# suryatmodulus/livekit-server

Hardware: AMD Instinct MI355X
Metric: forwarded RTP pkts/sec per GPU & node (bit-exact) + % HBM roofline (higher is better)
Workload: dtype u8; 1 GPU; configs[1]: 100 rooms x 10 participants per GPU, VP8 3-layer simulcast + Opus, 18000 DownTracks, 2% loss, 1% reorder, layer switching; batch=1 s of media per step, step=raw datagrams -> Buffer.calc -> forward (lkf_ingest_device + lkf_run), parallelism=room-sharded x1

## Files before the change

### livekit-server_amd/csrc/forward_kernels.hip

```cpp
#include <hip/hip_runtime.h>

#include "../../include/lkfwd.h"
#ifndef LKF_SVC_STATS
#define LKF_SVC_STATS 0
#endif
#if LKF_SVC_STATS
__device__ unsigned long long g_svc[64 * 48];
#define SVC_ADD(k, v) atomicAdd(&g_svc[(blockIdx.x & 63) * 48 + (k)], (unsigned long long)(v))
#endif
#include "dd_device.h"
#include "fwd_state.h"
#include "kernels.h"
#include "sender_device.h"

namespace lkf {

using u8 = uint8_t;
using u16 = uint16_t;
using u32 = uint32_t;
using u64 = uint64_t;
using i32 = int32_t;
using i64 = int64_t;

constexpr u64 HALF64 = 1ull << 63;
constexpr i32 INVALID = -1;


#ifndef LKF_CHECKED
#define LKF_CHECKED 0
#endif
#if LKF_CHECKED
__device__ unsigned long long g_chk[4];
__device__ __noinline__ void chk_fail(u32 site, u64 idx, u64 cap) {
  if (atomicAdd(&g_chk[0], 1ull) == 0) {
    g_chk[1] = site;
    g_chk[2] = idx;
    g_chk[3] = cap;
  }
}
#define CHK(cond, site, idx, cap)                   \
  do {                                              \
    if (!(cond)) chk_fail(site, u64(idx), u64(cap)); \
  } while (0)
#else
#define CHK(cond, site, idx, cap) \
  do {                            \
  } while (0)
#endif
enum ChkSite : u32 {
  CK_DEC_DT = 1,
  CK_DEC_TRACK,
  CK_DEC_PKT,
  CK_DEC_TUPLE,
  CK_DEC_SEQ,
  CK_DEC_LAYER,
  CK_DEC_EVENT,
  CK_EMIT_POS,
  CK_EMIT_DT,
  CK_EMIT_TUPLE,
  CK_EMIT_PKT,
  CK_EMIT_ARENA,
  CK_EMIT_OUT,
  CK_EMIT_BYTES,
  CK_EMIT_DD,
  CK_EMIT_GROUP,
  CK_PAD_DT,
  CK_PAD_SEQ,
  CK_EV_ORDER,
};

struct PktV {
  u64 esn, ets;
  i64 arr;
  u32 arenaOff, ssrc;
  u16 poff, plen;
  u8 hdr0, hdr1, flags, vfirst, vbits, vhs, tl0, tid, keyidx, vp9;
  int8_t spatial, temporal, layer;
  u16 pid;
};

__device__ __forceinline__ PktV decode_pkt(uint4 a, uint4 b, uint4 c, uint4 d) {
  PktV v;
  v.esn = (u64(a.y) << 32) | a.x;
  v.ets = (u64(a.w) << 32) | a.z;
  v.arr = i64((u64(b.y) << 32) | b.x);
  v.arenaOff = b.z;
  v.ssrc = c.x;
  v.poff = u16(c.y & 0xffff);
  v.plen = u16(c.y >> 16);
  v.hdr0 = u8(c.z);
  v.hdr1 = u8(c.z >> 8);
  v.spatial = int8_t(c.z >> 16);
  v.temporal = int8_t(c.z >> 24);
  v.flags = u8(c.w);
  v.vfirst = u8(c.w >> 8);
  v.vbits = u8(c.w >> 16);
  v.vhs = u8(c.w >> 24);
  v.pid = u16(d.x & 0xffff);
  v.tl0 = u8(d.x >> 16);
  v.tid = u8(d.x >> 24);
  v.keyidx = u8(d.y);
  v.layer = int8_t(d.y >> 8);
  v.vp9 = u8(d.y >> 24);
  return v;
}

__device__ __forceinline__ PktV load_pkt(const lkf_pkt *p) {
  const uint4 *q = reinterpret_cast<const uint4 *>(p);
  return decode_pkt(q[0], q[1], q[2], q[3]);
}

__device__ __forceinline__ uint4 rfl(uint4 v) {
  v.x = __builtin_amdgcn_readfirstlane(v.x);
  v.y = __builtin_amdgcn_readfirstlane(v.y);
  v.z = __builtin_amdgcn_readfirstlane(v.z);
  v.w = __builtin_amdgcn_readfirstlane(v.w);
  return v;
}

__device__ __forceinline__ u32 lane_id() { return threadIdx.x & 63u; }
__device__ __forceinline__ u32 rl32(u32 v, u32 l) { return __builtin_amdgcn_readlane(v, l); }
__device__ __forceinline__ u64 rl64(u64 v, u32 l) {
  return (u64(rl32(u32(v >> 32), l)) << 32) | u64(rl32(u32(v), l));
}
__device__ __forceinline__ u32 sh32(u32 v, int src) { return u32(__shfl(int(v), src, 64)); }
__device__ __forceinline__ u64 sh64(u64 v, int src) {
  return (u64(sh32(u32(v >> 32), src)) << 32) | u64(sh32(u32(v), src));
}
__device__ __forceinline__ int prev_in(u64 m, u64 lt) {
  const u64 pm = m & lt;
  return pm ? 63 - __clzll(pm) : -1;
}
__device__ __forceinline__ u32 excl_scan_u32(u32 v, u32 lane) {
  u32 x = v;
#pragma unroll
  for (int o = 1; o < 64; o <<= 1) {
    u32 y = u32(__shfl_up(int(x), o, 64));
    if (lane >= u32(o)) x += y;
  }
  return x - v;
}
__device__ __forceinline__ u32 wave_sum_u32(u32 v) {
#pragma unroll
  for (int o = 32; o > 0; o >>= 1) v += u32(__shfl_xor(int(v), o, 64));
  return v;
}
__device__ __forceinline__ u64 wave_max_u64(u64 v) {
#pragma unroll
  for (int o = 32; o > 0; o >>= 1) {
    u64 y = sh64(v, int(threadIdx.x) ^ o);
    v = y > v ? y : v;
  }
  return v;
}

__device__ __forceinline__ u64 wave_or_u64(u64 v) {
#pragma unroll
  for (int o = 32; o > 0; o >>= 1) v |= sh64(v, int(threadIdx.x) ^ o);
  return rl64(v, 0);
}
__device__ __forceinline__ void wave_lds_sync() { __syncthreads(); }

struct Lane {
  DTHot &h;
  RangeEntry *rm;
  RangeEntry *rmG;
  u32 rmNew;
  bool rmLoaded;
  bool vcDirty;
  VP8Cold *vc;
  i32 *dropKey;
  i32 *exKey;
  i32 *missKey;
  i32 *missVal;
  SeqMeta *seq;
  u32 seqSize;
  SeqRM *srm;
  u32 srmCap;
  u32 kind, codec, hasRefTS, clockRate;
  u32 *offs;
  u8 extPlayout, extAbs, extDD, extTcc;
  DDState *dd;
  const DDStruct *ddRing;
  DDStruct *ddS;
  u32 ddSSlot;
  const DDPkt *ddPkts;
  const u16 *ddSpill;
  u8 *ddBuf;
  DDPkt *ddPktL;
  u32 *err;
};

__device__ __forceinline__ bool hasf(const Lane &L, u32 f) { return (L.h.flags & f) != 0; }
__device__ __forceinline__ void setf(Lane &L, u32 f, bool v) {
  if (v)
    L.h.flags |= f;
  else
    L.h.flags &= ~f;
}

__device__ __forceinline__ RangeEntry rm_at(const Lane &L, int i) {
  int idx = (int(L.h.rmHead) + i) % kRangeCap;
  return L.rm[idx];
}
__device__ __forceinline__ void rm_load(Lane &L) {
  if (L.rmLoaded) return;
  L.rmLoaded = true;
  const u32 nc = L.h.rmCount, old = nc - min(L.rmNew, nc);
  if (!old) return;
  wave_lds_sync();
  for (u32 i = lane_id(); i < old; i += 64) {
    const u32 idx = (u32(L.h.rmHead) + i) % kRangeCap;
    L.rm[idx] = L.rmG[idx];
  }
  wave_lds_sync();
}
__device__ __forceinline__ void rm_reset(Lane &L, u64 start, u64 val) {
  L.h.rmHead = 0;
  L.h.rmCount = 0;
  L.rmNew = 0;
  L.h.rmOpenStart = start;
  L.h.rmOpenValue = val;
}
__device__ __forceinline__ bool rm_exclude(Lane &L, u64 s, u64 e) {
  if (e == s || (e - s) > HALF64) return false;
  if (L.h.rmOpenStart > s) return false;
  u64 nv = L.h.rmOpenValue + (e - s);
  if (L.h.rmOpenStart == s) {
    L.h.rmOpenStart = e;
    L.h.rmOpenValue = nv;
    return true;
  }
  RangeEntry c;
  c.start = L.h.rmOpenStart;
  c.end = s - 1;
  c.value = L.h.rmOpenValue;
  if (L.h.rmCount < kRangeCap) {
    int idx = (int(L.h.rmHead) + int(L.h.rmCount)) % kRangeCap;
    L.rm[idx] = c;
    L.h.rmCount++;
  } else {
    L.rm[L.h.rmHead] = c;
    L.h.rmHead = u16((L.h.rmHead + 1) % kRangeCap);
  }
  L.rmNew++;
  L.h.rmOpenStart = e;
  L.h.rmOpenValue = nv;
  return true;
}
__device__ __forceinline__ bool rm_get(Lane &L, u64 key, u64 &out) {
  out = 0;
  if (key >= L.h.rmOpenStart) {
    out = L.h.rmOpenValue;
    return true;
  }
  const int nc = L.h.rmCount;
  if (nc == 0) return false;
  rm_load(L);
  if (key < rm_at(L, 0).start) return false;
  const u32 l = lane_id();
  int best = -1;
  bool bestIn = false;
  u64 bestVal = 0;
  for (int base = 0; base <= nc; base += 64) {
    const int i = base + int(l);
    bool in = false, between = false;
    u64 val = 0;
    if (i <= nc) {
      u64 nextStart = L.h.rmOpenStart;
      if (i < nc) {
        const RangeEntry rv = rm_at(L, i);
        in = (key - rv.start) < HALF64 && (rv.end - key) < HALF64;
        val = rv.value;
        nextStart = rv.start;
      }
      if (i > 0) {
        const u64 before = key - rm_at(L, i - 1).end;
        const u64 after = nextStart - key;
        between = before > 0 && before < HALF64 && after > 0 && after < HALF64;
      }
    }
    const u64 m = __ballot(in || between);
    if (m) {
      const u32 j = 63 - __clzll(m);
      best = base + int(j);
      bestIn = rl32(u32(in), j) != 0;
      bestVal = rl64(val, j);
    }
  }
  if (best < 0 || !bestIn) return false;
  out = bestVal;
  return true;
}

__device__ __forceinline__ void mg_updateSnOffset(Lane &L) {
  u64 v = 0;
  rm_get(L, L.h.extHighestIncomingSN + 1, v);
  L.h.snOffset = v;
}
__device__ __forceinline__ void mg_setLastSnTs(Lane &L, u64 esn, u64 ets) {
  L.h.extHighestIncomingSN = esn - 1;
  L.h.extLastSN = esn;
  L.h.extSecondLastSN = esn - 1;
  rm_reset(L, esn, 0);
  mg_updateSnOffset(L);
  L.h.extLastTS = ets;
  L.h.extSecondLastTS = ets;
}
__device__ __forceinline__ void mg_updateSnTsOffsets(Lane &L, u64 esn, u64 ets, u64 snAdj, u64 tsAdj) {
  L.h.extHighestIncomingSN = esn - 1;
  rm_reset(L, esn, esn - L.h.extLastSN - snAdj);
  mg_updateSnOffset(L);
  L.h.tsOffset = ets - L.h.extLastTS - tsAdj;
}
__device__ __forceinline__ void mg_packetDropped(Lane &L, u64 esn) {
  if (L.h.extHighestIncomingSN != esn) return;
  rm_exclude(L, L.h.extHighestIncomingSN, L.h.extHighestIncomingSN + 1);
  L.h.extLastSN = L.h.extSecondLastSN;
  mg_updateSnOffset(L);
  L.h.extLastTS = L.h.extSecondLastTS;
  setf(L, F_LAST_MARKER, hasf(L, F_SECOND_LAST_MARKER));
}
enum { ORD_CONTIG = 0, ORD_OOO = 1, ORD_GAP = 2, ORD_DUP = 3 };
enum { MG_OK = 0, MG_PADDING, MG_DUP, MG_OOO_MISS };
__device__ __forceinline__ void mg_inorder(Lane &L, const PktV &p, bool marker, u64 &osn, u64 &ots) {
  L.h.extHighestIncomingSN = p.esn;
  u64 msn = p.esn - L.h.snOffset;
  u64 mts = p.ets - L.h.tsOffset;
  L.h.extSecondLastSN = L.h.extLastSN;
  L.h.extLastSN = msn;
  L.h.extSecondLastTS = L.h.extLastTS;
  L.h.extLastTS = mts;
  setf(L, F_SECOND_LAST_MARKER, hasf(L, F_LAST_MARKER));
  setf(L, F_LAST_MARKER, marker);
  if (p.flags & LKF_PKT_KEYFRAME) {
    L.h.extRtxGateSn = msn;
    setf(L, F_RTX_GATE, true);
  }
  if (hasf(L, F_RTX_GATE) && (msn - L.h.extRtxGateSn) > 2000) setf(L, F_RTX_GATE, false);
  osn = msn;
  ots = mts;
}

__device__ int mg_update(Lane &L, const PktV &p, bool marker, int &ord, u64 &osn, u64 &ots) {
  i64 diff = i64(p.esn - L.h.extHighestIncomingSN);
  if ((diff == 1 && p.plen != 0) || diff > 1) {
    L.h.extHighestIncomingSN = p.esn;
    ord = diff > 1 ? ORD_GAP : ORD_CONTIG;
    u64 msn = p.esn - L.h.snOffset;
    u64 mts = p.ets - L.h.tsOffset;
    L.h.extSecondLastSN = L.h.extLastSN;
    L.h.extLastSN = msn;
    L.h.extSecondLastTS = L.h.extLastTS;
    L.h.extLastTS = mts;
    setf(L, F_SECOND_LAST_MARKER, hasf(L, F_LAST_MARKER));
    setf(L, F_LAST_MARKER, marker);
    if (p.flags & LKF_PKT_KEYFRAME) {
      L.h.extRtxGateSn = msn;
      setf(L, F_RTX_GATE, true);
    }
    if (hasf(L, F_RTX_GATE) && (msn - L.h.extRtxGateSn) > 2000) setf(L, F_RTX_GATE, false);
    osn = msn;
    ots = mts;
    return MG_OK;
  }
  if (diff < 0) {
    ord = ORD_OOO;
    u64 off = 0;
    if (!rm_get(L, p.esn, off)) return MG_OOO_MISS;
    u64 esn = p.esn - off;
    if (esn >= L.h.extLastSN) return MG_OOO_MISS;
    osn = esn;
    ots = p.ets - L.h.tsOffset;
    return MG_OK;
  }
  if (diff == 1) {
    L.h.extHighestIncomingSN = p.esn;
    rm_exclude(L, L.h.extHighestIncomingSN, L.h.extHighestIncomingSN + 1);
    mg_updateSnOffset(L);
    ord = ORD_CONTIG;
    return MG_PADDING;
  }
  ord = ORD_DUP;
  return MG_DUP;
}

__device__ __forceinline__ int miss_find(const Lane &L, i32 key) {
  const u32 l = lane_id();
  for (int base = 0; base < int(L.h.missCount); base += 64) {
    const int i = base + int(l);
    const int idx = (L.h.missHead + i) % kMissCap;
    const u64 m = __ballot(i < int(L.h.missCount) && L.missKey[idx] == key);
    if (m) return (L.h.missHead + base + __ffsll((long long)m) - 1) % kMissCap;
  }
  return -1;
}
__device__ __forceinline__ bool set_has(const i32 *keys, u8 head, u8 count, i32 key) {
  for (int i = 0; i < count; i++)
    if (keys[(head + i) % kSetCap] == key) return true;
  return false;
}
__device__ __forceinline__ bool set_has_u(const i32 *keys, u8 head, u8 count, i32 key) {
  const u32 l = lane_id();
  return __ballot(l < count && keys[(head + l) % kSetCap] == key) != 0;
}
__device__ __forceinline__ void set_add(i32 *keys, u8 &head, u8 &count, i32 key, int keep) {
  if (set_has_u(keys, head, count, key)) return;
  wave_lds_sync();
  keys[(head + count) % kSetCap] = key;
  count++;
  if (count > keep) {
    head = u8((head + count - keep) % kSetCap);
    count = u8(keep);
  }
  wave_lds_sync();
}

__device__ void vp8_record_missing_wide(Lane &L, i32 prevMax, i32 ext, i32 off) {
  const int e0 = L.h.missCount;
  int inE = 0;
  for (int i = 0; i < e0; i++) {
    int idx = (L.h.missHead + i) % kMissCap;
    i32 k = L.missKey[idx];
// ... 316 lines not shown
      break;
  }
}

__device__ bool fw_sourceSwitch(Lane &L, const PktV &p, i32 layer) {
  if (!hasf(L, F_STARTED)) {
    setf(L, F_STARTED, true);
    L.h.referenceLayerSpatial = layer;
    mg_setLastSnTs(L, p.esn, p.ets);
    if (hasf(L, F_VP8)) vp8_setLast(L, p);
    return true;
  } else if (L.h.referenceLayerSpatial == INVALID) {
    L.h.referenceLayerSpatial = layer;
  }
  const u64 extLastTS = L.h.extLastTS;
  u64 extExpectedTS = extLastTS;
  u64 extRefTS = extExpectedTS;
  if (L.hasRefTS) {
    i32 ref = L.h.referenceLayerSpatial;
    if (layer < 0 || layer >= 3 || ref < 0 || ref >= 3) return false;
    const bool svc = L.codec == LKF_CODEC_VP9 || L.codec == LKF_CODEC_AV1;
    const u32 off = svc ? 0u : L.offs[ref * 3 + layer];
    if (!svc && layer != ref && off == 0) return false;
    u32 ts = u32(p.ets) + off;
    extRefTS = (extRefTS & 0xFFFFFFFF00000000ull) + u64(ts);
    u32 e32 = u32(extExpectedTS);
    if (u32(ts - e32) < (1u << 31) && ts < e32) extRefTS += (1ull << 32);
    if (u32(e32 - ts) < (1u << 31) && e32 < ts && extRefTS >= (1ull << 32)) extRefTS -= (1ull << 32);
  }
  if (hasf(L, F_HAS_EXPECTED)) {
    if (hasf(L, F_STATS_INIT)) {
      i64 diff = (p.arr - L.h.statsFirstTime) * i64(L.clockRate) / 1000000000LL;
      extExpectedTS = L.h.statsExtStartTS + u64(diff);
    } else if (L.h.preStartTime != 0) {
      i64 since = p.arr - L.h.preStartTime;
      u64 rtpDiff = u64(since * i64(L.clockRate) / 1000000000LL);
      extExpectedTS = L.h.extFirstTS + rtpDiff;
      if (L.h.refTSOffset == 0) L.h.refTSOffset = extExpectedTS - extRefTS;
    }
  }
  extRefTS += L.h.refTSOffset;
  u64 extNextTS;
  const double cr = double(L.clockRate);
  if (L.h.lastSSRC == 0) {
    double diffSeconds = double(i64(extExpectedTS - extRefTS)) / cr;
    if (diffSeconds >= 0.0) {
      if (hasf(L, F_RESUME_BEHIND) && diffSeconds > 0.2)
        extNextTS = extExpectedTS;
      else if (diffSeconds > 2.0)
        extNextTS = extExpectedTS;
      else
        extNextTS = extRefTS;
    } else {
      extNextTS = extRefTS;
    }
    setf(L, F_RESUME_BEHIND, false);
  } else {
    double diffSeconds = double(i64(extRefTS - extLastTS)) / cr;
    if (diffSeconds < 0.0) {
      if (fabs(diffSeconds) > 0.05) return false;
      extNextTS = extLastTS + 1;
    } else {
      extNextTS = extRefTS;
    }
  }
  if (i64(extNextTS - extLastTS) <= 0) extNextTS = extLastTS + 1;
  mg_updateSnTsOffsets(L, p.esn, p.ets, 1, extNextTS - extLastTS);
  if (hasf(L, F_VP8)) vp8_updateOffsets(L, p);
  return true;
}

__device__ __forceinline__ int fw_common(Lane &L, const PktV &p, i32 layer, bool marker, int &ord, u64 &osn,
                                         u64 &ots) {
  if (L.h.lastSSRC != p.ssrc) {
    if (!fw_sourceSwitch(L, p, layer)) return LKF_DROP_SWITCH;
    L.h.lastSSRC = p.ssrc;
  }
  int r = mg_update(L, p, marker, ord, osn, ots);
  if (r == MG_PADDING) return LKF_DROP_PADDING;
  if (r == MG_DUP) return LKF_DROP_DUPLICATE;
  if (r == MG_OOO_MISS) return LKF_DROP_OOO_MISS;
  return -1;
}

template <bool DDK = false>
__device__ __forceinline__ void vls_rollback(Lane &L) {
  if (DDK && hasf(L, F_DD)) {
    L.dd->mask = L.dd->prevMask;
    if (L.dd->flags & DS_HAS_PREV_MASK)
      L.dd->flags |= DS_HAS_MASK;
    else
      L.dd->flags &= ~u32(DS_HAS_MASK);
  }
  L.h.curS = L.h.prevS;
  L.h.curT = L.h.prevT;
  L.h.tgtS = L.h.ptgtS;
  L.h.tgtT = L.h.ptgtT;
}

struct Fwd {
  int ord;
  u64 osn, ots;
  bool switching, resuming, marker;
  int cbLen;
  u64 cb;
  int ddLen;
};

template <bool DDK>
__device__ int fw_translate(Lane &L, const PktV &p, u32 k, Fwd &o) {
  o.switching = o.resuming = o.marker = false;
  o.cbLen = 0;
  o.cb = 0;
  o.ddLen = 0;
  const i32 layer = p.layer;
  if (hasf(L, F_MUTED) || hasf(L, F_PUBMUTED)) return LKF_DROP_MUTED;
  if (!hasf(L, F_VIDEO)) return fw_common(L, p, layer, false, o.ord, o.osn, o.ots);
  if (L.h.tgtS == INVALID || L.h.tgtT == INVALID) return LKF_DROP_PAUSED;
  bool isSelected = false, isSwitching = false, isResuming = false;
  const bool kf = p.flags & LKF_PKT_KEYFRAME;
  const bool pktMarker = p.hdr1 & 0x80;
  if (hasf(L, F_SIMULCAST)) {
    if (L.h.curS != L.h.tgtS) {
      bool isActive = L.h.curS != INVALID && L.h.curT != INVALID;
      bool found = false;
      if (kf) {
        if (layer > L.h.curS && layer <= L.h.tgtS) found = true;
        if (layer < L.h.curS && layer >= L.h.tgtS) found = true;
      }
      if (found) {
        L.h.prevS = L.h.curS;
        L.h.prevT = L.h.curT;
        L.h.curS = layer;
        L.h.curT = p.temporal;
        L.h.ptgtS = L.h.tgtS;
        L.h.ptgtT = L.h.tgtT;
        if (L.h.curS >= L.h.maxS || L.h.curS == L.h.seenS) L.h.tgtS = L.h.curS;
        isSwitching = true;
        if (!isActive) isResuming = true;
      }
    }
    if (L.h.curS > L.h.maxS && layer <= L.h.maxS && kf) {
      L.h.prevS = L.h.curS;
      L.h.prevT = L.h.curT;
      L.h.curS = layer;
      L.h.ptgtS = L.h.tgtS;
      L.h.ptgtT = L.h.tgtT;
      if (L.h.curS >= L.h.maxS || L.h.curS == L.h.seenS) L.h.tgtS = layer;
      isSwitching = true;
    }
    isSelected = layer == L.h.curS;
  }
  bool marker = pktMarker;
  if (hasf(L, F_VP9)) {
    bool relevant = false;
    if (p.flags & LKF_PKT_VP9) {
      const bool U = p.vp9 & LKF_VP9_U, B = p.vp9 & LKF_VP9_B, E = p.vp9 & LKF_VP9_E, P = p.vp9 & LKF_VP9_P;
      const i32 pS = p.spatial, pT = p.temporal;
      i32 cS = L.h.curS, cT = L.h.curT;
      bool zero = false;
      if (L.h.curS != L.h.tgtS || L.h.curT != L.h.tgtT) {
        i32 uS = L.h.curS, uT = L.h.curT;
        const bool curValid = L.h.curS != INVALID && L.h.curT != INVALID;
        if (!curValid) {
          if (!kf)
            zero = true;
          else {
            uS = pS;
            uT = pT;
          }
        } else {
          if (L.h.curT != L.h.tgtT) {
            if (L.h.curT < L.h.tgtT) {
              if (pT > L.h.curT && pT <= L.h.tgtT && U && B) cT = uT = pT;
            } else if (E) {
              uT = L.h.tgtT;
            }
          }
          if (L.h.curS != L.h.tgtS) {
            if (L.h.curS < L.h.tgtS) {
              if (pS > L.h.curS && pS <= L.h.tgtS && !P && B) cS = uS = pS;
            } else if (E) {
              uS = L.h.tgtS;
            }
          }
        }
        if (!zero && (uS != L.h.curS || uT != L.h.curT)) {
          isSwitching = true;
          if (!curValid && uS != INVALID && uT != INVALID) isResuming = true;
          L.h.prevS = L.h.curS;
          L.h.prevT = L.h.curT;
          L.h.curS = uS;
          L.h.curT = uT;
        }
      }
      if (!zero) {
        if (E && pS == cS && (P || L.h.tgtS <= L.h.curS)) marker = true;
        isSelected = !(pS > cS || (pS == cS && pT > cT));
        relevant = true;
      }
    }
    if (!isSelected) {
      if (relevant && hasf(L, F_STARTED)) {
        int ord;
        u64 a, b;
        if (mg_update(L, p, marker, ord, a, b) == MG_OK && ord == ORD_CONTIG) mg_packetDropped(L, p.esn);
      }
      return LKF_DROP_NOT_SELECTED;
    }
  }
  if (DDK && hasf(L, F_DD)) {
    const bool inDD = (p.flags & LKF_PKT_DD) && L.ddPkts;
    if (inDD) {
      const u32 ln = lane_id();
      if (ln < sizeof(DDPkt) / 16)
        reinterpret_cast<uint4 *>(L.ddPktL)[ln] = reinterpret_cast<const uint4 *>(L.ddPkts + k)[ln];
      wave_lds_sync();
    }
    const bool hasDD = inDD && (L.ddPktL->flags & DP_VALID);
#if LKF_SVC_STATS
    const u64 tS0 = __builtin_amdgcn_s_memtime();
#endif
    const dd::SelResult r = dd::dd_select(*L.dd, L.ddRing, hasDD ? L.ddPktL : nullptr, pktMarker, L.h.curS, L.h.curT, L.h.prevS,
                                          L.h.prevT, L.h.tgtS, L.h.tgtT, L.ddBuf, L.ddS, L.ddSSlot, L.ddSpill);
#if LKF_SVC_STATS
    if (lane_id() == 0) {
      SVC_ADD(13, __builtin_amdgcn_s_memtime() - tS0);
      SVC_ADD(14, 1ull);
    }
#endif
    if (r.limit && lane_id() == 0) atomicOr(L.err, 16u);
    L.ddSSlot = r.stagedSlot;
    if (!r.selected) {
      if (r.relevant && hasf(L, F_STARTED)) {
        int ord;
        u64 a, b;
        if (mg_update(L, p, false, ord, a, b) == MG_OK && ord == ORD_CONTIG) mg_packetDropped(L, p.esn);
      }
      return LKF_DROP_NOT_SELECTED;
    }
    isSelected = true;
    isSwitching = r.switching;
    isResuming = r.resuming;
    marker = r.marker;
    o.ddLen = r.ddLen;
  }
  if (!isSelected) return LKF_DROP_NOT_SELECTED;
  o.resuming = isResuming;
  o.switching = isSwitching;
  o.marker = marker;
  if (hasf(L, F_DEFICIENT) && L.h.tgtS < L.h.curS) {
    if (isSwitching) vls_rollback<DDK>(L);
    return LKF_DROP_DOWNGRADE;
  }
  int dr = fw_common(L, p, layer, marker, o.ord, o.osn, o.ots);
  if (dr >= 0 || p.plen == 0) {
    if (isSwitching) vls_rollback<DDK>(L);
    return dr;
  }
  i32 tl = L.h.curT;
  bool tSwitch = false;
  if (hasf(L, F_TLS_VP8)) {
    i32 cur = L.h.curT, tgt = L.h.tgtT, nxt = cur;
    if (cur != tgt && (p.flags & LKF_PKT_VP8) && (p.vbits & LKF_VP8_T)) {
      i32 tid = i32(p.tid);
      if (cur < tgt) {
        if (tid > cur && tid <= tgt && (p.vbits & LKF_VP8_S) && (p.vbits & LKF_VP8_Y)) {
          tl = tid;
          nxt = tid;
        }
      } else if (pktMarker) {
        nxt = tgt;
      }
    }
    if (nxt != L.h.curT) {
      tSwitch = true;
      L.h.prevS = L.h.curS;
      L.h.prevT = L.h.curT;
      L.h.curT = nxt;
    }
  }
  if (hasf(L, F_VP8)) {
    int cr;
    if (!(p.flags & LKF_PKT_VP8))
      cr = CM_ERR;
    else
      cr = vp8_update(L, p, o.ord == ORD_OOO, o.ord == ORD_GAP, tl, o.cb, o.cbLen);
    if (cr != CM_OK) {
      if (cr == CM_FILTERED) mg_packetDropped(L, p.esn);
      if (isSwitching || tSwitch) vls_rollback<DDK>(L);
      return cr == CM_FILTERED ? LKF_DROP_TEMPORAL : cr == CM_PICID_MISS ? LKF_DROP_PICID_MISS : LKF_DROP_OTHER;
    }
  }
  return -1;
}


__device__ __forceinline__ u32 pack4(u8 a, u8 b, u8 c, u8 d) {
  return u32(a) | (u32(b) << 8) | (u32(c) << 16) | (u32(d) << 24);
}
struct __attribute__((aligned(8))) U4x8 {
  u32 x, y, z, w;
};
__device__ __forceinline__ void store_fwd(FwdRec *dst, FwdBase *wdst, u64 bSN, u64 bTS, u64 sn, u64 ts, u32 pkt,
                                          u32 relOff, u32 outLen, u32 flags, u32 ddLen, u32 aux) {
  if ((((sn - bSN) + 0x80000000ull) >> 32) != 0 || (((ts - bTS) + 0x80000000ull) >> 32) != 0) {
    flags |= T_WIDE;
    *wdst = FwdBase{sn, ts};
  }
  *reinterpret_cast<U4x8 *>(dst) = U4x8{u32(sn), u32(ts), pkt, relOff >> 4};
  reinterpret_cast<uint2 *>(dst)[2] = make_uint2(outLen | (flags << 16) | (ddLen << 24), aux);
}
__device__ __forceinline__ u32 vp8_aux(u32 mpid, u32 mtl0, u32 mkey) {
  return (mpid & 0xffffu) | ((mtl0 & 0xffu) << 16) | ((mkey & 0x1fu) << 24);
}
__device__ __forceinline__ u32 vp8_aux_of(u64 cb) {
  if (!(cb & 0x80)) return 0;
  const u32 x = u32(cb >> 8) & 0xff;
  int idx = 2;
  u32 pid = 0, tl0 = 0, key = 0;
  if (x & 0x80) {
    const u32 b = u32(cb >> (8 * idx)) & 0xff;
    if (b & 0x80) {
      pid = ((b & 0x7f) << 8) | (u32(cb >> (8 * (idx + 1))) & 0xff);
      idx += 2;
    } else {
      pid = b;
      idx++;
    }
  }
  if (x & 0x40) tl0 = u32(cb >> (8 * idx++)) & 0xff;
  if (x & 0x30) key = u32(cb >> (8 * idx)) & 0x1f;
  return vp8_aux(pid, tl0, key);
}
__device__ __forceinline__ void store_rec(SeqMeta *dst, const SeqMeta &m) {
  uint4 *d = reinterpret_cast<uint4 *>(dst);
  d[0] = make_uint4(u32(m.sourceSeqNo) | (u32(m.targetSeqNo) << 16), m.timestamp, m.lastNack,
                    pack4(m.marker, m.nacked, u8(m.layer), m.codecLen));
  d[1] = make_uint4(pack4(m.codec[0], m.codec[1], m.codec[2], m.codec[3]),
                    pack4(m.codec[4], m.codec[5], m.codec[6], m.codec[7]), 0u, 0u);
}

__device__ __forceinline__ void seq_invalidate(Lane &L, u32 n) {
  const SeqMeta z = {};
  for (u32 i = lane_id(); i < n; i += 64) {
    u32 x = u32(L.h.seqHighSlot) + 1 + i;
    while (x >= L.seqSize) x -= L.seqSize;
    store_rec(L.seq + x, z);
  }
}
__device__ __forceinline__ RangeEntry *srm_ring(SeqRM *h) { return reinterpret_cast<RangeEntry *>(h + 1); }
__device__ bool srm_get(SeqRM *h, u32 cap, u64 key, u64 &out) {
  out = 0;
  if (key >= h->openStart) {
    out = h->openValue;
    return true;
  }
  const u32 nc = h->count;
  const RangeEntry *ring = srm_ring(h);
  if (nc == 0 || key < ring[h->head].start) return false;
  for (i32 idx = i32(nc); idx >= 0; idx--) {
    u64 start = h->openStart;
    if (idx != i32(nc)) {
      const RangeEntry rv = ring[(h->head + u32(idx)) % cap];
      if ((key - rv.start) < HALF64 && (rv.end - key) < HALF64) {
        out = rv.value;
        return true;
      }
      start = rv.start;
    }
    if (idx > 0) {
      const RangeEntry pv = ring[(h->head + u32(idx) - 1) % cap];
      const u64 before = key - pv.end, after = start - key;
      if (before > 0 && before < HALF64 && after > 0 && after < HALF64) return false;
    }
  }
  return false;
}
__device__ bool srm_exclude(SeqRM *h, u32 cap, u64 s, u64 e, bool store) {
  if (e == s || (e - s) > HALF64) return false;
  if (h->openStart > s) return false;
  const u64 nv = h->openValue + (e - s);
  if (h->openStart == s) {
    if (store) {
      h->openStart = e;
      h->openValue = nv;
    }
    return true;
  }
  if (store) {
    RangeEntry c;
    c.start = h->openStart;
    c.end = s - 1;
    c.value = h->openValue;
    RangeEntry *ring = srm_ring(h);
    if (h->count < cap) {
      ring[(h->head + h->count) % cap] = c;
      h->count++;
    } else {
      ring[h->head] = c;
      h->head = (h->head + 1) % cap;
    }
    h->openStart = e;
    h->openValue = nv;
  }
  return true;
}
__device__ __noinline__ void seq_push_rm(DTHot *h, SeqMeta *seq, u32 size, SeqRM *srm, u32 cap, u64 esn,
                                         const SeqMeta *rec, u64 ets) {
  const bool init = !(h->flags & F_SEQ_INIT);
  u64 snOff = srm->snOffset;
  if (init) {
    h->flags |= F_SEQ_INIT;
    h->seqExtStartSN = esn;
    h->seqExtHighestSN = esn;
    h->seqExtHighestTS = ets;
    u64 off = 0;
    if (srm_get(srm, cap, esn + 1, off)) snOff = off;
    if (lane_id() == 0) srm->snOffset = snOff;
    h->seqHighSlot = u16((esn - snOff) % size);
  }
  if (esn < h->seqExtStartSN) return;
  const u64 adjH = h->seqExtHighestSN - snOff;
  u64 adjM = esn - snOff;
  if (esn < h->seqExtHighestSN) {
    u64 off = 0;
    if (!srm_get(srm, cap, esn, off)) return;
    adjM = esn - off;
  }
  const i64 delta = i64(adjM - adjH);
  if (delta <= -i64(size)) return;
  u32 slot;
  if (delta >= 0) {
    slot = u32((u64(h->seqHighSlot) + u64(delta) % size) % size);
  } else {
    const i32 sl = i32(h->seqHighSlot) + i32(delta);
    slot = u32(sl < 0 ? sl + i32(size) : sl);
  }
  if (adjM > adjH + 1) {
    const u64 nInv = (adjM - adjH - 1) < u64(size) ? (adjM - adjH - 1) : u64(size);
    for (u32 i = lane_id(); i < u32(nInv); i += 64) seq[(u32(h->seqHighSlot) + 1 + i) % size] = SeqMeta{};
  }
  if (lane_id() == 0) seq[slot] = *rec;
  if (esn > h->seqExtHighestSN) {
    h->seqExtHighestSN = esn;
    h->seqHighSlot = u16(slot);
  }
  if (ets > h->seqExtHighestTS) h->seqExtHighestTS = ets;
}

template <bool RM>
__device__ void seq_push(Lane &L, i64 arrMs, u64 inSN, u64 esn, u64 ets, bool marker, int8_t layer, u64 cb,
                         int cbLen) {
  const u32 size = L.seqSize;
  if (hasf(L, F_SEQ_INIT) && esn == L.h.seqExtHighestSN + 1) {
    u32 slot = u32(L.h.seqHighSlot) + 1;
    if (slot == size) slot = 0;
    SeqMeta m = {};
    m.sourceSeqNo = u16(inSN);
    m.targetSeqNo = u16(esn);
    m.timestamp = u32(ets);
    m.lastNack = u32(arrMs - L.h.seqStartMs);
    m.marker = marker;
    m.layer = layer;
    m.codecLen = u8(cbLen);
#pragma unroll
    for (int i = 0; i < 8; i++) m.codec[i] = u8(cb >> (8 * i));
    CHK(slot < size, CK_DEC_SEQ, slot, size);
    if (lane_id() == 0) store_rec(L.seq + slot, m);
    L.h.seqExtHighestSN = esn;
    L.h.seqHighSlot = u16(slot);
    if (ets > L.h.seqExtHighestTS) L.h.seqExtHighestTS = ets;
    return;
  }

  if (hasf(L, F_SEQ_RM) && (!hasf(L, F_SEQ_INIT) || esn < L.h.seqExtHighestSN)) {
    if (!RM) {
      if (lane_id() == 0) atomicOr(L.err, 32u);
      return;
    }
    SeqMeta m = {};
    m.sourceSeqNo = u16(inSN);
    m.targetSeqNo = u16(esn);
    m.timestamp = u32(ets);
    m.lastNack = u32(arrMs - L.h.seqStartMs);
    m.marker = marker;
    m.layer = layer;
    m.codecLen = u8(cbLen);
#pragma unroll
    for (int i = 0; i < 8; i++) m.codec[i] = u8(cb >> (8 * i));
    __shared__ SeqMeta sRec;
    if (lane_id() == 0) sRec = m;
    __syncthreads();
    seq_push_rm(&L.h, L.seq, size, L.srm, L.srmCap, esn, &sRec, ets);
    __syncthreads();
    return;
  }
  if (!hasf(L, F_SEQ_INIT)) {
    setf(L, F_SEQ_INIT, true);
    L.h.seqExtStartSN = esn;
    L.h.seqExtHighestSN = esn;
    L.h.seqExtHighestTS = ets;
    L.h.seqHighSlot = u16(esn % size);
  }
  if (esn < L.h.seqExtStartSN) return;
  const u64 adjH = L.h.seqExtHighestSN;
  const u64 adjM = esn;
  const i64 delta = i64(adjM - adjH);
  if (delta <= -i64(size)) return;
  u32 slot;
  if (delta >= 0) {
    u32 dm = delta < i64(size) ? u32(delta) : u32(u64(delta) % size);
    slot = L.h.seqHighSlot + dm;
    if (slot >= size) slot -= size;
  } else {
    i32 sl = i32(L.h.seqHighSlot) + i32(delta);
    slot = u32(sl < 0 ? sl + i32(size) : sl);
  }
  if (adjM > adjH + 1) {
    const u64 nInv = (adjM - adjH - 1) < u64(size) ? (adjM - adjH - 1) : u64(size);
    seq_invalidate(L, u32(nInv));
  }
  SeqMeta m = {};
  m.sourceSeqNo = u16(inSN);
  m.targetSeqNo = u16(esn);
  m.timestamp = u32(ets);
  m.lastNack = u32(arrMs - L.h.seqStartMs);
  m.marker = marker;
  m.nacked = 0;
  m.layer = layer;
  m.codecLen = u8(cbLen);
#pragma unroll
  for (int i = 0; i < 8; i++) m.codec[i] = u8(cb >> (8 * i));
  CHK(slot < size, CK_DEC_SEQ, slot, size);
  L.seq[slot] = m;
  if (esn > L.h.seqExtHighestSN) {
    L.h.seqExtHighestSN = esn;
    L.h.seqHighSlot = u16(slot);
  }
  if (ets > L.h.seqExtHighestTS) L.h.seqExtHighestTS = ets;
}

__device__ __forceinline__ u64 wave_sum(u64 v) {
  for (int o = 32; o > 0; o >>= 1) v += __shfl_xor(v, o, 64);
  return v;
}

__global__ void k_batch_init(u32 ntracks, u32 ndts, u32 nstats, u32 *__restrict__ tBegin, u32 *__restrict__ tEnd,
                             u32 *__restrict__ tRuns, u32 *__restrict__ err, u64 *__restrict__ stats,
                             u32 *__restrict__ fwdCnt, u64 *__restrict__ fwdBytes) {
  const u32 stride = gridDim.x * blockDim.x;
  for (u32 i = blockIdx.x * blockDim.x + threadIdx.x; i < ntracks || i < ndts || i < nstats || i < 4; i += stride) {
    if (i < ntracks) {
      tBegin[i] = 0;
      tEnd[i] = 0;
      tRuns[i] = 0;
    }
    if (i < ndts) {
      fwdCnt[i] = 0;
      fwdBytes[i] = 0;
    }
    if (i < nstats) stats[i] = 0;
    if (i < 4) err[i] = 0;
  }
}

__global__ void k_track_ranges(const RunDesc *__restrict__ desc, u32 ntracks, u32 *__restrict__ tBegin,
                               u32 *__restrict__ tEnd, u32 *__restrict__ tRuns, u32 *__restrict__ err) {
  const lkf_pkt *__restrict__ pkts = reinterpret_cast<const lkf_pkt *>(desc->pkts);
  u32 n = desc->n;
  const u64 *nDev = reinterpret_cast<const u64 *>(desc->nDev);
  u32 i = blockIdx.x * blockDim.x + threadIdx.x;
  if (nDev && *nDev < n) n = u32(*nDev);
  if (i >= n) return;
  u32 t = pkts[i].track;
  if (t >= ntracks) {
    atomicOr(err, 1u);
    return;
  }
  u32 tp = i > 0 ? pkts[i - 1].track : 0xffffffffu;
  u32 tn = i + 1 < n ? pkts[i + 1].track : 0xffffffffu;
  if (tp != t) {
    tBegin[t] = i;
    if (atomicAdd(&tRuns[t], 1u) != 0) atomicOr(err, 2u);
  }
  if (tn != t) tEnd[t] = i + 1;
}

constexpr int SCAN_T = 256;
#ifndef LKF_SCAN_ITEMS
#define LKF_SCAN_ITEMS 4
#endif
constexpr int SCAN_ITEMS = LKF_SCAN_ITEMS;
constexpr int SCAN_TILE = SCAN_T * SCAN_ITEMS;

struct ScanIn {
  int mode;
  const u32 *perm;
  const DevDT *dts;
  const u32 *tBegin, *tEnd;
  const u32 *cnt;
  const u64 *bytes;
  u32 *gFirst;
  u64 gCap;
};

__device__ __forceinline__ void scan_load(const ScanIn &in, u32 i, u64 &a, u64 &b) {
  const u32 d = in.perm ? in.perm[i] : i;
  if (in.mode == 3) {
    a = in.cnt[i] != 0 ? 1 : 0;
    b = in.cnt[i] & 0xffffu;
    return;
  }
  if (in.mode == 2) {
    a = in.cnt[i];
    b = 0;
    return;
  }
  if (in.mode == 0) {
    DevDT dt = in.dts[d];
    a = dt.active ? u64(in.tEnd[dt.track] - in.tBegin[dt.track]) : 0;
    b = 0;
  } else {
    a = in.cnt[d];
    b = in.bytes[d];
  }
}

__device__ __forceinline__ void block_scan_excl(u64 &a, u64 &b, u64 &ta, u64 &tb) {
  const int lane = threadIdx.x & 63, wid = threadIdx.x >> 6;
  u64 ia = a, ib = b;
  for (int o = 1; o < 64; o <<= 1) {
    u64 xa = __shfl_up(ia, o, 64), xb = __shfl_up(ib, o, 64);
    if (lane >= o) {
      ia += xa;
      ib += xb;
    }
  }
  __shared__ u64 wa[SCAN_T / 64], wb[SCAN_T / 64];
  if (lane == 63) {
    wa[wid] = ia;
    wb[wid] = ib;
  }
  __syncthreads();
  u64 pa = 0, pb = 0;
  ta = tb = 0;
  for (int w = 0; w < SCAN_T / 64; w++) {
    if (w < wid) {
      pa += wa[w];
      pb += wb[w];
    }
    ta += wa[w];
    tb += wb[w];
  }
  __syncthreads();
  a = pa + ia - a;
  b = pb + ib - b;
}

constexpr u32 kScanStHead = 16;
constexpr u32 kScanSpin = 1u << 22;

__device__ __forceinline__ void gr_put(u64 *g, u32 v, u32 tag = 1) {
  __hip_atomic_store(g, (u64(tag) << 32) | u64(v), __ATOMIC_RELAXED, __HIP_MEMORY_SCOPE_AGENT);
}

__global__ void __launch_bounds__(SCAN_T) k_scan_1p(ScanIn in, u32 n, u32 nb, u64 *__restrict__ st,
                                                    u64 *__restrict__ outA, u64 *__restrict__ outB,
                                                    u64 *__restrict__ totA, u64 *__restrict__ totB) {
  __shared__ u32 sTile, sLast;
  __shared__ u64 sPre[2];
  __shared__ u32 sBad;
  u32 *const ctr = reinterpret_cast<u32 *>(st);
  u64 *const gr = st + kScanStHead;
  const u32 tid = threadIdx.x, lane = tid & 63;
  if (tid == 0) {
    sTile = atomicAdd(&ctr[0], 1u);
    sBad = 0;
  }
  __syncthreads();
  const u32 tile = sTile;
  const u32 i0 = tile * SCAN_TILE + tid * SCAN_ITEMS;
  u64 va[SCAN_ITEMS], vb[SCAN_ITEMS], ta = 0, tb = 0;
#pragma unroll
  for (int k = 0; k < SCAN_ITEMS; k++) {
    va[k] = vb[k] = 0;
    if (i0 + k < n) scan_load(in, i0 + k, va[k], vb[k]);
    ta += va[k];
    tb += vb[k];
  }
  u64 ea = ta, eb = tb, TA, TB;
  block_scan_excl(ea, eb, TA, TB);
  u64 *const g = gr + 8 * size_t(tile);
  if (tid == 0) {
    if (tile == 0) {
      gr_put(g + 4, u32(TA)), gr_put(g + 5, u32(TA >> 32)), gr_put(g + 6, u32(TB)), gr_put(g + 7, u32(TB >> 32));
      sPre[0] = sPre[1] = 0;
    } else {
      gr_put(g + 0, u32(TA)), gr_put(g + 1, u32(TA >> 32)), gr_put(g + 2, u32(TB)), gr_put(g + 3, u32(TB >> 32));
    }
  }
  if (tile > 0 && tid < 64) {
    u64 pa = 0, pb = 0;
    int j = int(tile) - 1;
    for (u32 spins = 0;;) {
      const u64 x = lane < 8 ? __hip_atomic_load(gr + 8 * size_t(j) + lane, __ATOMIC_RELAXED, __HIP_MEMORY_SCOPE_AGENT)
                             : 0ull;
      const u64 rdy = __ballot(lane < 8 && (x >> 32) != 0);
      const u64 poison = __ballot(lane < 8 && (x >> 32) == 2);
      const u32 v = u32(x);
      if ((rdy & 0xF0) == 0xF0 || (rdy & 0x0F) == 0x0F) {
        const int o = (rdy & 0xF0) == 0xF0 ? 4 : 0;
        if (poison & (0x0Full << o)) {
          if (lane == 0) sBad = 1;
          break;
        }
        const u64 a = (u64(u32(__shfl(int(v), o + 1, 64))) << 32) | u32(__shfl(int(v), o, 64));
        const u64 b = (u64(u32(__shfl(int(v), o + 3, 64))) << 32) | u32(__shfl(int(v), o + 2, 64));
        pa += a;
        pb += b;
        if (o == 4) break;
        j--;
        spins = 0;
        continue;
      }
      if (++spins > kScanSpin) {
        if (lane == 0) sBad = 1;
        break;
      }
      __builtin_amdgcn_s_sleep(1);
    }
    if (lane == 0) {
      const u64 ia = pa + TA, ib = pb + TB;
      const u32 tag = sBad ? 2u : 1u;
      gr_put(g + 4, u32(ia), tag), gr_put(g + 5, u32(ia >> 32), tag), gr_put(g + 6, u32(ib), tag),
          gr_put(g + 7, u32(ib >> 32), tag);
      sPre[0] = pa;
      sPre[1] = pb;
    }
  }
  __syncthreads();
  u64 ca = sPre[0] + ea, cb = sPre[1] + eb;
#pragma unroll
  for (int k = 0; k < SCAN_ITEMS; k++) {
    const u32 d = i0 + k;
    if (d < n) {
      outA[d] = ca;
      if (outB) outB[d] = cb;
      if (in.gFirst && va[k]) {
        const u64 r0 = ca, r1 = min(r0 + va[k], in.gCap);
        for (u64 gg = (r0 + 63) >> 6; (gg << 6) < r1; gg++) in.gFirst[gg] = d;
      }
    }
    ca += va[k];
    cb += vb[k];
  }
  if (tile == nb - 1 && tid == 0) {
    *totA = sBad ? ~0ull : sPre[0] + TA;
    if (totB) *totB = sBad ? ~0ull : sPre[1] + TB;
  }
  __syncthreads();
  if (tid == 0) sLast = atomicAdd(&ctr[2], 1u) == nb - 1 ? 1u : 0u;
  __syncthreads();
  if (sLast) {
    for (u32 k = tid; k < 8 * nb; k += SCAN_T)
      __hip_atomic_store(gr + k, 0ull, __ATOMIC_RELAXED, __HIP_MEMORY_SCOPE_AGENT);
    if (tid == 0) {
      __hip_atomic_store(&ctr[0], 0u, __ATOMIC_RELAXED, __HIP_MEMORY_SCOPE_AGENT);
      __hip_atomic_store(&ctr[2], 0u, __ATOMIC_RELAXED, __HIP_MEMORY_SCOPE_AGENT);
    }
  }
}

struct SsEnt;
struct LaneOut {
  FwdRec *outT;
  FwdBase *outW;
  u64 nFwd, nBytes, nTuples;
  u64 bSN, bTS;
  SenderStats *ss;
  u32 *ssRing, *ssGap;
  SsEnt *ssBuf;
  u32 ssN;
  i32 sentDiff;
  u32 relOff;
  u32 drops[LKF_DROP_NREASONS];
  u8 *ddArena;
  u64 *ddUsed;
  u64 ddCap;
#if LKF_CHECKED
  u64 tupBase, tupCap;
#endif
};

__device__ __forceinline__ double rl_f64(double v, u32 k) {
  return __builtin_bit_cast(double, rl64(__builtin_bit_cast(u64, v), k));
}

struct SsEnt {
  u32 sn, ts;
  i64 t;
  u32 hp;
  u32 fl;
};
static_assert(sizeof(SsEnt) == 24, "SsEnt is 24 B");
__device__ __forceinline__ void ss_put(SsEnt *e, u64 sn, u64 ts, i64 t, u32 hdr, u32 pay, bool marker, bool kf) {
  *reinterpret_cast<uint2 *>(e) = make_uint2(u32(sn), u32(ts));
  reinterpret_cast<uint2 *>(e)[1] = make_uint2(u32(u64(t)), u32(u64(t) >> 32));
  reinterpret_cast<uint2 *>(e)[2] = make_uint2(hdr | (pay << 16), (marker ? 1u : 0u) | (kf ? 2u : 0u));
}

#ifndef LKF_SS_SCALAR
#define LKF_SS_SCALAR 0
#endif
__device__ __forceinline__ void ss_flush(SenderStats &S, u32 *ring, u32 *gap, const SsEnt *buf, u32 m, u64 bSN,
                                      u64 bTS) {
  if (m <= u32(LKF_SS_SCALAR)) {
    for (u32 i = 0; i < m; i++) {
      const SsEnt &e = buf[i];
      ss::ss_update(S, ring, gap, e.t, widen32(bSN, e.sn), widen32(bTS, e.ts), (e.fl & 1) != 0, e.hp & 0xffffu,
                    e.hp >> 16, 0);
      if (e.fl & 2) S.keyFrames++;
      wave_lds_sync();
    }
    return;
  }
  const u32 lane = lane_id();
  const u64 lt = (1ull << lane) - 1;
  const bool valid = lane < m;
  u64 esn = 0, ets = 0;
  i64 t = 0;
  u32 hdr = 0, pay = 0;
  bool marker = false, kf = false;
  if (valid) {
    const SsEnt &e = buf[lane];
    esn = widen32(bSN, e.sn);
    ets = widen32(bTS, e.ts);
    t = e.t;
    hdr = e.hp & 0xffffu;
    pay = e.hp >> 16;
    marker = e.fl & 1;
    kf = e.fl & 2;
  }
  const u64 pEsn = sh64(esn, lane ? int(lane) - 1 : 0), pEts = sh64(ets, lane ? int(lane) - 1 : 0);
  u32 pos = 0;
  while (pos < m) {
    const bool inSeg = valid && lane >= pos;
    const u64 prev = lane > pos ? pEsn : S.extHighestSN;
    const u64 g = esn - prev;
    const bool ok = S.initialized && pay > 0 && i64(g) > 0 && g <= 64 && ets >= S.extStartTS &&
                    (lane == pos || ets >= pEts);
    const u64 badM = __ballot(inSeg && !ok);
    const u32 end = badM ? u32(__ffsll((long long)badM) - 1) : m;
    if (end > pos) {
      const bool act = lane >= pos && lane < end;
      if (act && g >= 2) {
        atomicAdd(&gap[g - 1 > u64(kGapBins) ? kGapBins - 1 : u32(g - 2)], 1u);
        for (u64 q = prev + 1; q != esn; q++) ring[q & ss::kSnMask] = 0;
      }
      if (act)
        ring[esn & ss::kSnMask] =
            u32(u16(hdr + pay)) | (u32(u8(hdr)) << 16) | ((marker ? ss::kFlagMarker : 0u) << 24);
      const u64 before = (lane > pos && pEts > S.extHighestTS) ? pEts : S.extHighestTS;
      const u64 upM = __ballot(act && ets > before);
      const bool isNew = act && ets != (lane > pos ? pEts : S.lastJitterExtTimestamp);
      const u64 newM = __ballot(isNew);
      const i64 since = i64(u64(t) - u64(S.firstTime));
      const u64 rtp = u64(i64(u64(since) * u64(i64(S.clockRate))) / 1000000000LL);
      const u64 transit = rtp - ets;
      const int pn = prev_in(newM, lt);
      const u64 pnT = sh64(transit, pn >= 0 ? pn : int(lane));
      const u64 prevTransit = pn >= 0 ? pnT : S.lastTransit;
      i64 dj = i64(transit - prevTransit);
      if (dj < 0) dj = i64(0 - u64(dj));
      const double dd = double(dj);
      const u64 useM = __ballot(isNew && prevTransit != 0);
      const u32 sumB = wave_sum_u32(act ? hdr + pay : 0u), sumH = wave_sum_u32(act ? hdr : 0u);
      const u32 lost = wave_sum_u32((act && g >= 2) ? u32(g - 1) : 0u);
      const u32 frames = u32(__popcll(__ballot(act && marker))), kfs = u32(__popcll(__ballot(act && kf)));
      double j = S.jitter, mj = S.maxJitter;
      for (u64 w = newM; w; w &= w - 1) {
        const u32 k = u32(__ffsll((long long)w) - 1);
        if ((useM >> k) & 1) {
          j += (rl_f64(dd, k) - j) / 16;
          if (j > mj) mj = j;
        }
      }
      const u64 lastEsn = rl64(esn, end - 1);
      u64 trL = 0, etsL = 0, tU = 0, etsU = 0;
      if (newM) {
        const u32 kl = 63 - __clzll(newM);
        trL = rl64(transit, kl);
        etsL = rl64(ets, kl);
      }
      if (upM) {
        const u32 ku = 63 - __clzll(upM);
        tU = rl64(u64(t), ku);
        etsU = rl64(ets, ku);
      }
      wave_lds_sync();
      if (lane == 0) {
        S.jitter = j;
        S.maxJitter = mj;
        if (newM) {
          S.lastTransit = trL;
          S.lastJitterExtTimestamp = etsL;
        }
        if (upM) {
          S.highestTime = i64(tU);
          S.extHighestTS = etsU;
        }
        S.extHighestSN = lastEsn;
        S.packetsLost += lost;
        S.bytes += sumB;
        S.headerBytes += sumH;
        S.frames += frames;
        S.keyFrames += kfs;
      }
      wave_lds_sync();
    }
    pos = end;
    if (pos < m) {
      ss::ss_update(S, ring, gap, i64(rl64(u64(t), pos)), rl64(esn, pos), rl64(ets, pos), rl32(u32(marker), pos) != 0,
                    rl32(hdr, pos), rl32(pay, pos), 0);
      if (rl32(u32(kf), pos)) S.keyFrames++;
      wave_lds_sync();
      pos++;
    }
  }
}

__device__ __forceinline__ void fwd_base(LaneOut &o, u64 fwM, u64 osn, u64 ots) {
  if (!fwM || o.nFwd != 0) return;
  const u32 f0 = u32(__ffsll((long long)fwM) - 1);
  o.bSN = rl64(osn, f0);
  o.bTS = rl64(ots, f0);
}

template <bool DDK>
__device__ __forceinline__ void decide_step(Lane &L, const PktV &p, u32 k, LaneOut &o) {
  o.nTuples++;
  Fwd f;
  const u32 fl = L.h.flags;
  const bool contig = p.ssrc == L.h.lastSSRC && p.plen != 0 && p.esn == L.h.extHighestIncomingSN + 1;
  int dr;
  f.switching = f.resuming = false;
  f.cbLen = 0;
  f.cb = 0;
  f.ddLen = 0;
  f.ord = ORD_CONTIG;
  int cls;
  const i32 layer = p.layer;
  const bool kf = p.flags & LKF_PKT_KEYFRAME;
  if (fl & (F_MUTED | F_PUBMUTED)) {
    cls = LKF_DROP_MUTED;
  } else if (!(fl & F_VIDEO)) {
    cls = contig ? -1 : -2;
  } else if (L.h.tgtS == INVALID || L.h.tgtT == INVALID) {
    cls = LKF_DROP_PAUSED;
  } else if (!(fl & F_SIMULCAST)) {
    cls = (fl & (F_VP9 | F_DD)) ? -2 : LKF_DROP_NOT_SELECTED;
  } else {
    const bool willSwitch =
        kf && ((L.h.curS != L.h.tgtS && ((layer > L.h.curS && layer <= L.h.tgtS) ||
                                         (layer < L.h.curS && layer >= L.h.tgtS))) ||
               (L.h.curS > L.h.maxS && layer <= L.h.maxS));
    if (willSwitch)
      cls = -2;
    else if (layer != L.h.curS)
      cls = LKF_DROP_NOT_SELECTED;
    else if ((fl & F_DEFICIENT) && L.h.tgtS < L.h.curS)
      cls = LKF_DROP_DOWNGRADE;
    else if (contig && (fl & F_VP8) && (p.flags & LKF_PKT_VP8) && (fl & F_TLS_VP8))
      cls = -1;
    else
      cls = -2;
  }
  if (cls >= 0) {
    dr = cls;
  } else if (cls == -2) {
    dr = fw_translate<DDK>(L, p, k, f);
  } else if (!(fl & F_VIDEO)) {
    f.marker = false;
    mg_inorder(L, p, false, f.osn, f.ots);
    dr = -1;
  } else {
    const bool pktMarker = p.hdr1 & 0x80;
    f.marker = pktMarker;
    mg_inorder(L, p, pktMarker, f.osn, f.ots);
    i32 tl = L.h.curT;
    bool tSwitch = false;
    {
      const i32 cur = L.h.curT, tgt = L.h.tgtT;
      i32 nxt = cur;
      if (cur != tgt && (p.vbits & LKF_VP8_T)) {
        const i32 tid = i32(p.tid);
        if (cur < tgt) {
          if (tid > cur && tid <= tgt && (p.vbits & LKF_VP8_S) && (p.vbits & LKF_VP8_Y)) {
            tl = tid;
            nxt = tid;
          }
        } else if (pktMarker) {
          nxt = tgt;
        }
      }
      if (nxt != L.h.curT) {
        tSwitch = true;
        L.h.prevS = L.h.curS;
        L.h.prevT = L.h.curT;
        L.h.curT = nxt;
      }
    }
    const int cr = vp8_update(L, p, false, false, tl, f.cb, f.cbLen);
    if (cr != CM_OK) {
      if (cr == CM_FILTERED) mg_packetDropped(L, p.esn);
      if (tSwitch) vls_rollback(L);
      dr = cr == CM_FILTERED ? LKF_DROP_TEMPORAL : cr == CM_PICID_MISS ? LKF_DROP_PICID_MISS : LKF_DROP_OTHER;
    } else {
      dr = -1;
    }
  }
  if (dr >= 0) {
#pragma unroll
    for (int i = 0; i < LKF_DROP_NREASONS; i++) o.drops[i] += (dr == i) ? 1u : 0u;
    return;
  }
  const int cc = p.hdr0 & 0xf;
  const bool playout = L.extPlayout && !hasf(L, F_PLAYOUT_ACKED);
  const bool ddOn = DDK && f.ddLen > 0 && L.extDD;
  const int eh = (ddOn && f.ddLen > 16) ? 2 : 1;
  int extBytes = (ddOn ? eh + f.ddLen : 0) + (playout ? eh + 3 : 0) + (L.extAbs ? eh + 3 : 0) + (L.extTcc ? eh + 2 : 0);
  int extBlock = extBytes ? 4 + ((extBytes + 3) & ~3) : 0;
  int hdrLen = 12 + 4 * cc + extBlock;
  const bool useCodec = f.cbLen > 0 && (p.flags & LKF_PKT_VP8);
  int payLen = useCodec ? (f.cbLen + int(p.plen) - int(p.vhs)) : int(p.plen);
  const bool marker = f.marker || (p.hdr1 & 0x80);
  u32 flags = (f.switching ? LKF_OUT_SWITCHING : 0) | (f.resuming ? LKF_OUT_RESUMING : 0) |
              ((p.flags & LKF_PKT_KEYFRAME) ? LKF_OUT_KEYFRAME : 0) | (marker ? LKF_OUT_MARKER : 0) |
              (playout ? T_PLAYOUT : 0) | (useCodec ? T_CODEC : 0) | (ddOn ? T_DD : 0);
  u32 ddLen = ddOn ? u32(f.ddLen) : 0u;
  u32 aux = useCodec ? vp8_aux_of(f.cb) : 0u;
  if (DDK && ddOn) {
    u64 off = 0;
    if (lane_id() == 0) off = atomicAdd((unsigned long long *)o.ddUsed, (unsigned long long)f.ddLen);
    off = rl64(off, 0);
    if (off + u64(f.ddLen) > o.ddCap) {
      if (lane_id() == 0) atomicOr(L.err, 64u);
      flags &= ~u32(T_DD);
      ddLen = 0;
    } else {
      wave_lds_sync();
      for (int i = int(lane_id()); i < f.ddLen; i += 64) o.ddArena[off + u64(i)] = L.ddBuf[i];
      aux = u32(off);
    }
  }
#if LKF_CHECKED
  CHK(o.tupBase + o.nFwd < o.tupCap, CK_DEC_TUPLE, o.tupBase + o.nFwd, o.tupCap);
#endif
  fwd_base(o, 1ull, f.osn, f.ots);
  if (lane_id() == 0)
    store_fwd(o.outT + o.nFwd, o.outW + o.nFwd, o.bSN, o.bTS, f.osn, f.ots, k, o.relOff, u32(hdrLen + payLen), flags,
              ddLen, aux);
  seq_push<DDK>(L, p.arr / 1000000LL, p.esn, f.osn, f.ots, marker, p.layer, f.cb, f.cbLen);
  if (!hasf(L, F_STATS_INIT) && payLen > 0) {
    setf(L, F_STATS_INIT, true);
    L.h.statsFirstTime = p.arr;
    L.h.statsExtStartTS = f.ots;
  }
  if (lane_id() == 0)
    ss_put(o.ssBuf + o.ssN, f.osn, f.ots, p.arr, p.poff, u32(payLen), marker, (p.flags & LKF_PKT_KEYFRAME) != 0);
  o.ssN++;
  o.nFwd++;
  o.nBytes += u64(hdrLen + payLen);
  o.sentDiff += i32(p.poff) - hdrLen;
  o.relOff += u32((hdrLen + payLen + 15) & ~15);
}


#ifndef LKF_DECIDE_WAVES
#define LKF_DECIDE_WAVES 5
#endif
#ifndef LKF_DECIDE_DD_WAVES
#define LKF_DECIDE_DD_WAVES 3
#endif
#define DECIDE_ATTR __attribute__((amdgpu_waves_per_eu(DDK ? LKF_DECIDE_DD_WAVES : LKF_DECIDE_WAVES, 8)))

__device__ __forceinline__ void vm_drain() {
  __builtin_amdgcn_s_waitcnt(0x0F70);
}

__device__ __forceinline__ void pin_loaded(const uint4 &a, const uint4 &b, const uint4 &c, const uint4 &d) {
  asm volatile("" ::"v"(a.x), "v"(a.y), "v"(a.z), "v"(a.w), "v"(b.x), "v"(b.y), "v"(b.z), "v"(b.w), "v"(c.x),
               "v"(c.y), "v"(c.z), "v"(c.w), "v"(d.x), "v"(d.y), "v"(d.z), "v"(d.w));
}

__device__ __forceinline__ bool steady_state(const Lane &L) {
  const u32 fl = L.h.flags;
  return (fl & F_VIDEO) && (fl & F_SIMULCAST) && !(fl & (F_MUTED | F_PUBMUTED)) &&
         L.h.tgtS != INVALID && L.h.tgtT != INVALID && L.h.curS == L.h.tgtS && L.h.curS <= L.h.maxS &&
         L.h.curS >= 0 && L.h.curS < 3;
}

__global__ void __launch_bounds__(64) k_layer_index(const RunDesc *__restrict__ desc, const u32 *__restrict__ tBegin,
                                                    const u32 *__restrict__ tEnd, u32 stride, u32 *__restrict__ list,
                                                    u32 *__restrict__ before, u32 *__restrict__ cnt,
                                                    u64 *__restrict__ zero2) {
  const lkf_pkt *__restrict__ pkts = reinterpret_cast<const lkf_pkt *>(desc->pkts);
  const u32 t = blockIdx.x, lane = threadIdx.x;
  if (zero2 && t == 0 && lane < 2) zero2[lane] = 0;
  const u64 lt = (1ull << lane) - 1;
  const u32 b = tBegin[t], e = tEnd[t];
  u32 c0 = 0, c1 = 0, c2 = 0;
  for (u32 base = b; base < e; base += 64) {
    const u32 i = base + lane;
    const int l = i < e ? int(reinterpret_cast<const int8_t *>(pkts + i)[53]) : -1;
    const u64 m0 = __ballot(l == 0), m1 = __ballot(l == 1), m2 = __ballot(l == 2);
    if (i < e) {
      const u32 r0 = c0 + u32(__popcll(m0 & lt)), r1 = c1 + u32(__popcll(m1 & lt)), r2 = c2 + u32(__popcll(m2 & lt));
      before[i] = r0;
      before[stride + i] = r1;
      before[2 * size_t(stride) + i] = r2;
      if (l == 0) list[b + r0] = i;
      if (l == 1) list[stride + b + r1] = i;
      if (l == 2) list[2 * size_t(stride) + b + r2] = i;
    }
    c0 += u32(__popcll(m0));
    c1 += u32(__popcll(m1));
    c2 += u32(__popcll(m2));
  }
  if (lane == 0) {
    cnt[t * 3] = c0;
    cnt[t * 3 + 1] = c1;
    cnt[t * 3 + 2] = c2;
  }
}

#ifndef LKF_SVC_CHAINS
#define LKF_SVC_CHAINS 1
#endif
constexpr int kSvcDDBytes = 48;
constexpr int kSvcFrames = 72;
enum : u32 { SK_BAD = 0, SK_FWD = 1, SK_MDROP = 2, SK_NDROP = 3 };

#if LKF_SVC_STATS
#define SVC_WHY(c) \
  if (why == 0 && inWin && !good) why = (c)
#else
#define SVC_WHY(c)
#endif

template <bool DDK>
__device__ __forceinline__ u32 svc_run(Lane &L, LaneOut &o, const PktV &p, u32 pi, u32 n, u32 pos, u32 nextAt,
                                       bool valid, i32 &sentAcc, u8 *sScr, u8 *sFD) {
  const u32 lane = lane_id();
  const u64 lt = (1ull << lane) - 1;
  const u32 fl = L.h.flags;
  const bool inWin = valid && lane >= pos && pi < nextAt;
  const u64 winM = __ballot(inWin);
  const bool dd = DDK && (fl & F_DD);
  {
    const int ns = (fl & (F_MUTED | F_PUBMUTED)) ? LKF_DROP_MUTED
                   : (L.h.tgtS == INVALID || L.h.tgtT == INVALID) ? LKF_DROP_PAUSED
                                                                  : -1;
    if (ns >= 0) {
      const u32 k = u32(__popcll(winM));
      o.nTuples += k;
      if (ns == LKF_DROP_MUTED)
        o.drops[LKF_DROP_MUTED] += k;
      else
        o.drops[LKF_DROP_PAUSED] += k;
      return pos + k;
    }
  }
  const bool curValid = L.h.curS != INVALID && L.h.curT != INVALID;
  const bool started = fl & F_STARTED;
  const bool relevantDrop = curValid && started;
  bool uni = true;
  const DDStruct *s = nullptr;
  int hiPos = -1, maxTgt = -1;
  u32 hiTarget = 0;
  bool swAll = false;
  u32 aboveM = 0, hiChain = 0xffffffffu;
  if (DDK && dd) {
    const DDState &d = *L.dd;
    uni = (d.flags & DS_KF_VALID) && (d.flags & DS_CACHE_INIT);
    uni = uni && u32(d.slot) == L.ddSSlot;
    s = L.ddS;
    for (int i = 0; uni && i < int(d.numTargets); i++) {
      if (!((d.dtActive >> i) & 1) || i32(s->dtS[i]) > L.h.tgtS || i32(s->dtT[i]) > L.h.tgtT) continue;
      const int target = s->dtTarget[i];
      maxTgt = max(maxTgt, target);
      if (d.numChains == 0 || !((d.chBroken >> s->protectedBy[target]) & 1)) {
        hiPos = i;
        hiTarget = u32(target);
        if (d.numChains) hiChain = s->protectedBy[target];
        break;
      }
      aboveM |= 1u << s->protectedBy[target];
    }
    swAll = hiPos >= 0 && (i32(s->dtS[hiPos]) != L.h.curS || i32(s->dtT[hiPos]) != L.h.curT);
  }
#if LKF_SVC_STATS
  if (!uni && lane == 0) SVC_ADD(3, 1ull);
  u32 why = 0;
#endif
  if (!uni) return pos;
#if LKF_SVC_STATS
  const u64 tA = __builtin_amdgcn_s_memtime();
  u64 tB = tA, tC = tA;
#endif
  bool good = inWin;
  u32 kind = SK_BAD;
  int nsr = LKF_DROP_NOT_SELECTED;
  bool mk = false;
  int ddLen = 0;
  u64 ddEfn = 0;
  bool ddPut = false, ddFwdSel = false;
  u32 chBrk = 0, chRst = 0;
  if (!dd) {
    const bool isV = p.flags & LKF_PKT_VP9;
    const bool U = p.vp9 & LKF_VP9_U, B = p.vp9 & LKF_VP9_B, E = p.vp9 & LKF_VP9_E, P = p.vp9 & LKF_VP9_P;
    const i32 pS = p.spatial, pT = p.temporal;
    const bool kf = p.flags & LKF_PKT_KEYFRAME;
    bool zero = !isV, sw = false;
    if (isV && (L.h.curS != L.h.tgtS || L.h.curT != L.h.tgtT)) {
      if (!curValid) {
        if (kf)
          sw = true;
        else
          zero = true;
      } else {
        i32 uS = L.h.curS, uT = L.h.curT;
        if (L.h.curT != L.h.tgtT) {
          if (L.h.curT < L.h.tgtT) {
            if (pT > L.h.curT && pT <= L.h.tgtT && U && B) uT = pT;
          } else if (E) {
            uT = L.h.tgtT;
          }
        }
        if (L.h.curS != L.h.tgtS) {
          if (L.h.curS < L.h.tgtS) {
            if (pS > L.h.curS && pS <= L.h.tgtS && !P && B) uS = pS;
          } else if (E) {
            uS = L.h.tgtS;
          }
        }
        sw = uS != L.h.curS || uT != L.h.curT;
      }
    }
    good = good && !sw;
    SVC_WHY(2);
    const bool sel = !zero && !(pS > L.h.curS || (pS == L.h.curS && pT > L.h.curT));
    mk = (p.hdr1 & 0x80) || (!zero && E && pS == L.h.curS && (P || L.h.tgtS <= L.h.curS));
    if (!sel) {
      kind = (!zero && started) ? SK_MDROP : SK_NDROP;
    } else if ((fl & F_DEFICIENT) && L.h.tgtS < L.h.curS) {
      kind = SK_NDROP;
      nsr = LKF_DROP_DOWNGRADE;
    } else {
      kind = SK_FWD;
    }
  } else if (DDK) {
    DDState &d = *L.dd;
    DDPkt dp;
    const bool hasDD = inWin && (p.flags & LKF_PKT_DD) && L.ddPkts;
    const DDPkt *const dpg = L.ddPkts + (hasDD ? pi : 0u);
    {
      const uint4 *src = reinterpret_cast<const uint4 *>(dpg);
      uint4 *dst = reinterpret_cast<uint4 *>(&dp);
#pragma unroll
      for (int k = 0; k < int(kDDPktScalar / 16); k++) dst[k] = hasDD ? src[k] : make_uint4(0, 0, 0, 0);
    }
    const bool ddLane = hasDD && (dp.flags & DP_VALID);
    const bool tmplSrc = LKF_DD_FASTBEST && u32(dp.slot) == u32(d.slot) && dp.custom == 0 &&
                         !(dp.flags & DP_ATTACHED) && dp.tmplIdx < s->numTmpl;
    const DDTmpl &tq = s->t[tmplSrc ? dp.tmplIdx : 0];
    auto chainDiff = [&](int c) -> u32 { return tmplSrc ? dd_tmpl_chain(tq, c) : dd_chain_diff(*dpg, c); };
    const u64 cl0 = d.cLast;
    const u64 efn = dp.extFN;
    const u64 ddM = __ballot(ddLane);
    const int pdl = prev_in(ddM, lt);
    const u64 pEfnL = sh64(efn, pdl >= 0 ? pdl : int(lane));
    const u64 pEfn = pdl >= 0 && u32(pdl) >= pos ? pEfnL : cl0;
    const u64 fi = efn - cl0;
    if (ddLane) good = good && efn >= pEfn && fi < u64(kSvcFrames) - 8;
    SVC_WHY(3);
    const bool newF = ddLane && efn != pEfn;
    const u32 dti = hiPos >= 0 ? dd::dti_at(dp.dtis, int(hiTarget)) : 0u;
    const bool t0 = hiPos >= 0 && dti != 0;
    if (ddLane) good = good && (maxTgt < 0 || int(dp.ndti) > maxTgt);
    SVC_WHY(4);
    const u64 newM = __ballot(inWin && newF);
    const u64 upto = newM & (lt | (1ull << lane));
    const u32 head = (fi == 0 || !upto) ? pos : u32(63 - __clzll(upto));
    const u64 after = newM & ~((2ull << lane) - 1);
    const u32 nextHead = after ? u32(__ffsll((long long)after) - 1) : 64u;
    const u64 frameM = (nextHead >= 64 ? ~0ull : ((1ull << nextHead) - 1)) & ~((1ull << head) - 1) & ddM;
    const int headL = frameM ? __ffsll((long long)frameM) - 1 : int(lane);
    const bool t0Head = sh32(u32(t0), headL) != 0;
    const u32 cache0 = dd::c_get(d, cl0);
    const bool drop0 = fi == 0 && cache0 == dd::SD_DROPPED;
    const bool early = ddLane && (drop0 || (!t0Head && int(lane) != headL));
    const bool eval = ddLane && !early;
    if (eval) good = good && t0 == t0Head;
    SVC_WHY(5);
    if (eval)
      good = good && !(dp.flags & DP_ATTACHED) && !(dp.extFlags & (LKF_DD_STRUCTURE_UPDATED | LKF_DD_ACTIVE_UPDATED)) &&
             dp.extKFN == d.extKeyFrameNum && int(dp.nchain) == int(d.numChains);
    SVC_WHY(6);
    ddFwdSel = eval && t0;
    if (ddFwdSel) good = good && !swAll && (d.flags & DS_FN_INIT);
    SVC_WHY(7);
    const u64 ordBadM = __ballot(ddLane && inWin && !(efn >= pEfn && fi < u64(kSvcFrames) - 8));
    const u32 ordEnd = ordBadM ? u32(__ffsll((long long)ordBadM) - 1) : 64u;
    const bool adds = inWin && lane < ordEnd && eval && (!t0 || (dp.extFlags & LKF_DD_INTEGRITY));
    for (int c = 0; c < int(d.numChains); c++) {
      if (((d.chBroken >> c) & 1) || !adds) continue;
      bool hit = dd::x_has(d, c, efn);
      if (efn > cl0) {
        const u64 k0 = cl0 >= dd::kNack ? cl0 - dd::kNack : 0, k1 = efn >= dd::kNack ? efn - dd::kNack : 0;
        const u64 a0 = cl0 >= dd::kEntries ? cl0 - dd::kEntries : 0, a1 = efn >= dd::kEntries ? efn - dd::kEntries : 0;
        hit = hit || dd::x_any_frames(d, c, k0, k1) || dd::x_any_frames(d, c, a0, a1);
      }
      if (hit) good = false;
    }
    SVC_WHY(14);
    const u64 addM = __ballot(adds);
    const bool firstAdd = adds && !(addM & frameM & lt);
    if (lane < u32(kSvcFrames)) sFD[lane] = u8(lane == 0 ? cache0 : dd::SD_UNKNOWN);
    if (lane + 64 < u32(kSvcFrames)) sFD[lane + 64] = u8(dd::SD_UNKNOWN);
    wave_lds_sync();
    if (firstAdd && fi < u64(kSvcFrames)) sFD[fi] = u8(t0 ? dd::SD_FORWARDED : dd::SD_DROPPED);
    wave_lds_sync();
    auto dec = [&](u64 e) -> u32 {
      if (e >= cl0 && e < efn) return sFD[e - cl0];
      bool old;
      return dd::c_decision(d, e, old);
    };
    if (eval && good)
      for (int c = 0; c < int(d.numChains); c++) {
        if (!((d.chActive >> c) & 1) || int(dp.nchain) <= c || chainDiff(c) != 0) continue;
        if (((aboveM >> c) & 1) || dd::x_any(d, c) || (!LKF_SVC_CHAINS && ((d.chBroken >> c) & 1)))
          good = false;
        else if (LKF_SVC_CHAINS)
          chRst |= 1u << c;
      }
    u32 rstSeen = 0;
    for (int c = 0; c < int(d.numChains); c++)
      if (__ballot(inWin && ((chRst >> c) & 1)) & lt) rstSeen |= 1u << c;
    if (eval && good)
      for (int c = 0; c < int(d.numChains); c++) {
        if (!((d.chActive >> c) & 1) || int(dp.nchain) <= c) continue;
        const u32 diff = chainDiff(c);
        if (diff == 0 || (((d.chBroken & ~rstSeen) >> c) & 1)) continue;
        const u32 sd = dec(efn - diff);
        if (sd == dd::SD_FORWARDED) continue;
        if (sd == dd::SD_UNKNOWN || u32(c) == hiChain || !LKF_SVC_CHAINS)
          good = false;
        else
          chBrk |= 1u << c;
      }
    SVC_WHY(8);
    if (ddFwdSel) good = good && (tmplSrc || dp.fdKind == FD_INLINE);
    if (ddFwdSel && good)
      for (int j = 0; j < int(dp.nfd) && (tmplSrc || j < kDDFdInline); j++) {
        const u32 f = tmplSrc ? u32(s->fdPool[tq.fdOff + j]) : u32(dpg->fd[j]);
        if (f != 0 && dec(efn - f) == dd::SD_DROPPED) good = false;
      }
    SVC_WHY(9);
#if LKF_SVC_STATS
    tB = __builtin_amdgcn_s_memtime();
#endif
    if (ddFwdSel && good) {
      const bool hasMask = d.flags & DS_HAS_MASK;
      const bool hasActive = (dp.flags & DP_ACTIVE) || hasMask;
      const u32 active = hasMask ? d.mask : dp.activeMask;
      ddLen = tmplSrc ? dd::dd_marshal_tmpl(*s, dp.tmplIdx, dp.flags, u16(efn + d.fnOffset), hasActive, active,
                                            sScr + lane * kSvcDDBytes, kSvcDDBytes)
                      : dd::dd_marshal_inl(*s, *dpg, u16(efn + d.fnOffset), hasActive, active,
                                           sScr + lane * kSvcDDBytes, kSvcDDBytes, nullptr, nullptr, false);
      if (ddLen < 0) good = false;
      mk = (p.hdr1 & 0x80) || ((dp.flags & DP_LAST) && L.h.curS == i32(dp.sid));
    }
    SVC_WHY(10);
#if LKF_SVC_STATS
    tC = __builtin_amdgcn_s_memtime();
#endif
    kind = ddFwdSel ? SK_FWD : (relevantDrop ? SK_MDROP : SK_NDROP);
    ddEfn = efn;
    ddPut = firstAdd;
  }
  const bool adv = kind == SK_FWD || kind == SK_MDROP;
  if (kind == SK_FWD) good = good && started && (fl & F_SEQ_INIT) && (fl & F_STATS_INIT);
  SVC_WHY(1);
  const u64 advM = __ballot(inWin && adv);
  const int pa = prev_in(advM, lt);
  const u64 paEsn = sh64(p.esn, pa >= 0 ? pa : int(lane));
  const u64 prevEsn = pa >= 0 && u32(pa) >= pos ? paEsn : L.h.extHighestIncomingSN;
  const u64 dEsn = p.esn - prevEsn;
  const bool contig = dEsn == 1;
  const bool gap = dEsn > 1 && dEsn < u64(L.seqSize) - 64;
  if (adv) good = good && p.ssrc == L.h.lastSSRC && p.plen != 0 && (contig || gap);
  SVC_WHY(11);
  const bool excl = kind == SK_MDROP && contig;
  if (excl) good = good && L.h.snOffset == L.h.rmOpenValue && L.h.rmOpenStart <= p.esn;
  SVC_WHY(12);
  const u64 exM = __ballot(inWin && excl);
  const u64 fwdM = __ballot(inWin && kind == SK_FWD);
  const u64 snOff = L.h.snOffset + u64(__popcll(exM & lt));
  const u64 osn = p.esn - snOff;
  const u64 ots = p.ets - L.h.tsOffset;
  const int pf = prev_in(fwdM, lt);
  const int pfs = pf >= 0 ? pf : int(lane);
  const u64 pfOsn = sh64(osn, pfs), pfOts = sh64(ots, pfs);
  const u64 prevOsn = pf >= 0 && u32(pf) >= pos ? pfOsn : L.h.seqExtHighestSN;
  const u64 hiTS = pf >= 0 && u32(pf) >= pos ? pfOts : L.h.seqExtHighestTS;
  if (kind == SK_FWD)
    good = good && ots >= hiTS && osn - prevOsn >= 1 && osn - prevOsn < u64(L.seqSize) - 64 &&
           osn - L.h.seqExtHighestSN < u64(L.seqSize) - 64;
  SVC_WHY(13);
  const u64 stopM = __ballot(inWin ? !good : (valid && lane >= pos));
  const u32 x = stopM ? u32(__ffsll((long long)stopM) - 1) : n;
#if LKF_SVC_STATS
  {
    const u32 wx = x < 64 ? rl32(why, x) : 0u;
    if (lane == 0) {
      SVC_ADD(0, 1ull);
      SVC_ADD(1, (unsigned long long)(x > pos ? x - pos : 0));
      if (x < n) SVC_ADD(16 + (wx ? wx : 15), 1ull);
    }
  }
#endif
#if LKF_SVC_STATS
  const u64 tD = __builtin_amdgcn_s_memtime();
  if (lane == 0 && dd) {
    SVC_ADD(10, (unsigned long long)(tB - tA));
    SVC_ADD(11, (unsigned long long)(tC - tB));
    SVC_ADD(12, (unsigned long long)(tD - tC));
  }
#endif
  if (x <= pos) return pos;
  const u64 runM = (x >= 64 ? ~0ull : ((1ull << x) - 1)) & ~((1ull << pos) - 1);
  const bool inRun = (runM >> lane) & 1;
  if (DDK && dd) {
    {
      DDState &d = *L.dd;
      for (int c = 0; c < int(d.numChains); c++) {
        const u64 bm = __ballot(inRun && ((chBrk >> c) & 1)), rm = __ballot(inRun && ((chRst >> c) & 1));
        if (!(bm | rm)) continue;
        const int lb = bm ? 63 - __clzll(bm) : -1, lr = rm ? 63 - __clzll(rm) : -1;
        if (lane == 0) d.chBroken = lb > lr ? (d.chBroken | (1u << c)) : (d.chBroken & ~(1u << c));
      }
      wave_lds_sync();
    }
    DDState &d = *L.dd;
    const u64 pM = __ballot(inRun && ddPut);
    const int pp = prev_in(pM, lt);
    const u64 ppE = sh64(ddEfn, pp >= 0 ? pp : int(lane));
    const u64 cur = pp >= 0 ? ppE : d.cLast;
    const bool put = inRun && ddPut && ddEfn > d.cBase;
    const bool grow = put && ddEfn > cur;
    const u64 g1M = __ballot(grow && ddEfn == cur + 1);
    const u64 gNM = __ballot(grow && ddEfn > cur + 1);
    u64 missE = 0;
    bool miss = false;
    if ((g1M >> lane) & 1) {
      const u64 ms = cur > dd::kNack + d.cBase ? cur - dd::kNack : d.cBase;
      const u64 me = ddEfn > dd::kNack + d.cBase ? ddEfn - dd::kNack : d.cBase;
      if (me > ms && dd::c_get(d, ms) == dd::SD_UNKNOWN) {
        miss = true;
        missE = ms;
      }
    }
    for (u64 m = gNM; m; m &= m - 1) {
      const u32 b = u32(__ffsll((long long)m) - 1);
      const u64 e = rl64(ddEfn, b), c0 = rl64(cur, b);
      const u64 ms = c0 > dd::kNack + d.cBase ? c0 - dd::kNack : d.cBase;
      const u64 me = e > dd::kNack + d.cBase ? e - dd::kNack : d.cBase;
      u32 st = dd::SD_UNKNOWN + 1;
      u64 ent = 0;
      if (lane < u32(e - c0 - 1)) {
        ent = c0 + 1 + lane;
        st = dd::SD_UNKNOWN;
      }
      const u64 mk2 = (me > ms && lane < u32(me - ms)) ? ms + lane : 0;
      const bool mMiss = me > ms && lane < u32(me - ms) && dd::c_get(d, mk2) == dd::SD_UNKNOWN;
      wave_lds_sync();
      if (st == dd::SD_UNKNOWN) {
        const u64 off = (ent - d.cBase) % dd::kEntries;
        const u32 bp = u32(off & 31) * 2;
        atomicOr(reinterpret_cast<unsigned long long *>(&d.masks[off >> 5]), 3ull << bp);
      }
      if (mMiss) {
        const u64 off = (mk2 - d.cBase) % dd::kEntries;
        const u32 bp = u32(off & 31) * 2;
        unsigned long long *w = reinterpret_cast<unsigned long long *>(&d.masks[off >> 5]);
        atomicAnd(w, ~(3ull << bp));
        atomicOr(w, u64(dd::SD_MISSING) << bp);
      }
      wave_lds_sync();
    }
    wave_lds_sync();
    if (miss) {
      const u64 off = (missE - d.cBase) % dd::kEntries;
      const u32 bp = u32(off & 31) * 2;
      unsigned long long *w = reinterpret_cast<unsigned long long *>(&d.masks[off >> 5]);
      atomicAnd(w, ~(3ull << bp));
      atomicOr(w, u64(dd::SD_MISSING) << bp);
    }
    if (put) {
      const u64 off = (ddEfn - d.cBase) % dd::kEntries;
      const u32 bp = u32(off & 31) * 2;
      unsigned long long *w = reinterpret_cast<unsigned long long *>(&d.masks[off >> 5]);
      atomicAnd(w, ~(3ull << bp));
      atomicOr(w, u64(kind == SK_FWD ? dd::SD_FORWARDED : dd::SD_DROPPED) << bp);
    }
    wave_lds_sync();
    const u64 aM = __ballot(put);
    const u64 eLast = aM ? rl64(ddEfn, 63 - __clzll(aM)) : 0;
    const u64 fM = __ballot(inRun && ddFwdSel);
    const u64 eF = fM ? rl64(ddEfn, 63 - __clzll(fM)) : 0;
    wave_lds_sync();
    if (aM && eLast > d.cLast) d.cLast = eLast;
    if (fM && eF > d.fnLast) d.fnLast = eF;
    wave_lds_sync();
  }
  const u64 fwR = fwdM & runM, exR = exM & runM;
  const u64 advR = advM & runM;
  const u64 setR = advR & ~exR;
  const bool f = inRun && kind == SK_FWD;
  o.nTuples += x - pos;
  {
    const bool nd = inRun && kind == SK_NDROP;
    o.drops[LKF_DROP_NOT_SELECTED] += u32(__popcll(__ballot(inRun && kind == SK_MDROP))) +
                                      u32(__popcll(__ballot(nd && nsr == LKF_DROP_NOT_SELECTED)));
    o.drops[LKF_DROP_DOWNGRADE] += u32(__popcll(__ballot(nd && nsr == LKF_DROP_DOWNGRADE)));
  }
  const int cc = p.hdr0 & 0xf;
  const bool playout = L.extPlayout && !(fl & F_PLAYOUT_ACKED);
  const bool ddOn = DDK && f && ddLen > 0 && L.extDD;
  const int eh = (ddOn && ddLen > 16) ? 2 : 1;
  const int extBytes =
      (ddOn ? eh + ddLen : 0) + (playout ? eh + 3 : 0) + (L.extAbs ? eh + 3 : 0) + (L.extTcc ? eh + 2 : 0);
  const int extBlock = extBytes ? 4 + ((extBytes + 3) & ~3) : 0;
  const int hdrLen = 12 + 4 * cc + extBlock;
  const u32 outLen = f ? u32(hdrLen + int(p.plen)) : 0u;
  const u32 aligned = (outLen + 15) & ~15u;
  const u32 relEx = excl_scan_u32(aligned, lane);
  bool ddKeep = ddOn;
  u32 ddOff = 0;
  if (DDK && dd) {
    const u32 dl = ddOn ? u32(ddLen) : 0u;
    const u32 dEx = excl_scan_u32(dl, lane);
    const u32 dTot = rl32(dEx + dl, 63);
    if (dTot) {
      u64 base = 0;
      if (lane == 0) base = atomicAdd(reinterpret_cast<unsigned long long *>(o.ddUsed), (unsigned long long)dTot);
      base = rl64(base, 0);
      if (base + dTot > o.ddCap) {
        if (lane == 0) atomicOr(L.err, 64u);
        ddKeep = false;
      } else if (ddOn) {
        u8 *dst = o.ddArena + base + dEx;
        const u32 *srcw = reinterpret_cast<const u32 *>(sScr + lane * kSvcDDBytes);
#pragma unroll
        for (int w = 0; w < kSvcDDBytes / 4; w++) {
          const u32 v = srcw[w];
#pragma unroll
          for (int b = 0; b < 4; b++)
            if (4 * w + b < ddLen) dst[4 * w + b] = u8(v >> (8 * b));
        }
        ddOff = u32(base + dEx);
      }
    }
  }
  const bool kf = p.flags & LKF_PKT_KEYFRAME;
  const u32 j = u32(__popcll(fwR & lt));
  fwd_base(o, fwR, osn, ots);
  if (f) {
#if LKF_CHECKED
    CHK(o.tupBase + o.nFwd + j < o.tupCap, CK_DEC_TUPLE, o.tupBase + o.nFwd + j, o.tupCap);
#endif
    store_fwd(o.outT + o.nFwd + j, o.outW + o.nFwd + j, o.bSN, o.bTS, osn, ots, pi, o.relOff + relEx, outLen,
              (kf ? LKF_OUT_KEYFRAME : 0) | (mk ? LKF_OUT_MARKER : 0) | (playout ? T_PLAYOUT : 0) | (ddKeep ? T_DD : 0),
              ddKeep ? u32(ddLen) : 0u, ddKeep ? ddOff : 0u);
    u32 slot = u32(L.h.seqHighSlot) + u32(osn - L.h.seqExtHighestSN);
    while (slot >= L.seqSize) slot -= L.seqSize;
    SeqMeta m = {};
    m.sourceSeqNo = u16(p.esn);
    m.targetSeqNo = u16(osn);
    m.timestamp = u32(ots);
    m.lastNack = u32(p.arr / 1000000LL - L.h.seqStartMs);
    m.marker = mk;
    m.layer = p.layer;
    m.codecLen = 0;
    CHK(slot < L.seqSize, CK_DEC_SEQ, slot, L.seqSize);
    store_rec(L.seq + slot, m);
  }
  for (u64 gm = __ballot(f && osn - prevOsn > 1); gm; gm &= gm - 1) {
    const u32 b = u32(__ffsll((long long)gm) - 1);
    const u64 from = rl64(prevOsn, b), to = rl64(osn, b);
    const u32 nsk = u32(to - from - 1);
    const u32 base = u32(L.h.seqHighSlot) + u32(from - L.h.seqExtHighestSN) + 1;
    for (u32 i = lane; i < nsk; i += 64) {
      u32 x2 = base + i;
      while (x2 >= L.seqSize) x2 -= L.seqSize;
      store_rec(L.seq + x2, SeqMeta{});
    }
  }
  if (f) ss_put(o.ssBuf + o.ssN + j, osn, ots, p.arr, p.poff, p.plen, mk, kf);
  o.ssN += u32(__popcll(fwR));
  const u32 sumLen = wave_sum_u32(outLen);
  sentAcc += f ? i32(p.poff) - hdrLen : 0;
  if (fwR) {
    o.nBytes += sumLen;
    o.nFwd += u32(__popcll(fwR));
    const u32 lastF = 63 - __clzll(fwR);
    u32 slot = u32(L.h.seqHighSlot) + u32(rl64(osn, lastF) - L.h.seqExtHighestSN);
    while (slot >= L.seqSize) slot -= L.seqSize;
    L.h.seqHighSlot = u16(slot);
    L.h.seqExtHighestSN = rl64(osn, lastF);
    L.h.seqExtHighestTS = rl64(ots, lastF);
    o.relOff += rl32(relEx + aligned, lastF);
  }
  if (advR) {
    const u64 mkM = __ballot(mk);
    const u32 lastA = 63 - __clzll(advR);
    L.h.extHighestIncomingSN = rl64(p.esn, lastA);
    const bool lastSets = (setR >> lastA) & 1;
    const u64 psM = setR & ((1ull << lastA) - 1);
    u64 sSN = L.h.extLastSN, sTS = L.h.extLastTS;
    bool sMk = fl & F_LAST_MARKER;
    if (psM) {
      const u32 b = 63 - __clzll(psM);
      sSN = rl64(osn, b);
      sTS = rl64(ots, b);
      sMk = (mkM >> b) & 1;
    }
    if (lastSets) {
      L.h.extSecondLastSN = sSN;
      L.h.extSecondLastTS = sTS;
      L.h.extLastSN = rl64(osn, lastA);
      L.h.extLastTS = rl64(ots, lastA);
      setf(L, F_SECOND_LAST_MARKER, sMk);
      setf(L, F_LAST_MARKER, (mkM >> lastA) & 1);
    } else {
      L.h.extSecondLastSN = L.h.extLastSN = sSN;
      L.h.extSecondLastTS = L.h.extLastTS = sTS;
      setf(L, F_SECOND_LAST_MARKER, sMk);
      setf(L, F_LAST_MARKER, sMk);
    }
    const u64 kfM = __ballot(((advR >> lane) & 1) && kf);
    if (kfM) {
      L.h.extRtxGateSn = rl64(osn, 63 - __clzll(kfM));
      setf(L, F_RTX_GATE, true);
    }
    if (hasf(L, F_RTX_GATE) && (rl64(osn, lastA) - L.h.extRtxGateSn) > 2000) setf(L, F_RTX_GATE, false);
    u64 m = exR;
    while (m) {
      const u32 b = u32(__ffsll((long long)m) - 1);
      const u64 s0 = rl64(p.esn, b);
      u64 e0 = s0 + 1;
      m &= m - 1;
      while (m) {
        const u32 b2 = u32(__ffsll((long long)m) - 1);
        if (rl64(p.esn, b2) != e0) break;
        e0++;
        m &= m - 1;
      }
      rm_exclude(L, s0, e0);
    }
    if (exR) L.h.snOffset = L.h.rmOpenValue;
  }
  return x;
}
#undef SVC_WHY

#ifndef LKF_DD_RESTAGE
#define LKF_DD_RESTAGE 1
#endif
__device__ __forceinline__ void dd_stage_struct(Lane &L, const DDState *sDD, u8 *sDDSRaw, u32 lane) {
  const u32 slot = __builtin_amdgcn_readfirstlane(u32(sDD->slot));
  const uint4 *gs = reinterpret_cast<const uint4 *>(L.ddRing + slot);
  uint4 *ls = reinterpret_cast<uint4 *>(sDDSRaw);
  const u32 nT = __builtin_amdgcn_readfirstlane(u32(L.ddRing[slot].numTmpl));
  const u32 nP = __builtin_amdgcn_readfirstlane(u32(L.ddRing[slot].nfdPool));
  constexpr u32 kTOff = __builtin_offsetof(DDStruct, t) / 16, kPOff = __builtin_offsetof(DDStruct, fdPool) / 16;
  const u32 nHead = kTOff + nT * (sizeof(DDTmpl) / 16), nPool = (nP + 15) / 16;
  for (u32 i = lane; i < nHead + nPool; i += 64) {
    const u32 k = i < nHead ? i : kPOff + (i - nHead);
    ls[k] = gs[k];
  }
  L.ddSSlot = slot;
  __syncthreads();
}
__device__ __forceinline__ void dd_restage(Lane &L, const DDState *sDD, u8 *sDDSRaw, u32 lane) {
  wave_lds_sync();
  const bool moved = __builtin_amdgcn_readfirstlane(int((sDD->flags & DS_KF_VALID) && u32(sDD->slot) != L.ddSSlot));
  if (LKF_DD_RESTAGE && moved) dd_stage_struct(L, sDD, sDDSRaw, lane);
}

constexpr u32 kDecideMaxK = 8;
#ifndef LKF_DEC_PREFETCH
#define LKF_DEC_PREFETCH 0
#endif
template <bool DDK>
__global__ void __launch_bounds__(64) DECIDE_ATTR k_decide_dt(DecideArgs A, const lkf_pkt *__restrict__ pkts) {
  __shared__ i32 sDrop[kSetCap];
  __shared__ i32 sEx[kSetCap];
  __shared__ i32 sMissKey[kMissCap];
  __shared__ i32 sMissVal[kMissCap];
  __shared__ RangeEntry sRm[kRangeCap];
  __shared__ __attribute__((aligned(16))) u8 sDDRaw[DDK ? sizeof(DDState) + kDDMaxBytes + 1 : 16];
  __shared__ __attribute__((aligned(16))) u8 sSvcScr[DDK ? 64 * kSvcDDBytes : 16];
  __shared__ __attribute__((aligned(16))) u8 sDDSRaw[DDK ? __builtin_offsetof(DDStruct, serBits) : 16];
  __shared__ u8 sSvcFD[kSvcFrames];
  DDState *const sDD = reinterpret_cast<DDState *>(sDDRaw);
  u8 *const sDDBuf = sDDRaw + (DDK ? sizeof(DDState) : 0);
  __shared__ uint4 sSlot[2 * kDecideMaxK];
  u64 todo;
  {
    const u32 K = A.perWave, lane = threadIdx.x;
    const u32 wj = A.waveBase + ((blockIdx.x >> 3) * K + lane) * 8 + (blockIdx.x & 7);
    u32 dj = 0xffffffffu, tj = 0, ej = 0, eej = 0, pbj = 0, pej = 0, cj = 0;
    if (lane < K && wj < A.waveEnd) {
      dj = A.sched[wj];
      tj = A.waveTrack[wj];
      ej = A.evOff[wj];
      eej = A.evOff[wj + 1];
    }
    if (dj != 0xffffffffu) {
      pbj = A.tBegin[tj];
      pej = A.tEnd[tj];
      cj = A.tracks[tj].codec;
    }
    todo = __ballot(dj != 0xffffffffu && (pbj < pej || ej < eej));
    if (lane < K) {
      sSlot[2 * lane] = make_uint4(wj, dj, tj, ej);
      sSlot[2 * lane + 1] = make_uint4(eej, pbj, pej, cj);
    }
    wave_lds_sync();
  }
  while (todo) {
  const u32 jw = u32(__ffsll(static_cast<long long>(todo))) - 1;
  todo &= todo - 1;
#if LKF_SVC_STATS
  const u64 tP0 = __builtin_amdgcn_s_memtime();
  u64 tRun = 0, tStep = 0, tLoad = 0, tSs = 0;
#endif
  u32 laneR;
  asm volatile("v_mov_b32 %0, %1" : "=v"(laneR) : "v"(threadIdx.x));
  const u32 lane = laneR;
  const u64 lt = (1ull << lane) - 1;
  const uint4 sa = sSlot[2 * jw], sb = sSlot[2 * jw + 1];
  const u32 w = __builtin_amdgcn_readfirstlane(sa.x);
  const u32 d = __builtin_amdgcn_readfirstlane(sa.y);
  const u32 track = __builtin_amdgcn_readfirstlane(sa.z);
  u32 ev = __builtin_amdgcn_readfirstlane(sa.w);
  const u32 evEnd = __builtin_amdgcn_readfirstlane(sb.x);
  CHK(d < A.maxDts, CK_DEC_DT, d, A.maxDts);
  CHK(track < A.maxTracks, CK_DEC_TRACK, track, A.maxTracks);
  CHK(evEnd <= A.nev, CK_DEC_EVENT, evEnd, A.nev);
  const DevDT dt = A.dts[d];
  const u32 pb = __builtin_amdgcn_readfirstlane(sb.y);
  u32 pe = __builtin_amdgcn_readfirstlane(sb.z);
  const u64 slot0 = A.slotBase[d];
  bool pre = LKF_DEC_PREFETCH && pe - pb <= 64u;
  uint4 r0 = make_uint4(0, 0, 0, 0), r1 = r0, r2 = r0, r3 = r0;
  if (pre && lane < pe - pb) {
    CHK(pb + lane < A.npkts, CK_DEC_PKT, pb + lane, A.npkts);
    const uint4 *ps = reinterpret_cast<const uint4 *>(pkts) + u64(pb + lane) * 4;
    r0 = ps[0];
    r1 = ps[1];
    r2 = ps[2];
    r3 = ps[3];
  }
  LaneOut o;
  o.nFwd = o.nBytes = o.nTuples = 0;
  o.sentDiff = 0;
  i32 sentAcc = 0;
  o.relOff = 0;
  o.bSN = o.bTS = 0;
  for (int i = 0; i < LKF_DROP_NREASONS; i++) o.drops[i] = 0;
  __shared__ __attribute__((aligned(16))) DTHot sHot;
  __shared__ __attribute__((aligned(16))) SenderStats sSS;
  __shared__ u32 sHot0[64];
  Lane L{sHot};
  {
    const u32 h0 = reinterpret_cast<const u32 *>(A.hot + d)[lane];
    reinterpret_cast<u32 *>(&sHot)[lane] = h0;
    sHot0[lane] = h0;
  }
  if (lane < sizeof(SenderStats) / 16)
    reinterpret_cast<uint4 *>(&sSS)[lane] = reinterpret_cast<const uint4 *>(A.ss + d)[lane];
  const bool vp8Track = __builtin_amdgcn_readfirstlane(sb.w) == LKF_CODEC_VP8;
  if (vp8Track && lane < u32(kSetCap)) {
    sDrop[lane] = A.vc[d].dropKey[lane];
    sEx[lane] = A.vc[d].exKey[lane];
  }
  __shared__ __attribute__((aligned(16))) SsEnt sSsBuf[64];
  o.ss = &sSS;
  o.ssBuf = sSsBuf;
  o.ssN = 0;
  o.ssRing = A.ssRing + size_t(d) * kSnInfoSize;
  o.ssGap = A.ssGap + size_t(d) * kGapWords;
  __syncthreads();
#if LKF_SVC_STATS
  const u64 tPa = __builtin_amdgcn_s_memtime();
#endif
  RangeEntry *const rmG = A.rm + size_t(d) * kRangeCap;
  L.rm = sRm;
  L.rmG = rmG;
  L.rmNew = 0;
  L.rmLoaded = false;
  L.vcDirty = false;
  L.vc = A.vc + d;
  L.dropKey = sDrop;
  L.exKey = sEx;
  L.missKey = sMissKey;
  L.missVal = sMissVal;
  if (vp8Track) {
    for (u32 i = lane; i < L.h.missCount; i += 64) {
      const u32 idx = (L.h.missHead + i) % kMissCap;
      sMissKey[idx] = L.vc->missKey[idx];
      sMissVal[idx] = L.vc->missVal[idx];
    }
  }
  if (slot0 + (pe - pb) > A.tupleCap) {
    if (lane == 0) atomicOr(A.err, 8u);
    pe = pb;
  }
  __syncthreads();
  L.seq = A.seq + size_t(d) * A.seqSize;
  L.seqSize = A.seqSize;
  L.srm = DDK ? reinterpret_cast<SeqRM *>(A.srm + size_t(d) * A.srmStride) : nullptr;
  L.srmCap = A.srmCap;
  const DevTrack &tk = A.tracks[track];
  L.kind = tk.kind;
  L.codec = tk.codec;
  L.hasRefTS = tk.hasRefTS;
  L.clockRate = tk.clockRate;
  L.offs = A.dtOffs + size_t(d) * kDTOffsWords;
  L.extPlayout = dt.extPlayout;
  L.extAbs = dt.extAbs;
  L.extDD = dt.extDD;
  L.extTcc = dt.extTcc;
  L.err = A.err;
  L.ddPkts = A.ddPkts;
  __shared__ __attribute__((aligned(16))) DDPkt sDDPkt;
  L.ddPktL = &sDDPkt;
  L.ddSpill = A.ddSpill;
  L.ddRing = nullptr;
  L.ddS = reinterpret_cast<DDStruct *>(sDDSRaw);
  L.ddSSlot = 0xffffffffu;
  L.dd = sDD;
  L.ddBuf = sDDBuf;
  o.ddArena = A.ddArena;
  o.ddUsed = A.ddUsed;
  o.ddCap = A.ddCap;
#if LKF_CHECKED
  o.tupBase = slot0;
  o.tupCap = A.tupleCap;
  CHK(pe <= A.npkts, CK_DEC_PKT, pe, A.npkts);
#endif
  const bool ddDT = DDK && (L.h.flags & F_DD) && A.ddState;
  if (ddDT) {
    L.ddRing = A.ddStructs + size_t(tk.ddIdx) * kDDSlots;
    const uint4 *g = reinterpret_cast<const uint4 *>(A.ddState + d);
    uint4 *l = reinterpret_cast<uint4 *>(sDD);
    const u32 nc0 = __builtin_amdgcn_readfirstlane(u32(A.ddState[d].numChains));
    const u32 nDD = (kDDStateHead + nc0 * kDDExpRow * 8) / 16;
    for (u32 i = lane; i < nDD; i += 64) l[i] = g[i];
    __syncthreads();
    if (sDD->flags & DS_KF_VALID) dd_stage_struct(L, sDD, sDDSRaw, lane);
  }
  o.outT = A.recs + slot0;
  o.outW = A.wide + slot0;
  const bool svcDT = DDK && (L.h.flags & F_VIDEO) && !(L.h.flags & F_SIMULCAST) &&
                     ((L.h.flags & F_VP9) || ((L.h.flags & F_DD) && ddDT));
  u32 nextAt = ev < evEnd ? A.events[ev].at : 0xffffffffu;
  const uint4 *src = reinterpret_cast<const uint4 *>(pkts);

  u32 kpos = pb;
#if LKF_SVC_STATS
  const u64 tP1 = __builtin_amdgcn_s_memtime();
#endif
  while (kpos < pe) {
#if LKF_SVC_STATS
    const u64 tc0 = __builtin_amdgcn_s_memtime();
#endif
    if (nextAt <= kpos) {
      while (nextAt <= kpos) {
        apply_ctl(L, A.events[ev++]);
        nextAt = ev < evEnd ? A.events[ev].at : 0xffffffffu;
      }
      vm_drain();
    }
    const bool steady = pe - pb > 64 && steady_state(L);
    u32 pi, n, lim;
    if (steady) {
      const u32 ls = u32(L.h.curS);
      CHK(size_t(ls) * A.pktStride + kpos < 3 * size_t(A.pktStride), CK_DEC_LAYER, size_t(ls) * A.pktStride + kpos,
          3 * size_t(A.pktStride));
      const u32 j = A.layerBefore[size_t(ls) * A.pktStride + kpos] + lane;
      pi = j < A.layerCnt[track * 3 + ls] ? A.layerList[size_t(ls) * A.pktStride + pb + j] : 0xffffffffu;
      const u32 stopAt = min(nextAt, pe);
      n = u32(__popcll(__ballot(pi < stopAt)));
      lim = n == 64 ? rl32(pi, 63) + 1 : stopAt;
    } else {
      n = min(64u, pe - kpos);
      pi = kpos + lane;
      lim = kpos + n;
    }
    const bool valid = lane < n;
    if (!pre) {
      r0 = r1 = r2 = r3 = make_uint4(0, 0, 0, 0);
      if (valid) {
        CHK(pi < A.npkts, CK_DEC_PKT, pi, A.npkts);
        const u64 q = u64(pi) * 4;
        r0 = src[q];
        r1 = src[q + 1];
        r2 = src[q + 2];
        r3 = src[q + 3];
      }
    }
    pre = false;
    pin_loaded(r0, r1, r2, r3);
#if LKF_SVC_STATS
    {
      u64 tl0;
      const u32 dep = __builtin_amdgcn_readfirstlane(r0.x ^ r3.w);
      asm volatile("s_memtime %0\n s_waitcnt lgkmcnt(0)" : "=s"(tl0) : "s"(dep));
      tLoad += tl0 - tc0;
    }
#endif
    const PktV p = decode_pkt(r0, r1, r2, r3);
    u32 pos = 0;
    u32 own = n;
    while (pos < n) {
      if (nextAt <= rl32(pi, pos)) {
        while (nextAt <= rl32(pi, pos)) {
          apply_ctl(L, A.events[ev++]);
          nextAt = ev < evEnd ? A.events[ev].at : 0xffffffffu;
        }
        vm_drain();
      }
      u32 x;
      bool gapStop = false;
      if (DDK && svcDT) {
#if LKF_SVC_STATS
        const u64 tr0 = __builtin_amdgcn_s_memtime();
#endif
        x = svc_run<DDK>(L, o, p, pi, n, pos, nextAt, valid, sentAcc, sSvcScr, sSvcFD);
        pos = x;
#if LKF_SVC_STATS
        const u64 tr1 = __builtin_amdgcn_s_memtime();
        tRun += tr1 - tr0;
#endif
        if (x < n && rl32(pi, x) < nextAt) {
          const u32 px = rl32(pi, x);
          decide_step<DDK>(L, load_pkt(pkts + px), px, o);
          vm_drain();
          if (ddDT) dd_restage(L, sDD, sDDSRaw, lane);
#if LKF_SVC_STATS
          tStep += __builtin_amdgcn_s_memtime() - tr1;
#endif
#if LKF_SVC_STATS
          if (lane == 0) SVC_ADD(2, 1ull);
#endif
          pos = x + 1;
        }
        continue;
      } else {
      const bool inWin = valid && lane >= pos && pi < nextAt;
      const u32 fl = L.h.flags;
      const bool video = fl & F_VIDEO;
      const i32 layer = p.layer;
      const bool kf = p.flags & LKF_PKT_KEYFRAME;
      const bool pktMarker = p.hdr1 & 0x80;
      int cls;
      if (fl & (F_MUTED | F_PUBMUTED)) {
        cls = LKF_DROP_MUTED;
      } else if (!video) {
        cls = -1;
      } else if (L.h.tgtS == INVALID || L.h.tgtT == INVALID) {
        cls = LKF_DROP_PAUSED;
      } else if (!(fl & F_SIMULCAST)) {
        cls = (fl & (F_VP9 | F_DD)) ? -2 : LKF_DROP_NOT_SELECTED;
      } else {
        const bool willSwitch =
            kf && ((L.h.curS != L.h.tgtS && ((layer > L.h.curS && layer <= L.h.tgtS) ||
                                             (layer < L.h.curS && layer >= L.h.tgtS))) ||
                   (L.h.curS > L.h.maxS && layer <= L.h.maxS));
        if (willSwitch)
          cls = -2;
        else if (layer != L.h.curS)
          cls = LKF_DROP_NOT_SELECTED;
        else if ((fl & F_DEFICIENT) && L.h.tgtS < L.h.curS)
          cls = LKF_DROP_DOWNGRADE;
        else if ((fl & F_VP8) && (fl & F_TLS_VP8) && (p.flags & LKF_PKT_VP8))
          cls = -1;
        else
          cls = -2;
      }
      const bool cand = inWin && cls == -1;
      const bool candIn = cand;
      const u64 candM = __ballot(candIn);
      const int pc = prev_in(candM, lt);
      const int pcs = pc >= 0 ? pc : int(lane);
      const u64 pcEsn = sh64(p.esn, pcs);
      const u64 prevEsn = pc >= 0 ? pcEsn : L.h.extHighestIncomingSN;
      const u64 dEsn = p.esn - prevEsn;
      const bool gapLane = candIn && dEsn > 1 && dEsn < u64(L.seqSize) - 64 &&
                           p.plen != 0 && p.ssrc == L.h.lastSSRC;
      bool ok = candIn && (dEsn == 1 || gapLane) && p.plen != 0 && p.ssrc == L.h.lastSSRC;
      const bool gapLater = candIn && pc >= 0 && dEsn > 1 && dEsn < u64(L.seqSize) - 64 && p.plen != 0 &&
                            p.ssrc == L.h.lastSSRC;
      const bool M = p.vbits & LKF_VP8_M, I = p.vbits & LKF_VP8_I, T = p.vbits & LKF_VP8_T;
      const i32 np = M ? i32(p.pid & 0x7fff) : i32(p.pid & 0x7f);
      const i32 ext = np + L.h.wrTotalWrap;
      const i32 pcExt = i32(sh32(u32(ext), pcs));
      const bool pcM = sh32(u32(M), pcs) != 0;
      const i32 prevExt = pc >= 0 ? pcExt : L.h.wrMaxPictureId;
      const bool prevM = pc >= 0 ? pcM : ((fl & F_WR_MAX_MBIT) != 0);
      bool dropT = false;
      u64 tswM = 0;
      bool overT = false;
      if (video) {
        i32 mp = prevExt;
        if (mp > 0) mp = prevM ? (prevExt & 0x7fff) : (prevExt & 0x7f);
        const bool wrapBack = L.h.wrTotalWrap > 0 && (prevExt + (L.h.wrLastWrap >> 1)) < (np + L.h.wrTotalWrap);
        const bool wraps = np < mp && (mp - np) > (prevM ? (1 << 14) : (1 << 6));
        const i32 cT = L.h.curT, gT = L.h.tgtT;
        const bool tsw = cT != gT && T &&
                         (cT < gT ? (i32(p.tid) > cT && i32(p.tid) <= gT && (p.vbits & LKF_VP8_S) &&
                                     (p.vbits & LKF_VP8_Y))
                                  : pktMarker);
        overT = candIn && T && p.tid > u8(cT);
        bool exIn = false;
        for (u64 ge = __ballot(gapLane && overT); ge; ge &= ge - 1) {
          const u32 k = u32(__ffsll((long long)ge) - 1);
          exIn = exIn || (lane > k && ext == i32(rl32(u32(ext), k)));
        }
        dropT = overT && !gapLane && !exIn;
        if (__ballot(dropT) && L.h.exCount)
          dropT = dropT && !set_has(L.exKey, L.h.exHead, L.h.exCount, ext);
        if (tsw && cT < gT) dropT = false;
        const bool tswOk = tsw && !gapLane && !dropT;
        ok = ok && !wrapBack && !wraps && (!tsw || tswOk) && (!dropT || L.h.snOffset == L.h.rmOpenValue);
        tswM = __ballot(inWin && ok && tsw);
      }
      const u64 tdM = __ballot(ok && dropT);
      const u64 snOff = L.h.snOffset + u64(__popcll(tdM & lt));
      u64 osn = p.esn - snOff;
      const u64 ots = p.ets - L.h.tsOffset;
      const bool picDrop = ok && dropT && I && ext != prevExt;
      const i32 picOff = L.h.pictureIdOffset + i32(__popcll(__ballot(picDrop) & lt));
      const bool fwdIn = ok && !dropT;
      const i32 mext = ext - picOff;
      const u16 mpid = u16(mext & 0x7fff);
      const u8 mtl0 = u8(p.tl0 - L.h.tl0Off);
      const u8 mkey = u8((p.keyidx - L.h.keyIdxOff) & 0x1f);
      u64 cb = 0;
      int cbLen = 0;
      if (video) {
        const bool mM = mpid > 127;
        const int hs = int(p.vhs) + (mM == M ? 0 : (mM ? 1 : -1));
        cbLen = vp8_marshal(p.vfirst, I, mM, mpid, p.vbits & LKF_VP8_L, mtl0, T, p.tid, p.vbits & LKF_VP8_Y,
                            p.vbits & LKF_VP8_K, mkey, hs, cb);
      }
      const u64 fwC = __ballot(fwdIn);
      const int pf = prev_in(fwC, lt);
      const int pfs = pf >= 0 ? pf : int(lane);
      const u64 pfOsn = sh64(osn, pfs);
      const u64 prevOsn = pf >= 0 ? pfOsn : L.h.seqExtHighestSN;
      const u64 pfOts = sh64(ots, pfs);
      const u64 hiTS = pf >= 0 ? pfOts : L.h.seqExtHighestTS;
      bool fwd = fwdIn;
      const bool tsMono = ots >= hiTS;
      const bool seqOk = (fl & F_SEQ_INIT) && (fl & F_STATS_INIT) && cbLen >= 0 && tsMono &&
                         (osn == prevOsn + 1 || (gapLane && osn - prevOsn > 1 &&
                                                 osn - prevOsn < u64(L.seqSize) - 64)) &&
                         osn - L.h.seqExtHighestSN < u64(L.seqSize) - 64;
      const bool bad =
          inWin && ((cls == -2) || (cls == -1 && !ok) || (fwdIn && !seqOk));
      const u64 stopM = __ballot(bad || (valid && lane >= pos && !inWin));
      x = stopM ? u32(__ffsll((long long)stopM) - 1) : n;
      if (tswM & ~((1ull << pos) - 1)) x = min(x, u32(__ffsll((long long)(tswM & ~((1ull << pos) - 1))) - 1) + 1u);
      if (x > pos) {
        const u64 runM = (x >= 64 ? ~0ull : ((1ull << x) - 1)) & ~((1ull << pos) - 1);
        const bool inRun = (runM >> lane) & 1;
        const u64 tdR = tdM & runM;
        fwd = fwd && inRun;
        const u64 fwR = __ballot(fwd);
        const u64 fwInR = fwR;
        const u64 selR = tdR | fwInR;
        o.nTuples += x - pos;
        o.drops[LKF_DROP_MUTED] += u32(__popcll(__ballot(inRun && cls == LKF_DROP_MUTED)));
        o.drops[LKF_DROP_PAUSED] += u32(__popcll(__ballot(inRun && cls == LKF_DROP_PAUSED)));
        o.drops[LKF_DROP_NOT_SELECTED] += u32(__popcll(__ballot(inRun && cls == LKF_DROP_NOT_SELECTED)));
        o.drops[LKF_DROP_DOWNGRADE] += u32(__popcll(__ballot(inRun && cls == LKF_DROP_DOWNGRADE)));
        o.drops[LKF_DROP_TEMPORAL] += u32(__popcll(tdR));
        const u64 pdR = video ? __ballot(picDrop && inRun) : 0ull;
        const u64 gR = __ballot(gapLane && inRun);
        if (gR) {
          for (u64 m = gR | pdR; m; m &= m - 1) {
            const u32 b = u32(__ffsll((long long)m) - 1);
            const i32 eb = i32(rl32(u32(ext), b));
            if ((pdR >> b) & 1) {
              L.vcDirty = true;
              set_add(L.dropKey, L.h.dropHead, L.h.dropCount, eb, kDropKeep);
              continue;
            }
            if (video) {
              vp8_record_missing(L, i32(rl32(u32(prevExt), b)), eb, i32(rl32(u32(picOff), b)));
              if (rl32(u32(overT), b)) {
                L.vcDirty = true;
                set_add(L.exKey, L.h.exHead, L.h.exCount, eb, kExemptKeep);
              }
            }
            const u64 from = rl64(prevOsn, b), to = rl64(osn, b);
            const u32 n = u32(to - from - 1);
            u32 base = u32(L.h.seqHighSlot) + u32(from - L.h.seqExtHighestSN) + 1;
            for (u32 i = lane; i < n; i += 64) {
              u32 x2 = base + i;
              while (x2 >= L.seqSize) x2 -= L.seqSize;
              store_rec(L.seq + x2, SeqMeta{});
            }
          }
        }
        const int cc = p.hdr0 & 0xf;
        const bool playout = L.extPlayout && !(fl & F_PLAYOUT_ACKED);
        const int extBytes = (playout ? 4 : 0) + (L.extAbs ? 4 : 0) + (L.extTcc ? 3 : 0);
        const int extBlock = extBytes ? 4 + ((extBytes + 3) & ~3) : 0;
        const int hdrLen = 12 + 4 * cc + extBlock;
        const bool useCodec = video && cbLen > 0 && (p.flags & LKF_PKT_VP8);
        const int payLen = useCodec ? (cbLen + int(p.plen) - int(p.vhs)) : int(p.plen);
        const u32 outLen = fwd ? u32(hdrLen + payLen) : 0u;
        const u32 aligned = (outLen + 15) & ~15u;
        const u32 relEx = excl_scan_u32(aligned, lane);
        const bool marker = pktMarker;
        const u32 j = u32(__popcll(fwR & lt));
        fwd_base(o, fwR, osn, ots);
        if (fwd) {
#if LKF_CHECKED
          CHK(slot0 + o.nFwd + j < A.tupleCap, CK_DEC_TUPLE, slot0 + o.nFwd + j, A.tupleCap);
#endif
          store_fwd(o.outT + o.nFwd + j, o.outW + o.nFwd + j, o.bSN, o.bTS, osn, ots, pi, o.relOff + relEx, outLen,
                    ((p.flags & LKF_PKT_KEYFRAME) ? LKF_OUT_KEYFRAME : 0) | (marker ? LKF_OUT_MARKER : 0) |
                        (playout ? T_PLAYOUT : 0) | (useCodec ? T_CODEC : 0),
                    0u, useCodec ? vp8_aux(mpid, mtl0, mkey) : 0u);
          u32 slot = u32(L.h.seqHighSlot) + u32(osn - L.h.seqExtHighestSN);
          while (slot >= L.seqSize) slot -= L.seqSize;
          SeqMeta m = {};
          m.sourceSeqNo = u16(p.esn);
          m.targetSeqNo = u16(osn);
          m.timestamp = u32(ots);
          m.lastNack = u32(p.arr / 1000000LL - L.h.seqStartMs);
          m.marker = marker;
          m.layer = p.layer;
          m.codecLen = u8(video ? cbLen : 0);
#pragma unroll
          for (int i = 0; i < 8; i++) m.codec[i] = u8(cb >> (8 * i));
          CHK(slot < L.seqSize, CK_DEC_SEQ, slot, L.seqSize);
          store_rec(L.seq + slot, m);
        }
        if (fwd) ss_put(o.ssBuf + o.ssN + j, osn, ots, p.arr, p.poff, u32(payLen), marker, kf);
        o.ssN += u32(__popcll(fwR));
        const u32 sumLen = wave_sum_u32(outLen);
        sentAcc += fwd ? i32(p.poff) - hdrLen : 0;
        if (fwR) {
          o.nBytes += sumLen;
          o.nFwd += u32(__popcll(fwR));
        }
        if (fwInR) {
          const u32 lastF = 63 - __clzll(fwInR);
          u32 slot = u32(L.h.seqHighSlot) + u32(rl64(osn, lastF) - L.h.seqExtHighestSN);
          while (slot >= L.seqSize) slot -= L.seqSize;
          L.h.seqHighSlot = u16(slot);
          L.h.seqExtHighestSN = rl64(osn, lastF);
          L.h.seqExtHighestTS = rl64(ots, lastF);
          if (video) {
            L.h.extLastPictureId = i32(rl32(u32(mext), lastF));
            L.h.lastTl0 = u8(rl32(mtl0, lastF));
            L.h.lastKeyIdx = u8(rl32(mkey, lastF));
          }
        }
        if (selR) {
          const u32 lastSel = 63 - __clzll(selR);
          const u64 mk = __ballot(video && pktMarker);
          L.h.extHighestIncomingSN = rl64(p.esn, lastSel);
          const bool lastIsF = (fwInR >> lastSel) & 1;
          const u64 pfM = fwInR & ((1ull << lastSel) - 1);
          u64 sSN = L.h.extLastSN, sTS = L.h.extLastTS;
          bool sMk = fl & F_LAST_MARKER;
          if (pfM) {
            const u32 b = 63 - __clzll(pfM);
            sSN = rl64(osn, b);
            sTS = rl64(ots, b);
            sMk = (mk >> b) & 1;
          }
          if (lastIsF) {
            L.h.extSecondLastSN = sSN;
            L.h.extSecondLastTS = sTS;
            L.h.extLastSN = rl64(osn, lastSel);
            L.h.extLastTS = rl64(ots, lastSel);
            setf(L, F_SECOND_LAST_MARKER, sMk);
            setf(L, F_LAST_MARKER, (mk >> lastSel) & 1);
          } else {
            L.h.extSecondLastSN = L.h.extLastSN = sSN;
            L.h.extSecondLastTS = L.h.extLastTS = sTS;
            setf(L, F_SECOND_LAST_MARKER, sMk);
            setf(L, F_LAST_MARKER, sMk);
          }
          if (hasf(L, F_RTX_GATE) && (rl64(osn, lastSel) - L.h.extRtxGateSn) > 2000) setf(L, F_RTX_GATE, false);
          const u64 kfM = __ballot(((selR >> lane) & 1) && kf);
          if (kfM) {
            L.h.extRtxGateSn = rl64(osn, 63 - __clzll(kfM));
            setf(L, F_RTX_GATE, true);
          }
          if (video) {
            L.h.wrMaxPictureId = i32(rl32(u32(ext), lastSel));
            setf(L, F_WR_MAX_MBIT, rl32(u32(M), lastSel) != 0);
            u64 m = tdR;
            while (m) {
              const u32 b = u32(__ffsll((long long)m) - 1);
              const u64 after = fwInR & ~((2ull << b) - 1);
              const u32 nf = after ? u32(__ffsll((long long)after) - 1) : 64u;
              const u64 runD = tdR & (nf >= 64 ? ~0ull : ((1ull << nf) - 1)) & ~((1ull << b) - 1);
              const u64 s0 = rl64(p.esn, b);
              rm_exclude(L, s0, s0 + u64(__popcll(runD)));
              m &= ~runD;
            }
            if (tdR) L.h.snOffset = L.h.rmOpenValue;
            const u64 tswR = tswM & runM;
            if (tswR) {
              const u32 b = 63 - __clzll(tswR);
              const i32 nxt = L.h.curT < L.h.tgtT ? i32(rl32(u32(p.tid), b)) : L.h.tgtT;
              L.h.prevS = L.h.curS;
              L.h.prevT = L.h.curT;
              L.h.curT = nxt;
            }
            u64 pd = pdR;
            L.h.pictureIdOffset += i32(__popcll(pd));
            while (pd && !gR) {
              const u32 b = u32(__ffsll((long long)pd) - 1);
              L.vcDirty = true;
              set_add(L.dropKey, L.h.dropHead, L.h.dropCount, i32(rl32(u32(ext), b)), kDropKeep);
              pd &= pd - 1;
            }
          }
        }
        if (fwR) o.relOff += rl32(relEx + aligned, 63 - __clzll(fwR));
      }
      gapStop = x < n && rl32(u32(gapLater), x) != 0;
      }
      pos = x;
      if (x < n && rl32(pi, x) < nextAt && !gapStop) {
        const uint4 a0 = make_uint4(rl32(r0.x, x), rl32(r0.y, x), rl32(r0.z, x), rl32(r0.w, x));
        const uint4 a1 = make_uint4(rl32(r1.x, x), rl32(r1.y, x), rl32(r1.z, x), rl32(r1.w, x));
        const uint4 a2 = make_uint4(rl32(r2.x, x), rl32(r2.y, x), rl32(r2.z, x), rl32(r2.w, x));
        const uint4 a3 = make_uint4(rl32(r3.x, x), rl32(r3.y, x), rl32(r3.z, x), rl32(r3.w, x));
        const u32 px = rl32(pi, x);
        decide_step<DDK>(L, decode_pkt(a0, a1, a2, a3), px, o);
        vm_drain();
        if (DDK && ddDT) dd_restage(L, sDD, sDDSRaw, lane);
        pos = x + 1;
        if (steady && !steady_state(L)) {
          own = x + 1;
          lim = px + 1;
          break;
        }
      }
    }
    if (steady) {
      const u32 skipped = (lim - kpos) - own;
      o.nTuples += skipped;
      o.drops[LKF_DROP_NOT_SELECTED] += skipped;
    }
    if (o.ssN) {
      wave_lds_sync();
#if LKF_SVC_STATS
      const u64 ts0 = __builtin_amdgcn_s_memtime();
#endif
      ss_flush(sSS, o.ssRing, o.ssGap, sSsBuf, o.ssN, o.bSN, o.bTS);
#if LKF_SVC_STATS
      tSs += __builtin_amdgcn_s_memtime() - ts0;
#endif
      o.ssN = 0;
    }
    kpos = lim;
  }
#if LKF_SVC_STATS
  const u64 tP2 = __builtin_amdgcn_s_memtime();
#endif
  while (ev < evEnd) apply_ctl(L, A.events[ev++]);
  __syncthreads();
  {
    const u32 h1 = reinterpret_cast<const u32 *>(&sHot)[lane];
    if (h1 != sHot0[lane]) reinterpret_cast<u32 *>(A.hot + d)[lane] = h1;
  }
  if (o.nFwd && lane < sizeof(SenderStats) / 16)
    reinterpret_cast<uint4 *>(A.ss + d)[lane] = reinterpret_cast<const uint4 *>(&sSS)[lane];
  if (L.rmNew) {
    wave_lds_sync();
    const u32 nc = L.h.rmCount, nn = min(L.rmNew, nc);
    for (u32 i = lane; i < nn; i += 64) {
      const u32 idx = (u32(L.h.rmHead) + nc - nn + i) % kRangeCap;
      rmG[idx] = sRm[idx];
    }
  }
  if (ddDT) {
    wave_lds_sync();
    uint4 *g = reinterpret_cast<uint4 *>(A.ddState + d);
    const uint4 *l = reinterpret_cast<const uint4 *>(sDD);
    const u32 nDD = (kDDStateHead + u32(sDD->numChains) * kDDExpRow * 8) / 16;
    for (u32 i = lane; i < nDD; i += 64) g[i] = l[i];
  }
  if ((L.h.flags & F_VP8) && L.vcDirty) {
    if (lane < u32(kSetCap)) {
      L.vc->dropKey[lane] = sDrop[lane];
      L.vc->exKey[lane] = sEx[lane];
    }
    for (u32 i = lane; i < L.h.missCount; i += 64) {
      const u32 idx = (L.h.missHead + i) % kMissCap;
      L.vc->missKey[idx] = sMissKey[idx];
      L.vc->missVal[idx] = sMissVal[idx];
    }
  }
  const i32 sentRun = i32(wave_sum_u32(u32(sentAcc)));
  if (lane == 0) {
    A.fwdCnt[d] = u32(o.nFwd);
    A.fwdBytes[d] = o.relOff;
    if (o.nFwd) A.fbase[d] = FwdBase{o.bSN, o.bTS};
    if (o.nFwd) atomicAdd((unsigned long long *)&A.dtCum[d].packets, (unsigned long long)o.nFwd);
    const u64 nSent = o.nBytes + u64(i64(sentRun) + o.sentDiff);
    if (nSent) atomicAdd((unsigned long long *)&A.dtCum[d].bytes, (unsigned long long)nSent);
    A.dtCum[d].flags = L.h.flags;
    u64 *st = A.stats + size_t(1 + (w % kStatCopies)) * kStatWords;
    if (o.nTuples) atomicAdd((unsigned long long *)&st[0], (unsigned long long)o.nTuples);
    if (o.nFwd) atomicAdd((unsigned long long *)&st[1], (unsigned long long)o.nFwd);
    if (o.nBytes) atomicAdd((unsigned long long *)&st[2], (unsigned long long)o.nBytes);
#pragma unroll
    for (int i = 0; i < LKF_DROP_NREASONS; i++)
      if (o.drops[i]) atomicAdd((unsigned long long *)&st[4 + i], (unsigned long long)o.drops[i]);
  }
#if LKF_SVC_STATS
  if (DDK && lane == 0 && (L.h.flags & (F_DD | F_VP9))) {
    const u64 tP3 = __builtin_amdgcn_s_memtime();
    SVC_ADD(4, (unsigned long long)(tP1 - tP0));
    SVC_ADD(5, (unsigned long long)tRun);
    SVC_ADD(6, (unsigned long long)tStep);
    SVC_ADD(7, (unsigned long long)(tP2 - tP1 - tRun - tStep));
    SVC_ADD(8, (unsigned long long)(tP3 - tP2));
    SVC_ADD(9, 1ull);
  }
  if (!DDK && lane == 0) {
    const u64 tP3 = __builtin_amdgcn_s_memtime();
    SVC_ADD(32, (unsigned long long)(tPa - tP0));
    SVC_ADD(33, (unsigned long long)(tP1 - tPa));
    SVC_ADD(34, (unsigned long long)(tP2 - tP1));
    SVC_ADD(35, (unsigned long long)(tP3 - tP2));
    SVC_ADD(36, 1ull);
    SVC_ADD(37, (unsigned long long)(pe - pb));
    SVC_ADD(38, tLoad);
    SVC_ADD(39, tSs);
  }
#endif
  }
}

constexpr int EMIT_T = 64;
constexpr int EMIT_G = 64;
constexpr int PRE_MAX = 96;
constexpr int PRE_MAX_DD = 352;

#ifndef LKF_EMIT_U
#define LKF_EMIT_U 6
#endif
constexpr int EMIT_U = LKF_EMIT_U;

__device__ __forceinline__ u32 align_byte(u32 hi, u32 lo, u32 sh) {
  return __builtin_amdgcn_alignbyte(hi, lo, sh);
}
__device__ __forceinline__ uint4 keep_bytes(uint4 v, int kb) {
  const u32 bits = u32(kb < 0 ? 0 : kb > 16 ? 16 : kb) * 8;
  const u64 lo = bits >= 64 ? ~0ull : ((1ull << bits) - 1);
  const u64 hi = bits <= 64 ? 0ull : bits >= 128 ? ~0ull : ((1ull << (bits - 64)) - 1);
  v.x &= u32(lo);
  v.y &= u32(lo >> 32);
  v.z &= u32(hi);
  v.w &= u32(hi >> 32);
  return v;
}
struct __attribute__((aligned(4))) U4A {
  u32 x, y, z, w;
};
__device__ __forceinline__ uint4 window_of(const U4A &a, u32 b, u32 rb) {
  uint4 v;
  v.x = align_byte(a.y, a.x, rb);
  v.y = align_byte(a.z, a.y, rb);
  v.z = align_byte(a.w, a.z, rb);
  v.w = align_byte(b, a.w, rb);
  return v;
}
__device__ __forceinline__ uint4 load_window(const u8 *arena, u64 s) {
  const u8 *q = arena + (s & ~u64(3));
  return window_of(*reinterpret_cast<const U4A *>(q), *reinterpret_cast<const u32 *>(q + 16), u32(s & 3));
}
__device__ __forceinline__ void store16(u8 *p, uint4 v) {
  __builtin_nontemporal_store(v.x, reinterpret_cast<u32 *>(p));
  __builtin_nontemporal_store(v.y, reinterpret_cast<u32 *>(p) + 1);
  __builtin_nontemporal_store(v.z, reinterpret_cast<u32 *>(p) + 2);
  __builtin_nontemporal_store(v.w, reinterpret_cast<u32 *>(p) + 3);
}

struct EmitRec {
  u64 extSN, extTS;
  u64 outOff;
  u64 src;
  u32 d, ord;
  u32 pkt, len, flags, ddLen, aux;
  PktV p;
  DevDT dt;
};

__device__ __forceinline__ EmitRec emit_locate(const EmitArgs &A, u64 r, u32 pLo, u32 pHi) {
  EmitRec q;
  u32 lo = pLo, hi = pHi;
  while (hi - lo > 1) {
    const u32 mid = (lo + hi) >> 1;
    if (A.recBase[mid] <= r)
      lo = mid;
    else
      hi = mid;
  }
  CHK(lo < A.ndts, CK_EMIT_POS, lo, A.ndts);
  const u32 d = A.perm[lo];
  CHK(d < A.maxDts, CK_EMIT_DT, d, A.maxDts);
  CHK(A.slotBase[d] + (r - A.recBase[lo]) < A.tupleCap, CK_EMIT_TUPLE, A.slotBase[d] + (r - A.recBase[lo]),
      A.tupleCap);
  const FwdRec *rp = A.recs + (A.slotBase[d] + (r - A.recBase[lo]));
  const U4x8 ra = *reinterpret_cast<const U4x8 *>(rp);
  const uint2 rb = reinterpret_cast<const uint2 *>(rp)[2];
  const u32 tPkt = ra.z, tLen = rb.x & 0xffffu, tFlags = (rb.x >> 16) & 0xffu, tDDLen = rb.x >> 24, tAux = rb.y;
  CHK(tPkt < A.npkts, CK_EMIT_PKT, tPkt, A.npkts);
  q.p = load_pkt(A.pkts + tPkt);
  q.dt = A.dts[d];
  const FwdBase fb = A.fbase[d];
  q.outOff = A.byteBase[lo] + (u64(ra.w) << 4);
  CHK(r < A.outCap, CK_EMIT_OUT, r, A.outCap);
  CHK(q.outOff + tLen <= A.outByteCap, CK_EMIT_BYTES, q.outOff + tLen, A.outByteCap);
  CHK(u64(q.p.arenaOff) + q.p.poff + q.p.plen <= A.arenaLen, CK_EMIT_ARENA, u64(q.p.arenaOff) + q.p.poff + q.p.plen,
      A.arenaLen);
  CHK(!(tFlags & T_DD) || u64(tAux) + tDDLen <= A.ddCap, CK_EMIT_DD, u64(tAux) + tDDLen, A.ddCap);
  q.extSN = widen32(fb.sn, ra.x);
  q.extTS = widen32(fb.ts, ra.y);
  if (tFlags & T_WIDE) {
    const FwdBase wv = A.wide[A.slotBase[d] + (r - A.recBase[lo])];
    q.extSN = wv.sn;
    q.extTS = wv.ts;
  }
  q.d = d;
  q.ord = u32(r - A.recBase[lo]);
  q.pkt = tPkt;
  q.len = tLen;
  q.flags = tFlags;
  q.ddLen = tDDLen;
  q.aux = tAux;
  q.src = u64(q.p.arenaOff) + q.p.poff + ((tFlags & T_CODEC) ? u32(q.p.vhs) : 0u);
  return q;
}

template <int PRE, bool WRITE>
__device__ __forceinline__ int emit_marshal(const EmitArgs &A, const EmitRec &q, u8 *w) {
  const PktV &p = q.p;
  const DevDT &dt = q.dt;
  const u32 tFlags = q.flags, tAux = q.aux;
  const int tDDLen = int(q.ddLen);
  auto put = [&](int i, u8 v) {
    if (WRITE) w[i] = v;
  };
  const int cc = p.hdr0 & 0xf;
  const bool playout = tFlags & T_PLAYOUT;
  const bool ddOn = (PRE == PRE_MAX_DD) && (tFlags & T_DD);
  const bool hasExt = playout || dt.extAbs || ddOn || dt.extTcc;
  const u16 tcc = dt.extTcc ? u16(A.twccBase[q.d] + q.ord) : u16(0);
  put(0, u8((p.hdr0 & 0xe0) | (hasExt ? 0x10 : 0) | cc));
  put(1, u8(((tFlags & LKF_OUT_MARKER) ? 0x80 : 0) | (dt.pt & 0x7f)));
  const u16 sn = u16(q.extSN);
  const u32 ts = u32(q.extTS);
  put(2, u8(sn >> 8));
  put(3, u8(sn));
  put(4, u8(ts >> 24));
  put(5, u8(ts >> 16));
  put(6, u8(ts >> 8));
  put(7, u8(ts));
  put(8, u8(dt.ssrc >> 24));
  put(9, u8(dt.ssrc >> 16));
  put(10, u8(dt.ssrc >> 8));
  put(11, u8(dt.ssrc));
  int n = 12;
  if (WRITE) {
    const u8 *raw = A.arena + p.arenaOff;
    for (int i = 0; i < 4 * cc; i++) w[n + i] = raw[12 + i];
  }
  n += 4 * cc;
  if (hasExt && !(ddOn && tDDLen > 16)) {
    const int eb = (ddOn ? 1 + tDDLen : 0) + (playout ? 4 : 0) + (dt.extAbs ? 4 : 0) + (dt.extTcc ? 3 : 0);
    const int words = (eb + 3) >> 2;
    put(n++, 0xBE);
    put(n++, 0xDE);
    put(n++, u8(words >> 8));
    put(n++, u8(words));
    if (ddOn) {
      put(n++, u8((dt.extDD << 4) | (tDDLen - 1)));
      if (WRITE)
        for (int i = 0; i < tDDLen; i++) w[n + i] = A.ddArena[tAux + i];
      n += tDDLen;
    }
    if (playout) {
      put(n++, u8((dt.extPlayout << 4) | 2));
      put(n++, dt.playout[0]);
      put(n++, dt.playout[1]);
      put(n++, dt.playout[2]);
    }
    if (dt.extAbs) {
      put(n++, u8((dt.extAbs << 4) | 2));
      put(n++, 0);
      put(n++, 0);
      put(n++, 0);
    }
    if (dt.extTcc) {
      put(n++, u8((dt.extTcc << 4) | 1));
      put(n++, u8(tcc >> 8));
      put(n++, u8(tcc));
    }
    for (int i = eb; i < 4 * words; i++) put(n++, 0);
  } else if (hasExt) {
    const int eb = 2 + tDDLen + (playout ? 5 : 0) + (dt.extAbs ? 5 : 0) + (dt.extTcc ? 4 : 0);
    const int words = (eb + 3) >> 2;
    put(n++, 0x10);
    put(n++, 0x00);
    put(n++, u8(words >> 8));
    put(n++, u8(words));
    put(n++, dt.extDD);
    put(n++, u8(tDDLen));
    if (WRITE)
      for (int i = 0; i < tDDLen; i++) w[n + i] = A.ddArena[tAux + i];
    n += tDDLen;
    if (playout) {
      put(n++, dt.extPlayout);
      put(n++, 3);
      put(n++, dt.playout[0]);
      put(n++, dt.playout[1]);
      put(n++, dt.playout[2]);
    }
    if (dt.extAbs) {
      put(n++, dt.extAbs);
      put(n++, 3);
      put(n++, 0);
      put(n++, 0);
      put(n++, 0);
    }
    if (dt.extTcc) {
      put(n++, dt.extTcc);
      put(n++, 2);
      put(n++, u8(tcc >> 8));
      put(n++, u8(tcc));
    }
    for (int i = eb; i < 4 * words; i++) put(n++, 0);
  }
  if (tFlags & T_CODEC) {
    const u16 mpid = u16(tAux & 0xffffu);
    const bool mM = mpid > 127, M = p.vbits & LKF_VP8_M;
    const int hs = int(p.vhs) + (mM == M ? 0 : (mM ? 1 : -1));
    u64 cb = 0;
    const int cl = vp8_marshal(p.vfirst, p.vbits & LKF_VP8_I, mM, mpid, p.vbits & LKF_VP8_L, u8(tAux >> 16),
                               p.vbits & LKF_VP8_T, p.tid, p.vbits & LKF_VP8_Y, p.vbits & LKF_VP8_K,
                               u8(tAux >> 24), hs, cb);
#pragma unroll
    for (int i = 0; i < 6; i++)
      if (i < cl) put(n + i, u8(cb >> (8 * i)));
    n += cl > 0 ? cl : 0;
  }
  return n;
}

#ifndef LKF_EMIT_XCD
#define LKF_EMIT_XCD 1
#endif
template <int PRE>
__global__ void __launch_bounds__(EMIT_T) k_emit(EmitArgs A) {
  __shared__ __attribute__((aligned(16))) u8 pre[EMIT_G][PRE];
  __shared__ u64 sSrc[EMIT_G];
  __shared__ u32 sCs[EMIT_G];
  __shared__ u32 sLen[EMIT_G];
  __shared__ u32 sPre[EMIT_G];
  const u32 lane = threadIdx.x;
  const u64 total = A.totals[0];
  const u64 ngroups = (total + EMIT_G - 1) / EMIT_G;
  if (total > A.outCap || A.totals[1] > A.outByteCap) {
    if (blockIdx.x == 0 && lane == 0) atomicOr(A.err, 4u);
    return;
  }
  const u32 nx = (LKF_EMIT_XCD && gridDim.x % 8 == 0) ? 8u : 1u;
  const u32 xcd = blockIdx.x % nx, slotInX = blockIdx.x / nx, perX = gridDim.x / nx;
  const u64 gpx = (ngroups + nx - 1) / nx;
  const u64 gBeg = u64(xcd) * gpx, gEnd = min(ngroups, gBeg + gpx);
  for (u64 g = gBeg + slotInX; g < gEnd; g += perX) {
    const u64 r0 = g * EMIT_G;
    const u32 nrec = u32(min(u64(EMIT_G), total - r0));
    CHK(g + 1 < A.gCap, CK_EMIT_GROUP, g + 1, A.gCap);
    const u32 pLo = A.gFirst[g];
    const u32 pHi = (g + 1 < ngroups) ? A.gFirst[g + 1] + 1 : A.ndts;
    u64 outOff = 0;
    if (lane < nrec) {
      const EmitRec q = emit_locate(A, r0 + lane, pLo, pHi);
      const u32 tLen = q.len;
      outOff = q.outOff;
      lkf_out o;
      o.ext_sn = q.extSN;
      o.ext_ts = q.extTS;
      o.out_off = outOff;
      o.dt = q.d;
      o.pkt = q.pkt;
      o.out_len = u16(tLen);
      o.flags = u8(q.flags & 0x0f);
      o.layer = q.p.layer;
      o.reserved = 0;
      A.out[r0 + lane] = o;
      u8 *w = pre[lane];
      const int n = emit_marshal<PRE, true>(A, q, w);
      const u64 src = q.src;
      const int R = (n + 15) & ~15;
      if (R > n) {
        const uint4 v = load_window(A.arena, src);
        const u32 vw[4] = {v.x, v.y, v.z, v.w};
        for (int i = n; i < R; i++) {
          const int b = i - n;
          w[i] = (i < int(tLen)) ? u8(vw[b >> 2] >> (8 * (b & 3))) : 0;
        }
      }
      sSrc[lane] = src;
      sLen[lane] = tLen;
      sPre[lane] = u32(n) | (u32(R) << 16);
    }
    const u64 gByte = rl64(outOff, 0);
// ... 1194 lines not shown
```

### livekit-server_amd/csrc/ingress_kernels.hip

```cpp
#include <cstdlib>
#include <vector>
#include <algorithm>
#include <hip/hip_runtime.h>

#include "../../include/lkfwd.h"
#include "dd_device.h"
#include "fwd_state.h"
#include "kernels.h"

namespace lkf {

using u8 = uint8_t;
using u16 = uint16_t;
using u32 = uint32_t;
using u64 = uint64_t;
using i16 = int16_t;
using i32 = int32_t;
using i64 = int64_t;

typedef const __attribute__((address_space(3))) u8 *LdsBytes;
struct StagedBytes {
  LdsBytes lds;
  const u8 *g;
  int n;
// ... 531 lines not shown
    h.rmCount++;
  } else {
    ring[h.rmHead] = c;
    h.rmHead = u16((h.rmHead + 1) % kRangeCap);
  }
  h.rmOpenStart = e;
  h.rmOpenValue = nv;
  return true;
}
__device__ __forceinline__ bool irm_get(const StreamHot &h, const RangeEntry *ring, u64 key, u64 &out) {
  out = 0;
  if (key >= h.rmOpenStart) {
    out = h.rmOpenValue;
    return true;
  }
  const int nc = h.rmCount;
  const u64 firstStart = nc > 0 ? ring[h.rmHead].start : h.rmOpenStart;
  if (key < firstStart) return false;
  RangeEntry next;
  next.start = h.rmOpenStart;
  next.end = 0;
  next.value = h.rmOpenValue;
  const u64 half = 1ull << 63;
  for (int idx = nc; idx >= 0; idx--) {
    if (idx != nc) {
      const RangeEntry rv = next;
      if ((key - rv.start) < half && (rv.end - key) < half) {
        out = rv.value;
        return true;
      }
    }
    if (idx > 0) {
      const RangeEntry prev = ring[(h.rmHead + idx - 1) % kRangeCap];
      const u64 before = key - prev.end, after = next.start - key;
      if (before > 0 && before < half && after > 0 && after < half) return false;
      next = prev;
    }
  }
  return false;
}

__device__ __noinline__ double level_smooth(double prev, u32 activeDuration, u8 loudest, u32 observeDuration,
                                            double smoothFactor) {
  const double activityWeight = 20.0 * log10(double(activeDuration) / double(observeDuration));
  const double adjusted = double(loudest) - activityWeight;
  const double linear = pow(10.0, adjusted * (-1.0 / 20));
  return prev + (linear - prev) * smoothFactor;
}
__device__ __forceinline__ void level_observe(StreamHot &h, const DevStream &s, u8 level, u32 durationMs, i64 arrivalNs) {
  h.lastObservedNs = arrivalNs;
  h.observedDuration += durationMs;
  if (level <= s.activeLevel) {
    h.activeDuration += durationMs;
    if (h.loudest > level) h.loudest = level;
  }
  if (h.observedDuration >= s.observeDuration) {
    h.smoothedLevel = h.activeDuration >= s.minActiveDuration
                          ? level_smooth(h.smoothedLevel, h.activeDuration, h.loudest, s.observeDuration, s.smoothFactor)
                          : 0.0;
    h.loudest = 127;
    h.activeDuration = 0;
    h.observedDuration = 0;
  }
}

__device__ __forceinline__ void level_step(StreamHot &h, const DevStream &s, u32 pflags, u32 ts, u8 level,
                                           i64 arrival) {
  if (!(h.flags & S_LVL_TS_INIT)) {
    h.flags |= S_LVL_TS_INIT;
    h.latestTSForAudioLevel = ts;
  }
  if (pflags & IP_LEVEL) {
    if (u32(ts - h.latestTSForAudioLevel) < (1u << 31)) {
      const i64 dur = (i64(ts) - i64(h.latestTSForAudioLevel)) * 1000 / i64(s.clockRate);
      if (dur > 0) level_observe(h, s, level, u32(dur), arrival);
      h.latestTSForAudioLevel = ts;
    }
  }
}

__global__ void __launch_bounds__(64) k_ing_lists(const lkf_raw_pkt *__restrict__ raws,
                                                  const DevStream *__restrict__ streams, u32 nstreams,
                                                  const u32 *__restrict__ tBegin, const u32 *__restrict__ tEnd,
                                                  u32 stride, u32 *__restrict__ list, u32 *__restrict__ cnt) {
  const u32 t = blockIdx.x, lane = threadIdx.x;
  const u64 lt = (1ull << lane) - 1;
  const u32 b = tBegin[t], e = tEnd[t];
  u32 c[3] = {0, 0, 0};
  for (u32 base = b; base < e; base += 64) {
    const u32 i = base + lane;
    int l = -1;
    if (i < e) {
      const u32 sid = raws[i].stream;
      if (sid < nstreams) l = int(streams[sid].layer);
      if (l > 2) l = -1;
    }
#pragma unroll
    for (int k = 0; k < 3; k++) {
      const u64 m = __ballot(l == k);
      if (l == k) list[size_t(k) * stride + b + c[k] + u32(__popcll(m & lt))] = i;
      c[k] += u32(__popcll(m));
    }
  }
  if (lane == 0)
    for (int k = 0; k < 3; k++) cnt[t * 3 + k] = c[k];
}

__device__ inline u64 wa16_ext(u64 &cycles, u64 &extHighest, u16 &start, u16 &highest, u32 &flags, u32 initBit,
                               u16 val) {
  const u64 full = 1ull << 16;
  if (!(flags & initBit)) {
    start = val;
    highest = val;
    extHighest = cycles + u64(val);
    flags |= initBit;
    return u64(val);
  }
  const u16 gap = u16(val - highest);
  if (gap > u16(full >> 1)) {
    u64 cyc = cycles;
    const u64 total = extHighest - u64(start) + 1;
    const bool wrapBack = u64(highest) < (full >> 1) && u64(val) >= (full >> 1);
    if (total > (full >> 1)) {
      if (wrapBack) cyc -= full;
      return cyc + u64(val);
    }
    if (!(u16(val - start) > u16(full >> 1)) && wrapBack) cyc -= full;
    return cyc + u64(val);
  }
  if (val < highest) cycles += full;
  highest = val;
  extHighest = cycles + u64(val);
  return extHighest;
}

__device__ inline void ph_set(DDIngState &d, u64 seq, bool r) {
  const u64 i = (seq - d.phBase) % u64(kFICPktWords * 64);
  if (r)
    d.phBits[i >> 6] |= 1ull << (i & 63);
  else
    d.phBits[i >> 6] &= ~(1ull << (i & 63));
}
__device__ inline void ph_add(DDIngState &d, u64 seq) {
  if (!(d.flags & DI_PH_INIT)) {
    d.flags |= DI_PH_INIT;
    d.phBase = seq > 100 ? seq - 100 : 0;
    d.phLast = seq;
    ph_set(d, seq, true);
    return;
  }
  if (seq <= d.phBase) return;
  if (seq <= d.phLast) {
    if (d.phLast - seq < u64(kFICPktWords * 64)) ph_set(d, seq, true);
    return;
  }
  if (seq - d.phLast - 1 >= u64(kFICPktWords * 64)) {
    for (int w = 0; w < kFICPktWords; w++) d.phBits[w] = 0;
  } else {
    for (u64 i = d.phLast + 1; i < seq; i++) ph_set(d, i, false);
  }
  ph_set(d, seq, true);
  d.phLast = seq;
}
__device__ inline bool ph_consecutive(const DDIngState &d, u64 start, u64 end) {
  const u64 pc = u64(kFICPktWords * 64);
  if (start > end || end - start >= pc) return false;
  const u64 si = (start - d.phBase) % pc, ei = (end - d.phBase) % pc;
  const int sIdx = int(si >> 6), sOff = int(si & 63), eIdx = int(ei >> 6), eOff = int(ei & 63);
  if (sIdx == eIdx && end - start <= 64) {
    const int w = eOff - sOff + 1;
    const u64 tb = (w >= 64 ? ~0ull : ((1ull << w) - 1)) << sOff;
    return (d.phBits[sIdx] & tb) == tb;
  }
  const u64 lhs = (d.phBits[sIdx] >> sOff) + 1;
  const u64 rhs = (64 - sOff) >= 64 ? 0 : (1ull << (64 - sOff));
  if (lhs != rhs) return false;
  for (int i = sIdx + 1; i != eIdx; i++) {
    if (i == kFICPktWords) {
      i = 0;
      if (i == eIdx) break;
    }
    if (d.phBits[i] + 1 != 0) return false;
  }
  const u64 tb = eOff + 1 >= 64 ? ~0ull : ((1ull << (eOff + 1)) - 1);
  return (d.phBits[eIdx] & tb) == tb;
}
__device__ inline void fe_add(DDIngState &d, int slot, u64 seq, bool first, bool last) {
  u8 f = d.feFlags[slot];
  if (f & 4) return;
  if (!(f & 1) && first) {
    f |= 1;
    d.feStart[slot] = seq;
  }
  if (!(f & 2) && last) {
    f |= 2;
    d.feEnd[slot] = seq;
  }
  if ((f & 3) == 3 && ph_consecutive(d, d.feStart[slot], d.feEnd[slot])) f |= 4;
  d.feFlags[slot] = f;
}
__device__ inline void fc_add(DDIngState &d, u64 seq, u64 fn, bool first, bool last) {
  ph_add(d, seq);
  if (!(d.flags & DI_FC_INIT)) {
    d.flags |= DI_FC_INIT;
    d.fcBase = d.fcLast = fn;
  }
  if (fn < d.fcBase) return;
  if (fn <= d.fcLast) {
    if (d.fcLast - fn >= u64(kFICFrames)) return;
    fe_add(d, int((fn - d.fcBase) % u64(kFICFrames)), seq, first, last);
    return;
  }
  if (fn - d.fcLast >= u64(kFICFrames)) {
    for (int i = 0; i < kFICFrames; i++) d.feFlags[i] = 0;
  } else {
    for (u64 i = d.fcLast + 1; i <= fn; i++) d.feFlags[int((i - d.fcBase) % u64(kFICFrames))] = 0;
  }
  fe_add(d, int((fn - d.fcBase) % u64(kFICFrames)), seq, first, last);
  d.fcLast = fn;
}
__device__ inline bool fc_integrity(const DDIngState &d, u64 fn) {
  if (fn < d.fcBase || fn > d.fcLast || d.fcLast - fn >= u64(kFICFrames)) return false;
  return (d.feFlags[int((fn - d.fcBase) % u64(kFICFrames))] & 4) != 0;
}

struct DDLite {
  u16 frameNumber;
  u8 flags, sid, tid;
  u32 activeMask;
  int err;
};
__device__ bool dd_fold(DDIngState &d, u16 sn, const DDLite &o, bool att, IngDD &out) {
  const u64 extSeq = wa16_ext(d.seqCycles, d.seqExtHighest, d.seqStart, d.seqHighest, d.flags, DI_SEQ_INIT, sn);
  const u64 extFN = wa16_ext(d.fnCycles, d.fnExtHighest, d.fnStart, d.fnHighest, d.flags, DI_FN_INIT, o.frameNumber);
  if (extFN < d.structureExtFN) return false;
  fc_add(d, extSeq, extFN, o.flags & DP_FIRST, o.flags & DP_LAST);
  out.extFN = extFN;
  out.flags = fc_integrity(d, extFN) ? LKF_DD_INTEGRITY : 0;
  if (att) {
    if (!(o.flags & DP_FIRST)) return false;
    d.flags ^= DI_CUR;
    d.flags |= DI_HAS_STRUCT;
    d.structureExtFN = extFN;
    out.flags |= LKF_DD_STRUCTURE_UPDATED | LKF_DD_ACTIVE_UPDATED;
  }
  if ((o.flags & DP_ACTIVE) && extSeq > d.activeExtSeq) {
    d.activeExtSeq = extSeq;
    if (o.activeMask != d.activeMask) {
      d.activeMask = o.activeMask;
      out.flags |= LKF_DD_ACTIVE_UPDATED;
    }
  }
  out.extKFN = d.structureExtFN;
  out.present = 1;
  out.sid = o.sid;
  out.tid = o.tid;
  return true;
}

__device__ __noinline__ DDLite dd_parse_lite(const u8 *buf, int len, const DDStruct *cur) {
  DDPkt o = {};
  bool att = false;
  DDLite out;
  out.err = dd::dd_parse(buf, len, cur, nullptr, o, att);
  out.frameNumber = o.frameNumber;
  out.flags = o.flags;
  out.sid = o.sid;
  out.tid = o.tid;
  out.activeMask = o.activeMask;
  return out;
}
__device__ __forceinline__ bool dd_attaches(const u8 *buf, int len) { return len > 3 && (buf[3] & 0x80); }

__device__ __noinline__ bool dd_ingest(DDIngState &d, DDStruct *structs, const u8 *buf, int len, u16 sn, IngDD &out,
                                       bool &limit) {
  limit = false;
  const u32 cur = (d.flags & DI_CUR) ? 1u : 0u;
  DDPkt o = {};
  bool att = false;
  const int e = dd::dd_parse(buf, len, (d.flags & DI_HAS_STRUCT) ? structs + cur : nullptr, structs + (cur ^ 1u), o,
                             att);
  if (e) {
    limit = e == dd::LIMIT;
    return false;
  }
  DDLite l;
  l.frameNumber = o.frameNumber;
  l.flags = o.flags;
  l.sid = o.sid;
  l.tid = o.tid;
  l.activeMask = o.activeMask;
  return dd_fold(d, sn, l, att, out);
}

constexpr int kBktLds = 2048;
constexpr u32 kNoOwner = 0xFFFFFFFFu;
struct BktCtx {
  BucketState *b;
  u32 *tag;
  u64 *owner;
  u64 *store;
  u32 *sOwn;
  u64 ep;
  bool lds;
};
__device__ __forceinline__ int bkt_wrap(int x, int M) {
  x %= M;
  return x < 0 ? x + M : x;
}
__device__ __forceinline__ void bkt_supersede(const BktCtx &k, int sl, u32 ic) {
  if (k.lds) {
    const u32 o = k.sOwn[sl];
    if (o != kNoOwner) k.store[o] = 0;
    k.sOwn[sl] = ic;
  } else {
    const u64 o = k.owner[sl];
    if ((o & 0xFFFFFFFF00000000ull) == k.ep) k.store[u32(o)] = 0;
    k.owner[sl] = ic == kNoOwner ? 0 : (k.ep | ic);
  }
}
__device__ int bkt_add_one(const BktCtx &k, u16 sn, u32 len, u32 ic) {
  BucketState &b = *k.b;
  const int M = int(b.maxSteps);
  int slot = -1;
  if (len <= 1498) {
    if (!b.init) {
      b.head = u16(sn - 1);
      b.init = 1;
    }
    const u16 diff = u16(sn - b.head);
    if (diff == 0 || diff > (1u << 15)) {
      const int back = int(u16(b.head - sn));
      if (back < M) {
        const int sl = bkt_wrap(int(b.step) - back - 1, M);
        const u32 t = k.tag[sl];
        if (!((t >> 16) != 0xFFFFu && u16(t) == sn)) slot = sl;
      }
    } else {
      const int gap = int(diff) - 1;
      b.head = sn;
      for (int i = 0; i < min(gap, M); i++) {
        const int sl = bkt_wrap(int(b.step) + i, M);
        k.tag[sl] = 0xFFFF0000u;
        bkt_supersede(k, sl, kNoOwner);
      }
      slot = bkt_wrap(int(b.step) + gap, M);
      b.step = u32(bkt_wrap(int(b.step) + gap + 1, M));
    }
  }
  if (slot >= 0) {
    k.tag[slot] = (len << 16) | sn;
    bkt_supersede(k, slot, ic);
    k.store[ic] = (1ull << 63) | (u64(sn) << 32) | u64(b.base + u32(slot));
  }
  return slot;
}

__device__ __forceinline__ void rx_gap(u32 *gap, u64 g) {
  if (g < 2) return;
  const u64 missing = g - 1;
  atomicAdd(&gap[missing > u64(kGapBins) ? kGapBins - 1 : u32(missing - 1)], 1u);
}
__device__ __forceinline__ u64 rx_transit(const StreamHot &h, u32 clockRate, u64 ets, i64 t) {
  const i64 since = i64(u64(t) - u64(h.firstTime));
  return u64(i64(u64(since) * u64(i64(clockRate))) / 1000000000LL) - ets;
}
__device__ __forceinline__ void rx_jitter_fold(StreamHot &h, u64 transit, u64 ets) {
  if (h.lastTransit != 0) {
    i64 d = i64(transit - h.lastTransit);
    if (d < 0) d = i64(0 - u64(d));
    h.jitter += (double(d) - h.jitter) / 16;
    if (h.jitter > h.maxJitter) h.maxJitter = h.jitter;
  }
  h.lastTransit = transit;
  h.lastJitterExtTs = ets;
}
__device__ __forceinline__ void rx_jitter(StreamHot &h, u32 clockRate, u64 ets, i64 t) {
  if (h.lastJitterExtTs == ets) return;
  rx_jitter_fold(h, rx_transit(h, clockRate, ets, t), ets);
}

template <int HS>
__device__ __noinline__ lkf_flow ing_step(StreamHot &h, u64 *hs, RangeEntry *ring, const DevStream *sg,
                                         const IngParsed *pg, const lkf_raw_pkt *rg, u32 ic, lkf_flow *flows,
                                         u32 *fwd, IngDD *ingDD, const u8 *raw, DDIngState *dds,
                                         DDStruct *ddStructs, u32 *err, const BktCtx *bkg, bool bkOn, u32 *gap) {
  const DevStream s = *sg;
  const IngParsed p = *pg;
  const lkf_raw_pkt rp = *rg;
  const BktCtx bk = *bkg;
  const i64 arrival = rp.arrival_ns;
  lkf_flow f = {};
  f.pkt = 0xffffffffu;
  u32 forward = 0;
  IngDD dv = {};
  do {
    if (!(p.flags & IP_OK)) {
      f.flags = LKF_FLOW_BAD;
      break;
    }
    if (s.levelExt) level_step(h, s, p.flags, p.ts, p.level, arrival);
    const int hdrSize = p.hdrSize, payloadSize = p.payloadLen, paddingSize = p.paddingSize;
    WAResult rsn, rts;
    if (!(h.flags & S_INIT)) {
      if (payloadSize == 0) {
        f.flags = LKF_FLOW_NOT_HANDLED;
        break;
      }
      h.flags |= S_INIT;
      h.firstTime = arrival;
      h.highestTime = arrival;
      rsn = wa16_update(h, p.sn);
      rts = wa32_update(h, p.ts);
    } else {
      rsn = wa16_update(h, p.sn);
      if (rsn.unhandled) {
        f.flags = LKF_FLOW_NOT_HANDLED;
        break;
      }
      rts = wa32_update(h, p.ts);
    }
    const u64 pktSize = u64(hdrSize + payloadSize + paddingSize);
    const i64 gapSN = i64(rsn.extVal - rsn.preHighest);
    bool dup = false, ooo = false;
    if (gapSN <= 0) {
      if (gapSN != 0) h.packetsOutOfOrder++;
      const i64 diff = i64(rsn.preHighest - rsn.extVal);
      if (diff >= 0 && diff < i64(kHistWords) * 64) {
        if (hist_isset<HS>(hs, rsn.extVal)) {
          h.bytesDuplicate += pktSize;
          h.headerBytesDuplicate += u64(hdrSize);
          h.packetsDuplicate++;
          dup = true;
        } else {
          h.packetsLost--;
          hist_set<HS>(hs, rsn.extVal);
        }
      }
      ooo = true;
    } else {
      rx_gap(gap, u64(gapSN));
      hist_clear_range<HS>(hs, rsn.preHighest + 1, rsn.extVal - 1);
      h.packetsLost += u64(gapSN - 1);
      hist_set<HS>(hs, rsn.extVal);
      if (p.ts != u32(rts.preHighest)) h.highestTime = arrival;
      if (gapSN > 1) {
        f.flags |= LKF_FLOW_HAS_LOSS;
        f.loss_start = rsn.preHighest + 1;
        f.loss_end = rsn.extVal;
      }
    }
    f.ext_sn = rsn.extVal;
    f.ext_ts = rts.extVal;
    if (!dup) {
      if (payloadSize == 0) {
        h.packetsPadding++;
        h.bytesPadding += pktSize;
        h.headerBytesPadding += u64(hdrSize);
      } else {
        h.bytes += pktSize;
        h.headerBytes += u64(hdrSize);
        if (p.flags & IP_MARKER) h.frames++;
        rx_jitter(h, s.clockRate, rts.extVal, arrival);
      }
    }
    if (dup) f.flags |= LKF_FLOW_DUPLICATE;
    if (ooo) f.flags |= LKF_FLOW_OUT_OF_ORDER;
    if (payloadSize == 0 && (!ooo || dup)) {
      if (!ooo) irm_exclude(h, ring, rsn.extVal, rsn.extVal + 1);
      f.flags |= LKF_FLOW_PADDING;
      break;
    }
    u64 adj = 0;
    if (!irm_get(h, ring, rsn.extVal, adj)) {
      f.flags |= LKF_FLOW_BAD;
      break;
    }
    f.ext_sn = rsn.extVal - adj;
    if (dup) break;
    if (bkOn && bkt_add_one(bk, u16(f.ext_sn), rp.len, ic) < 0) break;
    f.flags |= LKF_FLOW_BUCKET;
    if (payloadSize > 0 && s.ddIdx != 0xffffffffu && p.ddLen) {
      bool limit = false;
      if (!dd_ingest(*dds, ddStructs + size_t(s.ddIdx) * 2, raw + rp.off + p.ddOff, p.ddLen,
                     u16(f.ext_sn), dv, limit)) {
        if (limit) atomicOr(err, 4u);
        f.flags |= LKF_FLOW_BAD;
        break;
      }
      dv.ddOff = p.ddOff;
      dv.ddLen = p.ddLen;
    }
    if ((p.flags & IP_VP8_BAD) && !(s.codec == LKF_CODEC_VP9 && dv.present)) {
      f.flags |= LKF_FLOW_BAD;
      break;
    }
    forward = 1;
    f.flags |= LKF_FLOW_FORWARD;
  } while (false);
  flows[ic] = f;
  fwd[ic] = forward;
  if (ingDD) ingDD[ic] = dv;
  return f;
}

__device__ void closed_flows(const DevStream &s, u32 sid, u32 pb, u32 pe, const lkf_raw_pkt *raws, lkf_flow *flows,
                             u32 *fwd, IngDD *ingDD, const u32 *list, const u32 *cnt, u32 stride, u32 first,
                             u32 step, NackIn *nackIn) {
  const bool useList = s.layer < 3;
  const u32 nIdx = useList ? cnt[s.track * 3 + s.layer] : pe - pb;
  const u32 *lst = list + size_t(useList ? s.layer : 0) * stride + pb;
  for (u32 k = first; k < nIdx; k += step) {
    const u32 ic = useList ? lst[k] : pb + k;
    if (raws[ic].stream != sid) continue;
    lkf_flow f = {};
    f.pkt = 0xffffffffu;
    f.flags = LKF_FLOW_NOT_HANDLED;
    flows[ic] = f;
    fwd[ic] = 0;
    if (ingDD) ingDD[ic] = IngDD{};
    if (nackIn && useList) nackIn[size_t(lst - list) + k] = NackIn{raws[ic].arrival_ns, sid, 0u, 0u, 0u};
  }
}

__device__ __forceinline__ u64 rl_u64(u64 v, u32 x) {
  return (u64(u32(__builtin_amdgcn_readlane(int(u32(v >> 32)), x))) << 32) |
         u64(u32(__builtin_amdgcn_readlane(int(u32(v)), x)));
}
__device__ __forceinline__ u64 wave_incl_scan_u64(u64 v, u32 lane) {
#pragma unroll
  for (int d = 1; d < 64; d <<= 1) {
    const u64 o = __shfl_up(v, d, 64);
    if (lane >= u32(d)) v += o;
  }
  return v;
}
__device__ __forceinline__ u64 wave_sum_u64(u64 v) {
#pragma unroll
  for (int d = 32; d >= 1; d >>= 1) v += __shfl_xor(v, d, 64);
  return v;
}

__device__ __forceinline__ u32 nk_snfl(const IngParsed &p, const lkf_flow &f) {
  const bool ok = (p.flags & IP_OK) != 0;
  return u32(p.sn) | ((ok ? 2u : 0u) | (ok && (f.flags & LKF_FLOW_HAS_LOSS) ? 4u : 0u)) << 16;
}

#ifndef LKF_ING_PER_WAVE
#define LKF_ING_PER_WAVE 0
#endif
#ifndef LKF_ING_WAVES
#define LKF_ING_WAVES 3
#endif
template <bool DDK>
__global__ void __launch_bounds__(64) __attribute__((amdgpu_waves_per_eu(LKF_ING_WAVES))) k_ing_stream_wave(
    const lkf_raw_pkt *__restrict__ raws, const IngParsed *__restrict__ q, const DevStream *__restrict__ streams,
    StreamHot *__restrict__ hot, u64 *__restrict__ hist, RangeEntry *__restrict__ rings,
    const u32 *__restrict__ tBegin, const u32 *__restrict__ tEnd, lkf_flow *__restrict__ flows,
    u32 *__restrict__ fwd, const u8 *__restrict__ raw, DDIngState *ddStates, DDStruct *ddStructs,
    IngDD *__restrict__ ingDD, u32 *err, const u32 *__restrict__ list, const u32 *__restrict__ cnt, u32 stride,
    BktArgs bka, u32 *__restrict__ rxGap, NackIn *__restrict__ nackIn, u32 nstreams, u32 perWave) {
  static_assert(kHistWords == 64, "one history word per lane");
  static_assert(sizeof(StreamHot) == 64 * sizeof(u32), "one StreamHot dword per lane");
  __shared__ u64 sHist[kHistWords];
  __shared__ StreamHot sh;
  __shared__ BucketState sB;
  __shared__ u32 sOwn[kBktLds];
  __shared__ __attribute__((aligned(16))) u8 sDDIRaw[DDK ? sizeof(DDIngState) : 16];
  __shared__ BktCtx sBk;
  const u32 lane = threadIdx.x;
  for (u32 jw = 0; jw < perWave; jw++) {
  const u32 sid = blockIdx.x * perWave + jw;
  if (sid >= nstreams) break;
  if (jw) __syncthreads();
  const DevStream s = streams[sid];
  if ((s.ddIdx != 0xffffffffu) != DDK) continue;
  const u32 pb = tBegin[s.track], pe = tEnd[s.track];
  if (pb >= pe) continue;
  if (s.closed) {
    closed_flows(s, sid, pb, pe, raws, flows, fwd, ingDD, list, cnt, stride, lane, 64, nackIn);
    continue;
  }
  u64 *const hg = hist + size_t(sid) * kHistWords;
  u32 *const gap = rxGap + size_t(sid) * kGapWords;
  const u64 hist0 = hg[lane];
  const u32 hot0 = reinterpret_cast<const u32 *>(hot + sid)[lane];
  sHist[lane] = hist0;
  reinterpret_cast<u32 *>(&sh)[lane] = hot0;
  const bool bkOn = bka.state != nullptr;
  BktCtx bk = {};
  int M = 1;
  if (bkOn) {
    if (lane < 4) reinterpret_cast<u32 *>(&sB)[lane] = reinterpret_cast<const u32 *>(bka.state + sid)[lane];
    __syncthreads();
    M = int(sB.maxSteps);
    bk.b = &sB;
    bk.tag = bka.tag + sB.base;
    bk.owner = bka.owner + sB.base;
    bk.store = bka.store;
    bk.sOwn = sOwn;
    bk.ep = u64(bka.epoch) << 32;
    bk.lds = M <= kBktLds;
    if (bk.lds)
      for (int i = int(lane); i < M; i += 64) sOwn[i] = kNoOwner;
  }
  if (lane == 0) sBk = bk;
  DDIngState *dds = nullptr;
  if (DDK) {
    dds = reinterpret_cast<DDIngState *>(sDDIRaw);
    const uint4 *g = reinterpret_cast<const uint4 *>(ddStates + s.ddIdx);
    uint4 *l = reinterpret_cast<uint4 *>(sDDIRaw);
    for (u32 i = lane; i < sizeof(DDIngState) / 16; i += 64) l[i] = g[i];
  }
  __syncthreads();
  RangeEntry *ring = rings + size_t(sid) * kRangeCap;
  const bool useList = s.layer < 3;
  const u32 nIdx = useList ? cnt[s.track * 3 + s.layer] : pe - pb;
  const u32 *lst = list + size_t(useList ? s.layer : 0) * stride + pb;
  const bool runStream = true;
  const bool hasDD = s.ddIdx != 0xffffffffu;
  for (u32 j = 0; runStream && j < nIdx; j += 64) {
    const u32 k = j + lane;
    const bool in = k < nIdx;
    u32 ic = 0;
    IngParsed p = {};
    lkf_raw_pkt rp = {};
    if (in) {
      ic = useList ? lst[k] : pb + k;
      p = q[ic];
      rp = raws[ic];
    }
    const u32 m = min(64u, nIdx - j);
    u32 nkSnFl = 0, nkS0 = 0, nkLen = 0;
    for (u32 pos = 0; pos < m;) {
    const u32 need = S_INIT | S_SN_INIT | S_TS_INIT;
    const bool stateOk = runStream && (sh.flags & need) == need && sh.rmOpenStart <= sh.snExtHighest + 1;
    const u16 prevSn = u16(__shfl_up(u32(p.sn), 1, 64));
    const u32 prevTs = u32(__shfl_up(p.ts, 1, 64));
    const u16 gs = u16(p.sn - (lane == pos ? sh.snHighest : prevSn));
    const u32 gt = p.ts - (lane == pos ? sh.tsHighest : prevTs);
    const bool ddLane = hasDD && p.ddLen;
    const bool ok = lane >= pos && stateOk && in && rp.stream == sid && (p.flags & IP_OK) && p.payloadLen > 0 &&
                    !(p.flags & IP_VP8_BAD) && !(ddLane && dd_attaches(raw + rp.off + p.ddOff, p.ddLen)) &&
                    gs >= 1 && gs <= 0x8000u && gt <= 0x80000000u && (!bkOn || rp.len <= 1498u);
    const u64 snScan = wave_incl_scan_u64(ok ? u64(gs) : 0, lane);
    u64 bad = ~__ballot(ok) & ~((1ull << pos) - 1);
    bad |= __ballot(lane >= pos && snScan >= u64(kHistWords) * 64);
    u64 bS = 0;
    u32 d0 = 0;
    if (bkOn) {
      const u32 gs0 = __builtin_amdgcn_readlane(u32(gs), pos);
      d0 = u32(u16(u16(sh.snExtHighest + gs0 - sh.rmOpenValue) - sB.head));
      if (!sB.init || d0 < 1 || d0 > 0x8000u) bad |= 1ull << pos;
      bS = snScan - gs0 + d0;
      bad |= __ballot(lane >= pos && bS > u64(M));
    }
    const u32 end = bad ? u32(__ffsll(static_cast<long long>(bad)) - 1) : 64u;
    if (end == pos) {
      if (lane == pos && rp.stream == sid) {
        const lkf_flow fo = ing_step<1>(sh, sHist, ring, streams + sid, q + ic, raws + ic, ic, flows, fwd, ingDD, raw,
                                        dds, ddStructs, err, &sBk, bkOn, gap);
        nkSnFl = nk_snfl(p, fo);
        nkS0 = u32(u16(fo.loss_start));
        nkLen = u32(min<u64>(fo.loss_end - fo.loss_start, 0xffffffffull));
      }
      __syncthreads();
      pos++;
      continue;
    }
    const u32 L = end - pos;
    const bool run = lane >= pos && lane < end;
    const u64 tsScan = wave_incl_scan_u64(run ? u64(gt) : 0, lane);
    const u64 ext = sh.snExtHighest + snScan, extTs = sh.tsExtHighest + tsScan;
    const u64 pktSize = u64(p.hdrSize + p.payloadLen + p.paddingSize);
    const u64 bytesRun = wave_sum_u64(run ? pktSize : 0), hdrRun = wave_sum_u64(run ? u64(p.hdrSize) : 0);
    const u32 framesRun = u32(__popcll(__ballot(run && (p.flags & IP_MARKER))));
    const u64 extLast = __shfl(ext, int(end - 1), 64), extTsLast = __shfl(extTs, int(end - 1), 64);
    const u16 snLast = u16(__shfl(u32(p.sn), int(end - 1), 64));
    const u32 tsLast = u32(__shfl(p.ts, int(end - 1), 64));
    const u64 bSLast = __shfl(bS, int(end - 1), 64);
    const u64 newTs = __ballot(run && p.ts != (lane == pos ? sh.tsHighest : prevTs));
    const u64 prevExtTs = __shfl_up(extTs, 1, 64);
    const u64 newJ = __ballot(run && extTs != (lane == pos ? sh.lastJitterExtTs : prevExtTs));
    const u64 transit = rx_transit(sh, s.clockRate, extTs, rp.arrival_ns);
    if (run) rx_gap(gap, u64(gs));
    u64 ddFail = 0;
    const u64 ddM = __ballot(run && ddLane);
    if (ddM) {
      DDIngState &dst = *dds;
      const u32 dfl = dst.flags;
      const DDStruct *curS = (dfl & DI_HAS_STRUCT) ? ddStructs + size_t(s.ddIdx) * 2 + ((dfl & DI_CUR) ? 1 : 0) : nullptr;
      DDLite dl = {};
      if (run && ddLane) dl = dd_parse_lite(raw + rp.off + p.ddOff, p.ddLen, curS);
      const int de = dl.err;
      const u32 dlw0 = u32(dl.frameNumber) | (u32(dl.flags) << 16) | (u32(dl.sid & 15) << 24) | (u32(dl.tid & 15) << 28);
      const u16 snL = u16(ext - sh.rmOpenValue);
      for (u64 w = ddM; w; w &= w - 1) {
        const u32 x = u32(__ffsll(static_cast<long long>(w)) - 1);
        const int ex = __builtin_amdgcn_readlane(de, x);
        const u32 icx = u32(__builtin_amdgcn_readlane(int(ic), x));
        const u32 w0 = u32(__builtin_amdgcn_readlane(int(dlw0), x));
        const u32 amx = u32(__builtin_amdgcn_readlane(int(dl.activeMask), x));
        const u16 snx = u16(__builtin_amdgcn_readlane(int(snL), x));
        const u32 offx = u32(__builtin_amdgcn_readlane(int(p.ddOff), x));
        const u32 lenx = u32(__builtin_amdgcn_readlane(int(p.ddLen), x));
        if (lane == 0) {
          IngDD dv = {};
          bool okx = false;
          if (ex) {
            if (ex == dd::LIMIT) atomicOr(err, 4u);
          } else {
            DDLite o;
            o.frameNumber = u16(w0);
            o.flags = u8(w0 >> 16);
            o.sid = u8((w0 >> 24) & 15);
            o.tid = u8(w0 >> 28);
            o.activeMask = amx;
            okx = dd_fold(dst, snx, o, false, dv);
            if (okx) {
              dv.ddOff = u16(offx);
              dv.ddLen = u8(lenx);
            }
          }
          if (ingDD) ingDD[icx] = dv;
          if (!okx) ddFail |= 1ull << x;
        }
      }
      ddFail = rl_u64(ddFail, 0);
    }
    if (run) {
      lkf_flow f = {};
      f.pkt = 0xffffffffu;
      f.ext_sn = ext - sh.rmOpenValue;
      f.ext_ts = extTs;
      f.flags = LKF_FLOW_FORWARD | LKF_FLOW_BUCKET;
      if (gs > 1) {
        f.flags |= LKF_FLOW_HAS_LOSS;
        f.loss_start = ext - gs + 1;
        f.loss_end = ext;
      }
      const bool failed = (ddFail >> lane) & 1;
      if (failed) f.flags = u8((f.flags & ~LKF_FLOW_FORWARD) | LKF_FLOW_BAD);
      flows[ic] = f;
      nkSnFl = nk_snfl(p, f);
      nkS0 = u32(u16(f.loss_start));
      nkLen = u32(min<u64>(f.loss_end - f.loss_start, 0xffffffffull));
      fwd[ic] = failed ? 0u : 1u;
      if (ingDD && !ddLane) ingDD[ic] = IngDD{};
      if (bkOn) {
        const u32 dk = lane == pos ? d0 : u32(gs);
        const int step0 = int(sB.step);
        const int first = int(bS - dk);
        for (u32 i = 0; i + 1 < dk; i++) {
          const int sl = bkt_wrap(step0 + first + int(i), M);
          bk.tag[sl] = 0xFFFF0000u;
          bkt_supersede(bk, sl, kNoOwner);
        }
        const int slot = bkt_wrap(step0 + int(bS) - 1, M);
        const u16 sn = u16(f.ext_sn);
        bk.tag[slot] = (rp.len << 16) | sn;
        bkt_supersede(bk, slot, ic);
        bk.store[ic] = (1ull << 63) | (u64(sn) << 32) | u64(sB.base + u32(slot));
      }
    }
    const u64 pre0 = sh.snExtHighest;
    const u64 adjLast = extLast - sh.rmOpenValue;
    if (s.levelExt) {
      StreamHot lh;
      lh.flags = sh.flags;
      lh.latestTSForAudioLevel = sh.latestTSForAudioLevel;
      lh.lastObservedNs = sh.lastObservedNs;
      lh.observedDuration = sh.observedDuration;
      lh.activeDuration = sh.activeDuration;
      lh.loudest = sh.loudest;
      lh.smoothedLevel = sh.smoothedLevel;
      for (u32 x = pos; x < end; x++)
        level_step(lh, s, __builtin_amdgcn_readlane(u32(p.flags), x), __builtin_amdgcn_readlane(p.ts, x),
                   u8(__builtin_amdgcn_readlane(u32(p.level), x)), i64(rl_u64(u64(rp.arrival_ns), x)));
      __syncthreads();
      if (lane == 0) {
        sh.flags |= lh.flags & S_LVL_TS_INIT;
        sh.latestTSForAudioLevel = lh.latestTSForAudioLevel;
        sh.lastObservedNs = lh.lastObservedNs;
        sh.observedDuration = lh.observedDuration;
        sh.activeDuration = lh.activeDuration;
        sh.loudest = lh.loudest;
        sh.smoothedLevel = lh.smoothedLevel;
      }
    }
    __syncthreads();
    if (lane == 0) {
      hist_clear_range<1>(sHist, pre0 + 1, extLast);
      sh.packetsLost += extLast - pre0 - L;
      sh.bytes += bytesRun;
      sh.headerBytes += hdrRun;
      sh.frames += framesRun;
      sh.snHighest = snLast;
      sh.snExtHighest = extLast;
      sh.snCycles = extLast - snLast;
      sh.tsHighest = tsLast;
      sh.tsExtHighest = extTsLast;
      sh.tsCycles = extTsLast - tsLast;
      if (bkOn) {
        sB.head = u16(adjLast);
        sB.step = u32(bkt_wrap(int(sB.step) + int(bSLast), M));
      }
    }
    if (newTs) {
      const int kl = 63 - __clzll(static_cast<long long>(newTs));
      const i64 tl = i64(rl_u64(u64(rp.arrival_ns), u32(kl)));
      if (lane == 0) sh.highestTime = tl;
    }
    if (newJ) {
      StreamHot jh;
      jh.lastTransit = sh.lastTransit;
      jh.jitter = sh.jitter;
      jh.maxJitter = sh.maxJitter;
      jh.lastJitterExtTs = sh.lastJitterExtTs;
      for (u64 w = newJ; w; w &= w - 1) {
        const u32 k = u32(__ffsll(static_cast<long long>(w)) - 1);
        rx_jitter_fold(jh, rl_u64(transit, k), rl_u64(extTs, k));
      }
      if (lane == 0) {
        sh.lastTransit = jh.lastTransit;
        sh.jitter = jh.jitter;
        sh.maxJitter = jh.maxJitter;
        sh.lastJitterExtTs = jh.lastJitterExtTs;
      }
    }
    __syncthreads();
    if (run) atomicOr(reinterpret_cast<unsigned long long *>(&sHist[(ext >> 6) & (kHistWords - 1)]), 1ull << (ext & 63));
    __syncthreads();
    pos = end;
    }
    if (nackIn && useList && in && rp.stream == sid)
      nackIn[size_t(lst - list) + k] = NackIn{rp.arrival_ns, sid, nkSnFl, nkS0, nkLen};
  }
  if (sHist[lane] != hist0) hg[lane] = sHist[lane];
  const u32 hot1 = reinterpret_cast<const u32 *>(&sh)[lane];
  if (hot1 != hot0) reinterpret_cast<u32 *>(hot + sid)[lane] = hot1;
  if (bkOn && lane < 4) reinterpret_cast<u32 *>(bka.state + sid)[lane] = reinterpret_cast<const u32 *>(&sB)[lane];
  if (DDK) {
    __syncthreads();
    uint4 *g = reinterpret_cast<uint4 *>(ddStates + s.ddIdx);
    const uint4 *l = reinterpret_cast<const uint4 *>(sDDIRaw);
    for (u32 i = lane; i < sizeof(DDIngState) / 16; i += 64) g[i] = l[i];
  }
  }
}


#ifndef LKF_NACK_FAST_MIN
#define LKF_NACK_FAST_MIN 16
#endif
#ifndef LKF_NACK_N
#define LKF_NACK_N 512
#endif
constexpr u32 kNackFastN = LKF_NACK_N;
constexpr u32 kNackFastEv = kNackFastPairs;
constexpr u32 kNackNone = 0xffffffffu;
constexpr u32 kNackHash = 256;
struct NackFastLds {
  i64 arr[kNackFastN];
  u16 sn[kNackFastN];
  u16 nextMine[kNackFastN + 1];
  u8 fl[kNackFastN];
  i64 eLast[kNackSlots];
  u32 eRem[kNackSlots];
  u16 eDeath[kNackSlots];
  int16_t eBirth[kNackSlots];
  u16 eSn[kNackSlots];
  u8 eTries[kNackSlots];
  u16 pushK[kNackCap], pushOff[kNackCap + 1];
  u16 pushS0[kNackCap];
  u16 key[kNackFastEv];
  u8 hash[256];
  u16 gStart[kNackFastEv + 1];
  u16 gNp[kNackFastEv], gOff[kNackFastEv];
  lkf_nack_pair stage[kNackFastEv];
  u32 nEv;
};
static_assert(kNackSlots <= 128 && kNackFastN <= 512 && kNackFastEv / kNackMaxTries < 127,
              "16-bit event keys: 9 bits of datagram, 7 of entry, below the 0xffff pad");

#ifndef LKF_NACK_DBG
#define LKF_NACK_DBG 0
#endif
#define NF_DECLINE(code)                                                                                 \
  do {                                                                                                   \
    if (LKF_NACK_DBG == 1 && lane == 0) printf("nack serial sid=%u why=%d nIdx=%u count0=%u\n", sid, code, nIdx, count0); \
    return false;                                                                                        \
  } while (0)
#if LKF_NACK_DBG == 2
constexpr u32 kNackStampCap = 1u << 16;
__device__ u64 gNackStamp[size_t(kNackStampCap) * 7];
#else
constexpr u32 kNackStampCap = 0;
__device__ u64 *const gNackStamp = nullptr;
#endif
__device__ __forceinline__ u64 *nack_stamp(u32 lane, u32 sid, u64 tEntry) {
  if (LKF_NACK_DBG != 2 || sid >= kNackStampCap) return nullptr;
  u64 *r = gNackStamp + size_t(sid) * 7;
  if (lane == 0) r[1] = tEntry;
  return r;
}
__device__ bool nack_fast(NackFastLds &F, u32 lane, u32 sid, NackState *g, u32 count0, u32 rtt, u32 nIdx,
                          const u32 *lst, bool useList, u32 pb, const NackIn *__restrict__ nk,
                          const lkf_raw_pkt *__restrict__ raws, const IngParsed *__restrict__ q,
                          const lkf_flow *__restrict__ flows, u32 *__restrict__ info,
                          u32 *__restrict__ pairOff, u32 *pairCnt, lkf_nack_pair *__restrict__ pairs, u32 pairCap,
                          u32 *err, u64 *stamp) {
#define NF_STAMP(w)                                                    \
  do {                                                                 \
    if (LKF_NACK_DBG == 2 && lane == 0 && stamp) stamp[w] = wall_clock64(); \
  } while (0)
  if (nIdx < LKF_NACK_FAST_MIN || nIdx > kNackFastN || count0 * kNackMaxTries > kNackFastEv) NF_DECLINE(1);
  static_assert(kNackFastEv / kNackMaxTries <= 64, "one queued entry per lane");
  u32 q0sn = 0, q0tries = 0;
  i64 q0last = 0;
  if (lane < count0) {
    q0sn = g->sn[lane];
    q0tries = g->tries[lane];
    q0last = g->last[lane];
  }
  u64 lossTot = 0;
  u32 nPush = 0;
  bool mono = true;
  i64 prevArr = INT64_MIN;
  constexpr u32 kCh = kNackFastN / 64;
  u32 stv[kCh], sfv[kCh];
  i64 arv[kCh];
  u64 s0v[kCh], lnv[kCh];
  if (nk) {
#pragma unroll
    for (u32 c = 0; c < kCh; c++) {
      const u32 k = c * 64 + lane;
      stv[c] = 0xffffffffu;
      arv[c] = 0;
      sfv[c] = 0;
      s0v[c] = lnv[c] = 0;
      if (k < nIdx) {
        const NackIn r = nk[k];
        stv[c] = r.stream;
        arv[c] = r.arrival;
        sfv[c] = r.snFl;
        s0v[c] = r.s0;
        lnv[c] = r.len;
      }
    }
  } else {
    u32 icv[kCh], ffv[kCh];
#pragma unroll
    for (u32 c = 0; c < kCh; c++) {
      const u32 k = c * 64 + lane;
      icv[c] = k < nIdx ? (useList ? lst[k] : pb + k) : 0u;
    }
#pragma unroll
    for (u32 c = 0; c < kCh; c++) {
      stv[c] = 0xffffffffu;
      arv[c] = 0;
      sfv[c] = 0;
      ffv[c] = 0;
      if (c * 64 + lane < nIdx) {
        stv[c] = raws[icv[c]].stream;
// ... 1263 lines not shown
```

Baseline: 1.505 billion forwarded RTP pkts/s.

## Cut register pressure in decide kernel and specialize non-DD ingest step

Kernel arguments in k_decide_dt are now read through the kernarg segment pointer instead of a by-value struct, and the packet decode is re-materialized per iteration behind an asm barrier. The aim is lower SGPR/VGPR pressure and fewer spills. Sender-stats entries now carry a wide-record flag and index, so ss_flush can reload full 64-bit SN/TS from the wide array, which adds a threadfence. lane_id uses inline asm, BktCtx's bool becomes padded u32, and the non-DD ingest path gets an inlined template specialization that skips dd_ingest and zero-fills IngDD.

```diff
diff --git a/livekit-server_amd/csrc/forward_kernels.hip b/livekit-server_amd/csrc/forward_kernels.hip
--- a/livekit-server_amd/csrc/forward_kernels.hip
+++ b/livekit-server_amd/csrc/forward_kernels.hip
@@ -118,7 +118,11 @@
   return v;
 }
 
-__device__ __forceinline__ u32 lane_id() { return threadIdx.x & 63u; }
+__device__ __forceinline__ u32 lane_id() {
+  u32 l;
+  asm volatile("v_and_b32 %0, 63, %1" : "=v"(l) : "v"(threadIdx.x));
+  return l;
+}
 __device__ __forceinline__ u32 rl32(u32 v, u32 l) { return __builtin_amdgcn_readlane(v, l); }
 __device__ __forceinline__ u64 rl64(u64 v, u32 l) {
   return (u64(rl32(u32(v >> 32), l)) << 32) | u64(rl32(u32(v), l));
@@ -1041,9 +1045,12 @@
 struct __attribute__((aligned(8))) U4x8 {
   u32 x, y, z, w;
 };
+__device__ __forceinline__ bool wide_rec(u64 bSN, u64 bTS, u64 sn, u64 ts) {
+  return (((sn - bSN) + 0x80000000ull) >> 32) != 0 || (((ts - bTS) + 0x80000000ull) >> 32) != 0;
+}
 __device__ __forceinline__ void store_fwd(FwdRec *dst, FwdBase *wdst, u64 bSN, u64 bTS, u64 sn, u64 ts, u32 pkt,
                                           u32 relOff, u32 outLen, u32 flags, u32 ddLen, u32 aux) {
-  if ((((sn - bSN) + 0x80000000ull) >> 32) != 0 || (((ts - bTS) + 0x80000000ull) >> 32) != 0) {
+  if (wide_rec(bSN, bTS, sn, ts)) {
     flags |= T_WIDE;
     *wdst = FwdBase{sn, ts};
   }
@@ -1543,22 +1550,33 @@
   u32 fl;
 };
 static_assert(sizeof(SsEnt) == 24, "SsEnt is 24 B");
-__device__ __forceinline__ void ss_put(SsEnt *e, u64 sn, u64 ts, i64 t, u32 hdr, u32 pay, bool marker, bool kf) {
+__device__ __forceinline__ void ss_put(SsEnt *e, const LaneOut &o, u32 rel, u64 sn, u64 ts, i64 t, u32 hdr, u32 pay,
+                                       bool marker, bool kf) {
+  const u32 wide = wide_rec(o.bSN, o.bTS, sn, ts) ? 4u | (rel << 3) : 0u;
   *reinterpret_cast<uint2 *>(e) = make_uint2(u32(sn), u32(ts));
   reinterpret_cast<uint2 *>(e)[1] = make_uint2(u32(u64(t)), u32(u64(t) >> 32));
-  reinterpret_cast<uint2 *>(e)[2] = make_uint2(hdr | (pay << 16), (marker ? 1u : 0u) | (kf ? 2u : 0u));
+  reinterpret_cast<uint2 *>(e)[2] = make_uint2(hdr | (pay << 16), (marker ? 1u : 0u) | (kf ? 2u : 0u) | wide);
+}
+__device__ __forceinline__ void ss_wide(const FwdBase *wide, u32 fl, u64 &esn, u64 &ets) {
+  const FwdBase w = wide[fl >> 3];
+  esn = w.sn;
+  ets = w.ts;
 }
 
 #ifndef LKF_SS_SCALAR
 #define LKF_SS_SCALAR 0
 #endif
 __device__ __forceinline__ void ss_flush(SenderStats &S, u32 *ring, u32 *gap, const SsEnt *buf, u32 m, u64 bSN,
-                                      u64 bTS) {
+                                      u64 bTS, const FwdBase *wide) {
   if (m <= u32(LKF_SS_SCALAR)) {
     for (u32 i = 0; i < m; i++) {
       const SsEnt &e = buf[i];
-      ss::ss_update(S, ring, gap, e.t, widen32(bSN, e.sn), widen32(bTS, e.ts), (e.fl & 1) != 0, e.hp & 0xffffu,
-                    e.hp >> 16, 0);
+      u64 esn = widen32(bSN, e.sn), ets = widen32(bTS, e.ts);
+      if (e.fl & 4) {
+        __threadfence();
+        ss_wide(wide, e.fl, esn, ets);
+      }
+      ss::ss_update(S, ring, gap, e.t, esn, ets, (e.fl & 1) != 0, e.hp & 0xffffu, e.hp >> 16, 0);
       if (e.fl & 2) S.keyFrames++;
       wave_lds_sync();
     }
@@ -1571,6 +1589,7 @@
   i64 t = 0;
   u32 hdr = 0, pay = 0;
   bool marker = false, kf = false;
+  u32 efl = 0;
   if (valid) {
     const SsEnt &e = buf[lane];
     esn = widen32(bSN, e.sn);
@@ -1578,8 +1597,13 @@
     t = e.t;
     hdr = e.hp & 0xffffu;
     pay = e.hp >> 16;
-    marker = e.fl & 1;
-    kf = e.fl & 2;
+    efl = e.fl;
+    marker = efl & 1;
+    kf = efl & 2;
+  }
+  if (__ballot(efl & 4)) {
+    __threadfence();
+    if (efl & 4) ss_wide(wide, efl, esn, ets);
   }
   const u64 pEsn = sh64(esn, lane ? int(lane) - 1 : 0), pEts = sh64(ets, lane ? int(lane) - 1 : 0);
   u32 pos = 0;
@@ -1807,7 +1831,8 @@
     L.h.statsExtStartTS = f.ots;
   }
   if (lane_id() == 0)
-    ss_put(o.ssBuf + o.ssN, f.osn, f.ots, p.arr, p.poff, u32(payLen), marker, (p.flags & LKF_PKT_KEYFRAME) != 0);
+    ss_put(o.ssBuf + o.ssN, o, u32(o.nFwd), f.osn, f.ots, p.arr, p.poff, u32(payLen), marker,
+           (p.flags & LKF_PKT_KEYFRAME) != 0);
   o.ssN++;
   o.nFwd++;
   o.nBytes += u64(hdrLen + payLen);
@@ -1831,6 +1856,11 @@
 __device__ __forceinline__ void pin_loaded(const uint4 &a, const uint4 &b, const uint4 &c, const uint4 &d) {
   asm volatile("" ::"v"(a.x), "v"(a.y), "v"(a.z), "v"(a.w), "v"(b.x), "v"(b.y), "v"(b.z), "v"(b.w), "v"(c.x),
                "v"(c.y), "v"(c.z), "v"(c.w), "v"(d.x), "v"(d.y), "v"(d.z), "v"(d.w));
+}
+
+__device__ __forceinline__ void relaunder(uint4 &a, uint4 &b, uint4 &c, uint4 &d) {
+  asm volatile("" : "+v"(a.x), "+v"(a.y), "+v"(a.z), "+v"(a.w), "+v"(b.x), "+v"(b.y), "+v"(b.z), "+v"(b.w),
+                 "+v"(c.x), "+v"(c.y), "+v"(c.z), "+v"(c.w), "+v"(d.x), "+v"(d.y), "+v"(d.z), "+v"(d.w));
 }
 
 __device__ __forceinline__ bool steady_state(const Lane &L) {
@@ -2347,7 +2377,7 @@
       store_rec(L.seq + x2, SeqMeta{});
     }
   }
-  if (f) ss_put(o.ssBuf + o.ssN + j, osn, ots, p.arr, p.poff, p.plen, mk, kf);
+  if (f) ss_put(o.ssBuf + o.ssN + j, o, u32(o.nFwd) + j, osn, ots, p.arr, p.poff, p.plen, mk, kf);
   o.ssN += u32(__popcll(fwR));
   const u32 sumLen = wave_sum_u32(outLen);
   sentAcc += f ? i32(p.poff) - hdrLen : 0;
@@ -2439,12 +2469,20 @@
   if (LKF_DD_RESTAGE && moved) dd_stage_struct(L, sDD, sDDSRaw, lane);
 }
 
+typedef const DecideArgs __attribute__((address_space(4))) *DecideArgsK;
+__device__ __forceinline__ DecideArgsK decide_args() {
+  DecideArgsK k = (DecideArgsK)__builtin_amdgcn_kernarg_segment_ptr();
+  asm volatile("" : "+s"(k));
+  return k;
+}
+
 constexpr u32 kDecideMaxK = 8;
 #ifndef LKF_DEC_PREFETCH
 #define LKF_DEC_PREFETCH 0
 #endif
 template <bool DDK>
-__global__ void __launch_bounds__(64) DECIDE_ATTR k_decide_dt(DecideArgs A, const lkf_pkt *__restrict__ pkts) {
+__global__ void __launch_bounds__(64) DECIDE_ATTR k_decide_dt(DecideArgs A_, const lkf_pkt *__restrict__ pkts) {
+  DecideArgsK A = decide_args();
   __shared__ i32 sDrop[kSetCap];
   __shared__ i32 sEx[kSetCap];
   __shared__ i32 sMissKey[kMissCap];
@@ -2459,19 +2497,19 @@
   __shared__ uint4 sSlot[2 * kDecideMaxK];
   u64 todo;
   {
-    const u32 K = A.perWave, lane = threadIdx.x;
-    const u32 wj = A.waveBase + ((blockIdx.x >> 3) * K + lane) * 8 + (blockIdx.x & 7);
+    const u32 K = A->perWave, lane = threadIdx.x;
+    const u32 wj = A->waveBase + ((blockIdx.x >> 3) * K + lane) * 8 + (blockIdx.x & 7);
     u32 dj = 0xffffffffu, tj = 0, ej = 0, eej = 0, pbj = 0, pej = 0, cj = 0;
-    if (lane < K && wj < A.waveEnd) {
-      dj = A.sched[wj];
-      tj = A.waveTrack[wj];
-      ej = A.evOff[wj];
-      eej = A.evOff[wj + 1];
+    if (lane < K && wj < A->waveEnd) {
+      dj = A->sched[wj];
+      tj = A->waveTrack[wj];
+      ej = A->evOff[wj];
+      eej = A->evOff[wj + 1];
     }
     if (dj != 0xffffffffu) {
-      pbj = A.tBegin[tj];
-      pej = A.tEnd[tj];
-      cj = A.tracks[tj].codec;
+      pbj = A->tBegin[tj];
+      pej = A->tEnd[tj];
+      cj = A->tracks[tj].codec;
     }
     todo = __ballot(dj != 0xffffffffu && (pbj < pej || ej < eej));
     if (lane < K) {
@@ -2483,6 +2521,7 @@
   while (todo) {
   const u32 jw = u32(__ffsll(static_cast<long long>(todo))) - 1;
   todo &= todo - 1;
+  const DecideArgsK A = decide_args();
 #if LKF_SVC_STATS
   const u64 tP0 = __builtin_amdgcn_s_memtime();
   u64 tRun = 0, tStep = 0, tLoad = 0, tSs = 0;
@@ -2497,17 +2536,17 @@
   const u32 track = __builtin_amdgcn_readfirstlane(sa.z);
   u32 ev = __builtin_amdgcn_readfirstlane(sa.w);
   const u32 evEnd = __builtin_amdgcn_readfirstlane(sb.x);
-  CHK(d < A.maxDts, CK_DEC_DT, d, A.maxDts);
-  CHK(track < A.maxTracks, CK_DEC_TRACK, track, A.maxTracks);
-  CHK(evEnd <= A.nev, CK_DEC_EVENT, evEnd, A.nev);
-  const DevDT dt = A.dts[d];
+  CHK(d < A->maxDts, CK_DEC_DT, d, A->maxDts);
+  CHK(track < A->maxTracks, CK_DEC_TRACK, track, A->maxTracks);
+  CHK(evEnd <= A->nev, CK_DEC_EVENT, evEnd, A->nev);
+  const DevDT dt = A->dts[d];
   const u32 pb = __builtin_amdgcn_readfirstlane(sb.y);
   u32 pe = __builtin_amdgcn_readfirstlane(sb.z);
-  const u64 slot0 = A.slotBase[d];
+  const u64 slot0 = A->slotBase[d];
   bool pre = LKF_DEC_PREFETCH && pe - pb <= 64u;
   uint4 r0 = make_uint4(0, 0, 0, 0), r1 = r0, r2 = r0, r3 = r0;
   if (pre && lane < pe - pb) {
-    CHK(pb + lane < A.npkts, CK_DEC_PKT, pb + lane, A.npkts);
+    CHK(pb + lane < A->npkts, CK_DEC_PKT, pb + lane, A->npkts);
     const uint4 *ps = reinterpret_cast<const uint4 *>(pkts) + u64(pb + lane) * 4;
     r0 = ps[0];
     r1 = ps[1];
@@ -2526,34 +2565,34 @@
   __shared__ u32 sHot0[64];
   Lane L{sHot};
   {
-    const u32 h0 = reinterpret_cast<const u32 *>(A.hot + d)[lane];
+    const u32 h0 = reinterpret_cast<const u32 *>(A->hot + d)[lane];
     reinterpret_cast<u32 *>(&sHot)[lane] = h0;
     sHot0[lane] = h0;
   }
   if (lane < sizeof(SenderStats) / 16)
-    reinterpret_cast<uint4 *>(&sSS)[lane] = reinterpret_cast<const uint4 *>(A.ss + d)[lane];
+    reinterpret_cast<uint4 *>(&sSS)[lane] = reinterpret_cast<const uint4 *>(A->ss + d)[lane];
   const bool vp8Track = __builtin_amdgcn_readfirstlane(sb.w) == LKF_CODEC_VP8;
   if (vp8Track && lane < u32(kSetCap)) {
-    sDrop[lane] = A.vc[d].dropKey[lane];
-    sEx[lane] = A.vc[d].exKey[lane];
+    sDrop[lane] = A->vc[d].dropKey[lane];
+    sEx[lane] = A->vc[d].exKey[lane];
   }
   __shared__ __attribute__((aligned(16))) SsEnt sSsBuf[64];
   o.ss = &sSS;
   o.ssBuf = sSsBuf;
   o.ssN = 0;
-  o.ssRing = A.ssRing + size_t(d) * kSnInfoSize;
-  o.ssGap = A.ssGap + size_t(d) * kGapWords;
+  o.ssRing = A->ssRing + size_t(d) * kSnInfoSize;
+  o.ssGap = A->ssGap + size_t(d) * kGapWords;
   __syncthreads();
 #if LKF_SVC_STATS
   const u64 tPa = __builtin_amdgcn_s_memtime();
 #endif
-  RangeEntry *const rmG = A.rm + size_t(d) * kRangeCap;
+  RangeEntry *const rmG = A->rm + size_t(d) * kRangeCap;
   L.rm = sRm;
   L.rmG = rmG;
   L.rmNew = 0;
   L.rmLoaded = false;
   L.vcDirty = false;
-  L.vc = A.vc + d;
+  L.vc = A->vc + d;
   L.dropKey = sDrop;
   L.exKey = sEx;
   L.missKey = sMissKey;
@@ -2565,59 +2604,59 @@
       sMissVal[idx] = L.vc->missVal[idx];
     }
   }
-  if (slot0 + (pe - pb) > A.tupleCap) {
-    if (lane == 0) atomicOr(A.err, 8u);
+  if (slot0 + (pe - pb) > A->tupleCap) {
+    if (lane == 0) atomicOr(A->err, 8u);
     pe = pb;
   }
   __syncthreads();
-  L.seq = A.seq + size_t(d) * A.seqSize;
-  L.seqSize = A.seqSize;
-  L.srm = DDK ? reinterpret_cast<SeqRM *>(A.srm + size_t(d) * A.srmStride) : nullptr;
-  L.srmCap = A.srmCap;
-  const DevTrack &tk = A.tracks[track];
+  L.seq = A->seq + size_t(d) * A->seqSize;
+  L.seqSize = A->seqSize;
+  L.srm = DDK ? reinterpret_cast<SeqRM *>(A->srm + size_t(d) * A->srmStride) : nullptr;
+  L.srmCap = A->srmCap;
+  const DevTrack &tk = A->tracks[track];
   L.kind = tk.kind;
   L.codec = tk.codec;
   L.hasRefTS = tk.hasRefTS;
   L.clockRate = tk.clockRate;
-  L.offs = A.dtOffs + size_t(d) * kDTOffsWords;
+  L.offs = A->dtOffs + size_t(d) * kDTOffsWords;
   L.extPlayout = dt.extPlayout;
   L.extAbs = dt.extAbs;
   L.extDD = dt.extDD;
   L.extTcc = dt.extTcc;
-  L.err = A.err;
-  L.ddPkts = A.ddPkts;
+  L.err = A->err;
+  L.ddPkts = A->ddPkts;
   __shared__ __attribute__((aligned(16))) DDPkt sDDPkt;
   L.ddPktL = &sDDPkt;
-  L.ddSpill = A.ddSpill;
+  L.ddSpill = A->ddSpill;
   L.ddRing = nullptr;
   L.ddS = reinterpret_cast<DDStruct *>(sDDSRaw);
   L.ddSSlot = 0xffffffffu;
   L.dd = sDD;
   L.ddBuf = sDDBuf;
-  o.ddArena = A.ddArena;
-  o.ddUsed = A.ddUsed;
-  o.ddCap = A.ddCap;
+  o.ddArena = A->ddArena;
+  o.ddUsed = A->ddUsed;
+  o.ddCap = A->ddCap;
 #if LKF_CHECKED
   o.tupBase = slot0;
-  o.tupCap = A.tupleCap;
-  CHK(pe <= A.npkts, CK_DEC_PKT, pe, A.npkts);
+  o.tupCap = A->tupleCap;
+  CHK(pe <= A->npkts, CK_DEC_PKT, pe, A->npkts);
 #endif
-  const bool ddDT = DDK && (L.h.flags & F_DD) && A.ddState;
+  const bool ddDT = DDK && (L.h.flags & F_DD) && A->ddState;
   if (ddDT) {
-    L.ddRing = A.ddStructs + size_t(tk.ddIdx) * kDDSlots;
-    const uint4 *g = reinterpret_cast<const uint4 *>(A.ddState + d);
+    L.ddRing = A->ddStructs + size_t(tk.ddIdx) * kDDSlots;
+    const uint4 *g = reinterpret_cast<const uint4 *>(A->ddState + d);
     uint4 *l = reinterpret_cast<uint4 *>(sDD);
-    const u32 nc0 = __builtin_amdgcn_readfirstlane(u32(A.ddState[d].numChains));
+    const u32 nc0 = __builtin_amdgcn_readfirstlane(u32(A->ddState[d].numChains));
     const u32 nDD = (kDDStateHead + nc0 * kDDExpRow * 8) / 16;
     for (u32 i = lane; i < nDD; i += 64) l[i] = g[i];
     __syncthreads();
     if (sDD->flags & DS_KF_VALID) dd_stage_struct(L, sDD, sDDSRaw, lane);
   }
-  o.outT = A.recs + slot0;
-  o.outW = A.wide + slot0;
+  o.outT = A->recs + slot0;
+  o.outW = A->wide + slot0;
   const bool svcDT = DDK && (L.h.flags & F_VIDEO) && !(L.h.flags & F_SIMULCAST) &&
                      ((L.h.flags & F_VP9) || ((L.h.flags & F_DD) && ddDT));
-  u32 nextAt = ev < evEnd ? A.events[ev].at : 0xffffffffu;
+  u32 nextAt = ev < evEnd ? A->events[ev].at : 0xffffffffu;
   const uint4 *src = reinterpret_cast<const uint4 *>(pkts);
 
   u32 kpos = pb;
@@ -2625,13 +2664,15 @@
   const u64 tP1 = __builtin_amdgcn_s_memtime();
 #endif
   while (kpos < pe) {
+    const DecideArgsK A = decide_args();
 #if LKF_SVC_STATS
     const u64 tc0 = __builtin_amdgcn_s_memtime();
 #endif
     if (nextAt <= kpos) {
+      const DecideArgsK A = decide_args();
       while (nextAt <= kpos) {
-        apply_ctl(L, A.events[ev++]);
-        nextAt = ev < evEnd ? A.events[ev].at : 0xffffffffu;
+        apply_ctl(L, A->events[ev++]);
+        nextAt = ev < evEnd ? A->events[ev].at : 0xffffffffu;
       }
       vm_drain();
     }
@@ -2639,10 +2680,10 @@
     u32 pi, n, lim;
     if (steady) {
       const u32 ls = u32(L.h.curS);
-      CHK(size_t(ls) * A.pktStride + kpos < 3 * size_t(A.pktStride), CK_DEC_LAYER, size_t(ls) * A.pktStride + kpos,
-          3 * size_t(A.pktStride));
-      const u32 j = A.layerBefore[size_t(ls) * A.pktStride + kpos] + lane;
-      pi = j < A.layerCnt[track * 3 + ls] ? A.layerList[size_t(ls) * A.pktStride + pb + j] : 0xffffffffu;
+      CHK(size_t(ls) * A->pktStride + kpos < 3 * size_t(A->pktStride), CK_DEC_LAYER, size_t(ls) * A->pktStride + kpos,
+          3 * size_t(A->pktStride));
+      const u32 j = A->layerBefore[size_t(ls) * A->pktStride + kpos] + lane;
+      pi = j < A->layerCnt[track * 3 + ls] ? A->layerList[size_t(ls) * A->pktStride + pb + j] : 0xffffffffu;
       const u32 stopAt = min(nextAt, pe);
       n = u32(__popcll(__ballot(pi < stopAt)));
       lim = n == 64 ? rl32(pi, 63) + 1 : stopAt;
@@ -2655,7 +2696,7 @@
     if (!pre) {
       r0 = r1 = r2 = r3 = make_uint4(0, 0, 0, 0);
       if (valid) {
-        CHK(pi < A.npkts, CK_DEC_PKT, pi, A.npkts);
+        CHK(pi < A->npkts, CK_DEC_PKT, pi, A->npkts);
         const u64 q = u64(pi) * 4;
         r0 = src[q];
         r1 = src[q + 1];
@@ -2673,14 +2714,16 @@
       tLoad += tl0 - tc0;
     }
 #endif
-    const PktV p = decode_pkt(r0, r1, r2, r3);
     u32 pos = 0;
     u32 own = n;
     while (pos < n) {
+      relaunder(r0, r1, r2, r3);
+      const PktV p = decode_pkt(r0, r1, r2, r3);
       if (nextAt <= rl32(pi, pos)) {
+        const DecideArgsK A = decide_args();
         while (nextAt <= rl32(pi, pos)) {
-          apply_ctl(L, A.events[ev++]);
-          nextAt = ev < evEnd ? A.events[ev].at : 0xffffffffu;
+          apply_ctl(L, A->events[ev++]);
+          nextAt = ev < evEnd ? A->events[ev].at : 0xffffffffu;
         }
         vm_drain();
       }
@@ -2883,7 +2926,7 @@
         fwd_base(o, fwR, osn, ots);
         if (fwd) {
 #if LKF_CHECKED
-          CHK(slot0 + o.nFwd + j < A.tupleCap, CK_DEC_TUPLE, slot0 + o.nFwd + j, A.tupleCap);
+          CHK(slot0 + o.nFwd + j < A->tupleCap, CK_DEC_TUPLE, slot0 + o.nFwd + j, A->tupleCap);
 #endif
           store_fwd(o.outT + o.nFwd + j, o.outW + o.nFwd + j, o.bSN, o.bTS, osn, ots, pi, o.relOff + relEx, outLen,
                     ((p.flags & LKF_PKT_KEYFRAME) ? LKF_OUT_KEYFRAME : 0) | (marker ? LKF_OUT_MARKER : 0) |
@@ -2904,7 +2947,7 @@
           CHK(slot < L.seqSize, CK_DEC_SEQ, slot, L.seqSize);
           store_rec(L.seq + slot, m);
         }
-        if (fwd) ss_put(o.ssBuf + o.ssN + j, osn, ots, p.arr, p.poff, u32(payLen), marker, kf);
+        if (fwd) ss_put(o.ssBuf + o.ssN + j, o, u32(o.nFwd) + j, osn, ots, p.arr, p.poff, u32(payLen), marker, kf);
         o.ssN += u32(__popcll(fwR));
         const u32 sumLen = wave_sum_u32(outLen);
         sentAcc += fwd ? i32(p.poff) - hdrLen : 0;
@@ -3022,7 +3065,7 @@
 #if LKF_SVC_STATS
       const u64 ts0 = __builtin_amdgcn_s_memtime();
 #endif
-      ss_flush(sSS, o.ssRing, o.ssGap, sSsBuf, o.ssN, o.bSN, o.bTS);
+      ss_flush(sSS, o.ssRing, o.ssGap, sSsBuf, o.ssN, o.bSN, o.bTS, o.outW);
 #if LKF_SVC_STATS
       tSs += __builtin_amdgcn_s_memtime() - ts0;
 #endif
@@ -3033,14 +3076,16 @@
 #if LKF_SVC_STATS
   const u64 tP2 = __builtin_amdgcn_s_memtime();
 #endif
-  while (ev < evEnd) apply_ctl(L, A.events[ev++]);
+  {
+  const DecideArgsK A = decide_args();
+  while (ev < evEnd) apply_ctl(L, A->events[ev++]);
   __syncthreads();
   {
     const u32 h1 = reinterpret_cast<const u32 *>(&sHot)[lane];
-    if (h1 != sHot0[lane]) reinterpret_cast<u32 *>(A.hot + d)[lane] = h1;
+    if (h1 != sHot0[lane]) reinterpret_cast<u32 *>(A->hot + d)[lane] = h1;
   }
   if (o.nFwd && lane < sizeof(SenderStats) / 16)
-    reinterpret_cast<uint4 *>(A.ss + d)[lane] = reinterpret_cast<const uint4 *>(&sSS)[lane];
+    reinterpret_cast<uint4 *>(A->ss + d)[lane] = reinterpret_cast<const uint4 *>(&sSS)[lane];
   if (L.rmNew) {
     wave_lds_sync();
     const u32 nc = L.h.rmCount, nn = min(L.rmNew, nc);
@@ -3051,7 +3096,7 @@
   }
   if (ddDT) {
     wave_lds_sync();
-    uint4 *g = reinterpret_cast<uint4 *>(A.ddState + d);
+    uint4 *g = reinterpret_cast<uint4 *>(A->ddState + d);
     const uint4 *l = reinterpret_cast<const uint4 *>(sDD);
     const u32 nDD = (kDDStateHead + u32(sDD->numChains) * kDDExpRow * 8) / 16;
     for (u32 i = lane; i < nDD; i += 64) g[i] = l[i];
@@ -3069,20 +3114,21 @@
   }
   const i32 sentRun = i32(wave_sum_u32(u32(sentAcc)));
   if (lane == 0) {
-    A.fwdCnt[d] = u32(o.nFwd);
-    A.fwdBytes[d] = o.relOff;
-    if (o.nFwd) A.fbase[d] = FwdBase{o.bSN, o.bTS};
-    if (o.nFwd) atomicAdd((unsigned long long *)&A.dtCum[d].packets, (unsigned long long)o.nFwd);
+    A->fwdCnt[d] = u32(o.nFwd);
+    A->fwdBytes[d] = o.relOff;
+    if (o.nFwd) A->fbase[d] = FwdBase{o.bSN, o.bTS};
+    if (o.nFwd) atomicAdd((unsigned long long *)&A->dtCum[d].packets, (unsigned long long)o.nFwd);
     const u64 nSent = o.nBytes + u64(i64(sentRun) + o.sentDiff);
-    if (nSent) atomicAdd((unsigned long long *)&A.dtCum[d].bytes, (unsigned long long)nSent);
-    A.dtCum[d].flags = L.h.flags;
-    u64 *st = A.stats + size_t(1 + (w % kStatCopies)) * kStatWords;
+    if (nSent) atomicAdd((unsigned long long *)&A->dtCum[d].bytes, (unsigned long long)nSent);
+    A->dtCum[d].flags = L.h.flags;
+    u64 *st = A->stats + size_t(1 + (w % kStatCopies)) * kStatWords;
     if (o.nTuples) atomicAdd((unsigned long long *)&st[0], (unsigned long long)o.nTuples);
     if (o.nFwd) atomicAdd((unsigned long long *)&st[1], (unsigned long long)o.nFwd);
     if (o.nBytes) atomicAdd((unsigned long long *)&st[2], (unsigned long long)o.nBytes);
 #pragma unroll
     for (int i = 0; i < LKF_DROP_NREASONS; i++)
       if (o.drops[i]) atomicAdd((unsigned long long *)&st[4 + i], (unsigned long long)o.drops[i]);
+  }
   }
 #if LKF_SVC_STATS
   if (DDK && lane == 0 && (L.h.flags & (F_DD | F_VP9))) {
diff --git a/livekit-server_amd/csrc/ingress_kernels.hip b/livekit-server_amd/csrc/ingress_kernels.hip
--- a/livekit-server_amd/csrc/ingress_kernels.hip
+++ b/livekit-server_amd/csrc/ingress_kernels.hip
@@ -857,7 +857,7 @@
   u64 *store;
   u32 *sOwn;
   u64 ep;
-  bool lds;
+  u32 lds, pad;
 };
 __device__ __forceinline__ int bkt_wrap(int x, int M) {
   x %= M;
@@ -935,11 +935,12 @@
   rx_jitter_fold(h, rx_transit(h, clockRate, ets, t), ets);
 }
 
-template <int HS>
-__device__ __noinline__ lkf_flow ing_step(StreamHot &h, u64 *hs, RangeEntry *ring, const DevStream *sg,
-                                         const IngParsed *pg, const lkf_raw_pkt *rg, u32 ic, lkf_flow *flows,
-                                         u32 *fwd, IngDD *ingDD, const u8 *raw, DDIngState *dds,
-                                         DDStruct *ddStructs, u32 *err, const BktCtx *bkg, bool bkOn, u32 *gap) {
+template <int HS, bool DD>
+__device__ __forceinline__ lkf_flow ing_step_body(StreamHot &h, u64 *hs, RangeEntry *ring, const DevStream *sg,
+                                                  const IngParsed *pg, const lkf_raw_pkt *rg, u32 ic, lkf_flow *flows,
+                                                  u32 *fwd, IngDD *ingDD, const u8 *raw, DDIngState *dds,
+                                                  DDStruct *ddStructs, u32 *err, const BktCtx *bkg, bool bkOn,
+                                                  u32 *gap) {
   const DevStream s = *sg;
   const IngParsed p = *pg;
   const lkf_raw_pkt rp = *rg;
@@ -1035,7 +1036,7 @@
     if (dup) break;
     if (bkOn && bkt_add_one(bk, u16(f.ext_sn), rp.len, ic) < 0) break;
     f.flags |= LKF_FLOW_BUCKET;
-    if (payloadSize > 0 && s.ddIdx != 0xffffffffu && p.ddLen) {
+    if (DD && payloadSize > 0 && s.ddIdx != 0xffffffffu && p.ddLen) {
       bool limit = false;
       if (!dd_ingest(*dds, ddStructs + size_t(s.ddIdx) * 2, raw + rp.off + p.ddOff, p.ddLen,
                      u16(f.ext_sn), dv, limit)) {
@@ -1055,8 +1056,24 @@
   } while (false);
   flows[ic] = f;
   fwd[ic] = forward;
-  if (ingDD) ingDD[ic] = dv;
+  if (ingDD) {
+    if (DD) {
+      ingDD[ic] = dv;
+    } else {
+      static_assert(sizeof(IngDD) == 32, "IngDD is two 16-B words");
+      reinterpret_cast<uint4 *>(ingDD + ic)[0] = make_uint4(0, 0, 0, 0);
+      reinterpret_cast<uint4 *>(ingDD + ic)[1] = make_uint4(0, 0, 0, 0);
+    }
+  }
   return f;
+}
+template <int HS>
+__device__ __noinline__ lkf_flow ing_step(StreamHot &h, u64 *hs, RangeEntry *ring, const DevStream *sg,
+                                         const IngParsed *pg, const lkf_raw_pkt *rg, u32 ic, lkf_flow *flows,
+                                         u32 *fwd, IngDD *ingDD, const u8 *raw, DDIngState *dds,
+                                         DDStruct *ddStructs, u32 *err, const BktCtx *bkg, bool bkOn, u32 *gap) {
+  return ing_step_body<HS, true>(h, hs, ring, sg, pg, rg, ic, flows, fwd, ingDD, raw, dds, ddStructs, err, bkg, bkOn,
+                                 gap);
 }
 
 __device__ void closed_flows(const DevStream &s, u32 sid, u32 pb, u32 pe, const lkf_raw_pkt *raws, lkf_flow *flows,
@@ -1213,8 +1230,11 @@
     const u32 end = bad ? u32(__ffsll(static_cast<long long>(bad)) - 1) : 64u;
     if (end == pos) {
       if (lane == pos && rp.stream == sid) {
-        const lkf_flow fo = ing_step<1>(sh, sHist, ring, streams + sid, q + ic, raws + ic, ic, flows, fwd, ingDD, raw,
-                                        dds, ddStructs, err, &sBk, bkOn, gap);
+        const lkf_flow fo =
+            DDK ? ing_step<1>(sh, sHist, ring, streams + sid, q + ic, raws + ic, ic, flows, fwd, ingDD, raw, dds,
+                              ddStructs, err, &sBk, bkOn, gap)
+                : ing_step_body<1, false>(sh, sHist, ring, streams + sid, q + ic, raws + ic, ic, flows, fwd, ingDD,
+                                          raw, dds, ddStructs, err, &sBk, bkOn, gap);
         nkSnFl = nk_snfl(p, fo);
         nkS0 = u32(u16(fo.loss_start));
         nkLen = u32(min<u64>(fo.loss_end - fo.loss_start, 0xffffffffull));
```

Measured after the change: 1.590 billion forwarded RTP pkts/s, median of 6. +5.7%, better.
